# microsoft/StemGNN

Hardware: AMD Instinct MI355X
Metric: forecast-steps/sec (train) (higher is better)
Workload: dtype f32

## Files before the change

### include/stemgnn_hip.h

```cpp
#ifndef STEMGNN_HIP_H
#define STEMGNN_HIP_H

#include <stddef.h>
#include <stdint.h>

#ifdef __cplusplus
extern "C" {
#endif

#define SG_EINVAL (-10001)

#define SG_BLOCK_NPARAMS 33

const char* stemgnn_version(void);
int stemgnn_num_cus(void);

size_t stemgnn_table_floats(int W, int multi);
size_t stemgnn_packed_floats(int W, int multi);
size_t stemgnn_saved_floats(int B, int N, int W, int multi);
size_t stemgnn_scratch_floats(int B, int N, int W, int multi);
size_t stemgnn_gradpart_floats(int W, int multi, int nsplit);
size_t stemgnn_attn_saved_floats(int B, int N);
size_t stemgnn_attn_scratch_floats(int B, int N, int nchunk);
size_t stemgnn_scratch_offset_dG(int B, int N, int W, int multi);
// ... 81 lines not shown
int stemgnn_gru_bwd_rank2_ok(int B, int Hd);
int stemgnn_gru_bwd_rank2(const float* dkey, const float* dquery, const float* wk, const float* wq, const float* x,
                          const float* w_hh, const float* h_ext, const float* reserve, int B, int S, int Hd, int W,
                          float* scratch, float* dw_ih, float* dw_hh, float* db_ih, float* db_hh, int* status, void* stream);
int stemgnn_gru_bwd_rank2_dq(const float* dkey, float* dquery, int nchunk, int flags, const float* wk, const float* wq, const float* x,
                             const float* w_hh, const float* h_ext, const float* reserve, int B, int S, int Hd, int W,
                             float* scratch, float* dw_ih, float* dw_hh, float* db_ih, float* db_hh, int* status, void* stream);
int stemgnn_gru_bwd_overlap_ok(int B, int S, int Hd, int W);
size_t stemgnn_gru_bwd_ctl_words(int S);
int stemgnn_gru_bwd_rank2_begin(const float* dkey, const float* dquery, const float* wk, const float* wq, const float* x,
                                const float* w_hh, const float* h_ext, const float* reserve, int B, int S, int Hd, int W,
                                float* scratch, float* dw_ih, float* dw_hh, float* db_ih, float* db_hh, int* status,
                                unsigned* ctl, void* stream);
int stemgnn_gru_bwd_rank2_finish(const float* dkey, const float* dquery, const float* wk, const float* wq, const float* x,
                                 const float* w_hh, const float* h_ext, const float* reserve, int B, int S, int Hd, int W,
                                 float* scratch, float* dw_ih, float* dw_hh, float* db_ih, float* db_hh, int* status,
                                 unsigned* ctl, void* side_stream, void* stream);
int stemgnn_gru_bwd_recur(const float* dh_all, const float* x, const float* w_hh, const float* h_ext, const float* reserve,
                          int B, int S, int Hd, int W, float* scratch, int* status, void* stream);
int stemgnn_gru_bwd_rank2_recur(const float* dkey, float* dquery, int nchunk, const float* wk, const float* wq, const float* x,
                                const float* w_hh, const float* h_ext, const float* reserve, int B, int S, int Hd, int W,
                                float* scratch, int* status, void* stream);
int stemgnn_gru_input_grad(const float* scratch, const float* w_ih, int B, int S, int Hd, int W, float* dx, void* stream);

int stemgnn_block_pack(const float* const* params_host, const float* tables, float* packed,
                       int W, int multi, void* stream);
int stemgnn_block_pack_panels(const float* const* params_host, const float* tables, float* packed, int W, int multi,
                              void* stream);
int stemgnn_glu_fused_repack(float* packed, int W, int multi, void* stream);
int stemgnn_block_unpack_grads(const float* gradpart, int nsplit, const float* tables,
                               float* const* grads_host, int W, int multi, int has_backcast, void* stream);

int stemgnn_gft_fwd(const float* mul_L, const float* X, long xs_b, long xs_n, long xs_t,
                    float* G, int B, int N, int W, void* stream);
int stemgnn_gft_bwd(const float* mul_L, const float* X, long xs_b, long xs_n, long xs_t,
                    const float* dG, float* dX, float* dmul_L, int accumulate,
                    int B, int N, int W, void* stream);
int stemgnn_gft_bwd_dt2(const float* X0, long xs0_b, long xs0_n, long xs0_t, const float* dG0, const float* X1, long xs1_b,
                        long xs1_n, long xs1_t, const float* dG1, float* dmul_L, int B, int N, int W, void* stream);

int stemgnn_spectral_glu_fwd(const float* packed, float* saved, int B, int N, int W, int multi, void* stream);
int stemgnn_spectral_glu_bwd(const float* packed, const float* saved, float* scratch, float* gradpart,
                             int nsplit, int parts, int B, int N, int W, int multi, void* stream);
size_t stemgnn_glu_split_floats(int W, int multi, int splits);
int stemgnn_glu_split_panels(const float* packed, float* split, int W, int multi, int splits, void* stream);
int stemgnn_spectral_glu_fwd_split(const float* packed, const float* split, float* saved, int B, int N, int W, int multi,
                                   int splits, void* stream);
size_t stemgnn_glu_warm_saved_floats(int W, int multi);
int stemgnn_spectral_glu_fwd_warm(const float* packed, const float* split, float* saved, int B, int N, int W, int multi,
                                  int splits, void* stream);
int stemgnn_spectral_glu_dgrad_split(const float* packed, const float* split, const float* saved, float* scratch,
                                     int B, int N, int W, int multi, int splits, void* stream);
int stemgnn_glu_fused_bf16_ok(int W, int multi, int splits);

int stemgnn_igft_heads_fwd(const float* const* params_host, const float* packed, float* saved,
                           const float* X, long xs_b, long xs_n, long xs_t,
                           float* forecast, int accumulate, float* backcast,
                           int B, int N, int W, int multi, void* stream);
int stemgnn_igft_heads_bwd(const float* const* params_host, const float* packed, const float* saved,
                           const float* X, long xs_b, long xs_n, long xs_t,
                           const float* dforecast, const float* dbackcast, const float* backcast,
                           float* scratch, float* gradpart, int nsplit, int parts,
                           int B, int N, int W, int multi, void* stream);

int stemgnn_shortcut_dx(const float* scratch, const float* bs_w, float* dX, int B, int N, int W, int multi, void* stream);

int stemgnn_block_wgrad(const float* const* params_host, const float* packed, const float* saved,
                        const float* X, long xs_b, long xs_n, long xs_t, const float* dforecast, int has_bc,
                        float* scratch, float* gradpart, int nsplit, int cu_percent,
                        int B, int N, int W, int multi, void* stream);
int stemgnn_block_wgrad_split(const float* const* params_host, const float* packed, const float* saved,
                              const float* X, long xs_b, long xs_n, long xs_t, const float* dforecast, int has_bc,
                              float* scratch, float* gradpart, int nsplit, int cu_percent, int B, int N, int W,
                              int multi, int splits, void* stream);

#define SG_PATH_GLU_FWD_FUSED   1
#define SG_PATH_GLU_DGRAD_FUSED 2
#define SG_PATH_HEADS_FWD_FUSED 4
#define SG_PATH_HEADS_BWD_FUSED 8
#define SG_PATH_HEADS_BWD_16W   16
#define SG_PATH_LONG_K          32
#define SG_PATH_WGRAD_FUSED     64
#define SG_PATH_GLU_WGRAD_FUSED 128
int stemgnn_block_paths(int B, int N, int W, int multi, int splits);

size_t stemgnn_infer_workspace_floats(int B, int N, int W, int multi);
size_t stemgnn_infer_workspace_split_floats(int B, int N, int W, int multi, int splits);
int stemgnn_gru_fwd_infer(const float* x, const float* w_ih, const float* w_hh, const float* b_ih, const float* b_hh,
                          int B, int S, int Hd, int W, float* scratch, float* h_ext, int* status, void* stream);
int stemgnn_spectral_glu_fwd_infer(const float* packed, float* ws, size_t ws_floats, int B, int N, int W, int multi,
                                   void* stream);
int stemgnn_spectral_glu_fwd_split_infer(const float* packed, const float* split, float* ws, size_t ws_floats, int B, int N,
                                         int W, int multi, int splits, void* stream);
int stemgnn_igft_heads_fwd_infer(const float* const* params_host, const float* packed, float* ws, size_t ws_floats,
                                 const float* X, long xs_b, long xs_n, long xs_t, float* forecast, int accumulate,
                                 float* backcast, int B, int N, int W, int multi, void* stream);

int stemgnn_fc_tail_supported(int W, int H);
size_t stemgnn_fc_tail_scratch_floats(int B, int N, int W, int H);
int stemgnn_fc_tail_fwd(const float* fsum, const float* w0, const float* b0, const float* w2, const float* b2,
                        int B, int N, int W, int H, float* forecast, void* stream);
int stemgnn_fc_tail_bwd(const float* dforecast, const float* fsum, const float* w0, const float* b0, const float* w2,
                        int B, int N, int W, int H, float* scratch, float* dfsum, float* dw0, float* db0,
                        float* dw2, float* db2, void* stream);
size_t stemgnn_fc_tail_train_scratch_floats(int B, int N, int W, int H);
int stemgnn_fc_tail_train(const float* fsum, const float* target, const float* w0, const float* b0, const float* w2,
                          const float* b2, int B, int N, int W, int H, float* scratch, float* forecast,
                          float* loss, double* loss_accum, float* dfsum, float* dw0, float* db0, float* dw2,
                          float* db2, void* stream);
int stemgnn_fc_tail_train_rows(const float* fsum, const float* target, const float* w0, const float* b0, const float* w2,
                               const float* b2, int B, int N, int W, int H, float* scratch, float* forecast, float* dfsum,
                               void* stream);
int stemgnn_fc_tail_train_finish(const float* scratch, int B, int N, int W, int H, float* loss, double* loss_accum,
                                 float* dw0, float* db0, float* dw2, float* db2, void* stream);
int stemgnn_fill_zero(void* ptr, size_t bytes, void* stream);
int stemgnn_rmsprop_step(float* params, float* grads, float* square_avg, size_t n, const float* lr_dev,
                         float alpha, float eps, int zero_grad, float grad_scale, void* stream);

int stemgnn_adam_step(float* params, float* grads, float* exp_avg, float* exp_avg_sq, size_t n, const float* lr_dev,
                      float* step_dev, float beta1, float beta2, float eps, int zero_grad, float grad_scale,
                      void* stream);

int stemgnn_normalize_series(const double* raw, const double* sub, const double* div, int clip01, float* out,
                             long T, int N, void* stream);
int stemgnn_window_gather(const float* series, const long long* hi, float* x, float* y, int B, int W, int H, int N,
                          long T, int* status, void* stream);
int stemgnn_window_gather_queue(const float* series, const long long* order, long long* queue, float* x, float* y, int B,
                                int W, int H, int N, long T, int* status, void* stream);
size_t stemgnn_mse_scratch_floats(void);
int stemgnn_mse_fwd(const float* forecast, const float* target, size_t n, float* scratch, float* loss,
                    double* loss_accum, void* stream);
int stemgnn_mse_bwd(const float* forecast, const float* target, size_t n, const float* grad_loss, float* dforecast,
                    void* stream);
int stemgnn_roll_window(const float* inputs, const float* forecast, float* inputs_next, float* forecast_steps,
                        int B, int W, int L, int N, int step, int horizon, void* stream);
int stemgnn_forecast_store(const float* forecast, const float* target, const long long* pos, float* out_forecast,
                           float* out_target, int B, int H, int N, long capacity, void* stream);
size_t stemgnn_eval_scratch_doubles(long count, int H, int N);
size_t stemgnn_eval_out_doubles(int H, int N);
int stemgnn_eval_metrics(const float* target, const float* forecast, const double* mul, const double* add,
                         long count, int H, int N, double* scratch, double* out, void* stream);

#ifdef __cplusplus
}
#endif
#endif
```

### stemgnn_amd/_lib.py

```python
import ctypes
import os
from ctypes import POINTER, c_char_p, c_float, c_int, c_long, c_size_t, c_void_p

_HERE = os.path.dirname(os.path.abspath(__file__))
LIB_PATH = os.environ.get("STEMGNN_HIP_LIB", os.path.join(_HERE, "libstemgnn_hip.so"))
SG_BLOCK_NPARAMS = 33
SG_EINVAL = -10001
SG_PATH = {"glu_fwd_fused": 1, "glu_dgrad_fused": 2, "heads_fwd_fused": 4, "heads_bwd_fused": 8, "heads_bwd_16w": 16,
           "long_k": 32, "wgrad_fused": 64, "glu_wgrad_fused": 128}
SG_GRU_PATH_WORDS = 16
SG_GRU_WORD = {"fwd_family": 0, "fwd_P": 1, "fwd_K": 2, "gi_stream": 3, "bwd_family": 4, "bwd_P": 5, "bwd_KU": 6,
               "bwd_slices": 7, "ih_folded": 8, "hh_form": 9, "ih_slabs": 10, "rank2_ok": 11, "wide_passes": 12,
               "wide_MT": 13, "wide_GWf": 14, "wide_GWb": 15}
SG_GRU_FAM = {"stream": 0, "cluster1": 1, "cluster2": 2, "cluster4": 3, "wide": 4}
SG_GRU_HH = {"slabs": 0, "tiles": 1, "flat": 2}


def gru_paths(B, S, Hd, W, cus=0):
    out = (c_int * SG_GRU_PATH_WORDS)()
    check(load().stemgnn_gru_paths(B, S, Hd, W, cus, out), "stemgnn_gru_paths")
    return {k: int(out[i]) for k, i in SG_GRU_WORD.items()}


_P = c_void_p
_PP = POINTER(c_void_p)

SIGNATURES = {
    "stemgnn_version": (c_char_p, []),
    "stemgnn_num_cus": (c_int, []),
    "stemgnn_table_floats": (c_size_t, [c_int, c_int]),
    "stemgnn_packed_floats": (c_size_t, [c_int, c_int]),
    "stemgnn_saved_floats": (c_size_t, [c_int, c_int, c_int, c_int]),
    "stemgnn_scratch_floats": (c_size_t, [c_int, c_int, c_int, c_int]),
    "stemgnn_scratch_offset_dG": (c_size_t, [c_int, c_int, c_int, c_int]),
    "stemgnn_gradpart_floats": (c_size_t, [c_int, c_int, c_int]),
    "stemgnn_attn_saved_floats": (c_size_t, [c_int, c_int]),
    "stemgnn_attn_scratch_floats": (c_size_t, [c_int, c_int, c_int]),
    "stemgnn_make_tables_host": (c_int, [c_int, c_int, _P]),
    "stemgnn_attn_laplacian_fwd": (c_int, [_P, _P, _P, c_float, c_float, c_int, _P, c_int, c_int, _P, _P, _P, c_int, _P]),
    "stemgnn_attn_laplacian_bwd": (c_int, [_P, _P, _P, _P, c_float, c_float, c_int, _P, c_int, c_int, _P, _P, c_int,
                                           _P, _P, _P, c_int, _P]),
    "stemgnn_attn_laplacian_bwd_ext": (c_int, [_P, _P, _P, _P, _P, c_float, c_float, c_int, _P, c_int, c_int, _P, _P, c_int,
                                               _P, _P, _P, c_int, _P]),
    "stemgnn_dropout_mask": (c_int, [c_float, _P, c_int, c_int, _P, _P]),
    "stemgnn_dropout_seed_next": (c_int, [_P, _P, _P]),
    "stemgnn_cheb_fwd": (c_int, [_P, c_int, _P]),
    "stemgnn_cheb_bwd": (c_int, [_P, _P, _P, _P, c_int, _P]),
    "stemgnn_eigh_scratch_floats": (c_size_t, [c_int]),
    "stemgnn_eigh_fwd": (c_int, [_P, _P, _P, _P, c_int, c_int, _P]),
    "stemgnn_eigh_batched": (c_int, [_P, _P, _P, _P, c_int, c_int, _P]),
    "stemgnn_eigh_status": (c_int, []),
    "stemgnn_eigh_cluster_fixes": (c_int, []),
    "stemgnn_split_planes_floats": (c_size_t, [c_int, c_int, c_int]),
    "stemgnn_split_weights_bf16": (c_int, [_P, c_int, c_int, c_int, _P, _P]),
    "stemgnn_glu_gemm_bf16": (c_int, [_P, _P, _P, c_int, c_int, c_int, c_int, _P]),
    "stemgnn_glu_gemm_f32": (c_int, [_P, _P, _P, c_int, c_int, c_int, _P]),
    "stemgnn_sgemm_f32": (c_int, [_P, c_int, c_int, _P, c_int, c_int, _P, c_int, c_int, c_int, c_int, c_int, _P]),
    "stemgnn_glu_combine_fwd": (c_int, [_P, _P, _P, _P, _P, _P, _P, c_int, c_int, _P]),
    "stemgnn_glu_combine_bwd": (c_int, [_P, _P, _P, _P, _P, c_int, c_int, _P]),
    "stemgnn_colsum": (c_int, [_P, c_int, c_int, _P, _P]),
    "stemgnn_glu_fused_repack": (c_int, [_P, c_int, c_int, _P]),
    "stemgnn_shortcut_dx": (c_int, [_P, _P, _P, c_int, c_int, c_int, c_int, _P]),
    "stemgnn_gru_reserve_floats": (c_size_t, [c_int, c_int, c_int]),
    "stemgnn_gru_fwd_scratch_floats": (c_size_t, [c_int, c_int, c_int]),
    "stemgnn_gru_bwd_scratch_floats": (c_size_t, [c_int, c_int, c_int, c_int]),
    "stemgnn_gru_bwd_cus": (c_int, [c_int, c_int]),
    "stemgnn_gru_paths": (c_int, [c_int, c_int, c_int, c_int, c_int, POINTER(c_int)]),
    "stemgnn_gru_fwd": (c_int, [_P, _P, _P, _P, _P, c_int, c_int, c_int, c_int, _P, _P, _P, _P, _P]),
    "stemgnn_gru_bwd": (c_int, [_P, _P, _P, _P, _P, c_int, c_int, c_int, c_int, _P, _P, _P, _P, _P, _P, _P]),
    "stemgnn_gru_bwd_rank2_ok": (c_int, [c_int, c_int]),
    "stemgnn_gru_bwd_rank2": (c_int, [_P, _P, _P, _P, _P, _P, _P, _P, c_int, c_int, c_int, c_int, _P, _P, _P, _P, _P, _P, _P]),
    "stemgnn_gru_bwd_rank2_dq": (c_int, [_P, _P, c_int, c_int, _P, _P, _P, _P, _P, _P, c_int, c_int, c_int, c_int, _P, _P, _P, _P, _P, _P, _P]),
    "stemgnn_gru_bwd_overlap_ok": (c_int, [c_int, c_int, c_int, c_int]),
    "stemgnn_gru_bwd_ctl_words": (c_size_t, [c_int]),
    "stemgnn_gru_bwd_rank2_begin": (c_int, [_P, _P, _P, _P, _P, _P, _P, _P, c_int, c_int, c_int, c_int, _P, _P, _P, _P, _P, _P, _P, _P]),
    "stemgnn_gru_bwd_rank2_finish": (c_int, [_P, _P, _P, _P, _P, _P, _P, _P, c_int, c_int, c_int, c_int, _P, _P, _P, _P, _P, _P, _P, _P, _P]),
    "stemgnn_gru_bwd_recur": (c_int, [_P, _P, _P, _P, _P, c_int, c_int, c_int, c_int, _P, _P, _P]),
    "stemgnn_gru_bwd_rank2_recur": (c_int, [_P, _P, c_int, _P, _P, _P, _P, _P, _P, c_int, c_int, c_int, c_int, _P, _P, _P]),
    "stemgnn_gru_input_grad": (c_int, [_P, _P, c_int, c_int, c_int, c_int, _P, _P]),
    "stemgnn_keyquery_wgrad": (c_int, [_P, _P, _P, _P, c_int, c_int, _P]),
    "stemgnn_attn_dquery_reduce": (c_int, [_P, c_int, c_int, c_int, _P, _P]),
    "stemgnn_keyquery_wgrad2": (c_int, [_P, _P, _P, _P, _P, c_int, c_int, _P]),
    "stemgnn_fc_tail_supported": (c_int, [c_int, c_int]),
    "stemgnn_fc_tail_scratch_floats": (c_size_t, [c_int, c_int, c_int, c_int]),
    "stemgnn_fc_tail_fwd": (c_int, [_P, _P, _P, _P, _P, c_int, c_int, c_int, c_int, _P, _P]),
    "stemgnn_fc_tail_bwd": (c_int, [_P, _P, _P, _P, _P, c_int, c_int, c_int, c_int, _P, _P, _P, _P, _P, _P, _P]),
    "stemgnn_fill_zero": (c_int, [_P, c_size_t, _P]),
    "stemgnn_rmsprop_step": (c_int, [_P, _P, _P, c_size_t, _P, c_float, c_float, c_int, c_float, _P]),
    "stemgnn_adam_step": (c_int, [_P, _P, _P, _P, c_size_t, _P, _P, c_float, c_float, c_float, c_int, c_float, _P]),
    "stemgnn_normalize_series": (c_int, [_P, _P, _P, c_int, _P, c_long, c_int, _P]),
    "stemgnn_window_gather": (c_int, [_P, _P, _P, _P, c_int, c_int, c_int, c_int, c_long, _P, _P]),
    "stemgnn_window_gather_queue": (c_int, [_P, _P, _P, _P, _P, c_int, c_int, c_int, c_int, c_long, _P, _P]),
    "stemgnn_mse_scratch_floats": (c_size_t, []),
    "stemgnn_mse_fwd": (c_int, [_P, _P, c_size_t, _P, _P, _P, _P]),
    "stemgnn_mse_bwd": (c_int, [_P, _P, c_size_t, _P, _P, _P]),
    "stemgnn_roll_window": (c_int, [_P, _P, _P, _P, c_int, c_int, c_int, c_int, c_int, c_int, _P]),
    "stemgnn_forecast_store": (c_int, [_P, _P, _P, _P, _P, c_int, c_int, c_int, c_long, _P]),
    "stemgnn_eval_scratch_doubles": (c_size_t, [c_long, c_int, c_int]),
    "stemgnn_eval_out_doubles": (c_size_t, [c_int, c_int]),
    "stemgnn_eval_metrics": (c_int, [_P, _P, _P, _P, c_long, c_int, c_int, _P, _P, _P]),
    "stemgnn_block_pack": (c_int, [_PP, _P, _P, c_int, c_int, _P]),
    "stemgnn_block_pack_panels": (c_int, [_PP, _P, _P, c_int, c_int, _P]),
    "stemgnn_block_unpack_grads": (c_int, [_P, c_int, _P, _PP, c_int, c_int, c_int, _P]),
    "stemgnn_gft_fwd": (c_int, [_P, _P, c_long, c_long, c_long, _P, c_int, c_int, c_int, _P]),
    "stemgnn_gft_bwd": (c_int, [_P, _P, c_long, c_long, c_long, _P, _P, _P, c_int, c_int, c_int, c_int, _P]),
    "stemgnn_gft_bwd_dt2": (c_int, [_P, c_long, c_long, c_long, _P, _P, c_long, c_long, c_long, _P, _P, c_int, c_int, c_int, _P]),
    "stemgnn_spectral_glu_fwd": (c_int, [_P, _P, c_int, c_int, c_int, c_int, _P]),
    "stemgnn_spectral_glu_bwd": (c_int, [_P, _P, _P, _P, c_int, c_int, c_int, c_int, c_int, c_int, _P]),
    "stemgnn_glu_split_floats": (c_size_t, [c_int, c_int, c_int]),
    "stemgnn_glu_split_panels": (c_int, [_P, _P, c_int, c_int, c_int, _P]),
    "stemgnn_glu_fused_bf16_ok": (c_int, [c_int, c_int, c_int]),
    "stemgnn_block_paths": (c_int, [c_int, c_int, c_int, c_int, c_int]),
    "stemgnn_spectral_glu_fwd_split": (c_int, [_P, _P, _P, c_int, c_int, c_int, c_int, c_int, _P]),
    "stemgnn_glu_warm_saved_floats": (c_size_t, [c_int, c_int]),
    "stemgnn_spectral_glu_fwd_warm": (c_int, [_P, _P, _P, c_int, c_int, c_int, c_int, c_int, _P]),
    "stemgnn_spectral_glu_dgrad_split": (c_int, [_P, _P, _P, _P, c_int, c_int, c_int, c_int, c_int, _P]),
    "stemgnn_igft_heads_fwd": (c_int, [_PP, _P, _P, _P, c_long, c_long, c_long, _P, c_int, _P,
                                       c_int, c_int, c_int, c_int, _P]),
    "stemgnn_igft_heads_bwd": (c_int, [_PP, _P, _P, _P, c_long, c_long, c_long, _P, _P, _P, _P, _P, c_int, c_int,
                                       c_int, c_int, c_int, c_int, _P]),
    "stemgnn_fc_tail_train_scratch_floats": (c_size_t, [c_int, c_int, c_int, c_int]),
    "stemgnn_fc_tail_train": (c_int, [_P, _P, _P, _P, _P, _P, c_int, c_int, c_int, c_int, _P, _P, _P, _P, _P, _P, _P, _P,
                                      _P, _P]),
    "stemgnn_fc_tail_train_rows": (c_int, [_P, _P, _P, _P, _P, _P, c_int, c_int, c_int, c_int, _P, _P, _P, _P]),
    "stemgnn_fc_tail_train_finish": (c_int, [_P, c_int, c_int, c_int, c_int, _P, _P, _P, _P, _P, _P, _P]),
    "stemgnn_infer_workspace_floats": (c_size_t, [c_int, c_int, c_int, c_int]),
    "stemgnn_infer_workspace_split_floats": (c_size_t, [c_int, c_int, c_int, c_int, c_int]),
    "stemgnn_gru_fwd_infer": (c_int, [_P, _P, _P, _P, _P, c_int, c_int, c_int, c_int, _P, _P, _P, _P]),
    "stemgnn_spectral_glu_fwd_infer": (c_int, [_P, _P, c_size_t, c_int, c_int, c_int, c_int, _P]),
    "stemgnn_spectral_glu_fwd_split_infer": (c_int, [_P, _P, _P, c_size_t, c_int, c_int, c_int, c_int, c_int, _P]),
    "stemgnn_igft_heads_fwd_infer": (c_int, [_PP, _P, _P, c_size_t, _P, c_long, c_long, c_long, _P, c_int, _P,
                                             c_int, c_int, c_int, c_int, _P]),
    "stemgnn_block_wgrad": (c_int, [_PP, _P, _P, _P, c_long, c_long, c_long, _P, c_int, _P, _P, c_int, c_int,
                                    c_int, c_int, c_int, c_int, _P]),
    "stemgnn_block_wgrad_split": (c_int, [_PP, _P, _P, _P, c_long, c_long, c_long, _P, c_int, _P, _P, c_int, c_int,
                                          c_int, c_int, c_int, c_int, c_int, _P]),
}

_lib = None


class StemGNNHipError(RuntimeError):
    pass


def load():
    global _lib
    if _lib is not None:
        return _lib
    if not os.path.isfile(LIB_PATH):
        raise StemGNNHipError(
            f"{LIB_PATH} not found -- build it with `python __graft_entry__.py` (hipcc --offload-arch=gfx950); "
            "stemgnn_amd has no CPU / eager fallback.")
    lib = ctypes.CDLL(LIB_PATH)
    for name, (res, args) in SIGNATURES.items():
        fn = getattr(lib, name)
        fn.restype = res
        fn.argtypes = args
    _lib = lib
    return lib


def check(rc, what):
    if rc != 0:
        if rc == SG_EINVAL:
            raise StemGNNHipError(f"{what}: invalid argument (SG_EINVAL)")
        raise StemGNNHipError(f"{what}: HIP error {-rc}")


def ptr_array(tensors):
    arr = (c_void_p * SG_BLOCK_NPARAMS)()
    for i, t in enumerate(tensors):
        arr[i] = None if t is None else t.data_ptr()
    return arr
```

### stemgnn_amd/base_model.py

```python
import itertools
import os

import torch
import torch.nn as nn

from . import _lib, ops
from .ops import FcTail, FcTailMse, GruFront, SpectralHotPath, StockBlockFn

_instance_counter = itertools.count()
_BLOCK_FIELDS = ("forecast", "forecast_result", "backcast", "backcast_short_cut")
_FC_TAIL_MAX_W, _FC_TAIL_MAX_H = 64, 32


class GLU(nn.Module):

    def __init__(self, input_channel, output_channel):
        super().__init__()
        self.linear_left = nn.Linear(input_channel, output_channel)
        self.linear_right = nn.Linear(input_channel, output_channel)

    def forward(self, x):
        if not x.is_cuda:
            raise _lib.StemGNNHipError(f"input is on {x.device}: stemgnn_amd.GLU runs only on a HIP device (no CPU fallback)")
        lead = x.shape[:-1]
# ... 34 lines not shown
            raise _lib.StemGNNHipError(
                f"input is on {x.device}: stemgnn_amd.StockBlockLayer runs only on a HIP device (no CPU fallback)")
        B, _, N, W = x.shape
        forecast, backcast = StockBlockFn.apply(x.reshape(B, N, W), mul_L, self.multi, self.stack_cnt == 0,
                                                *self.hip_params())
        return forecast, (backcast.unsqueeze(1) if backcast is not None else None)


class Model(nn.Module):
    def __init__(self, units, stack_cnt, time_step, multi_layer, horizon=1, dropout_rate=0.5, leaky_rate=0.2,
                 device='cpu'):
        super().__init__()
        self.unit, self.stack_cnt, self.alpha = units, stack_cnt, leaky_rate
        self.time_step, self.horizon, self.multi_layer = time_step, horizon, multi_layer
        if time_step > _FC_TAIL_MAX_W or horizon > _FC_TAIL_MAX_H:
            raise _lib.StemGNNHipError(
                f"Model(time_step={time_step}, horizon={horizon}): the fc tail kernels (csrc/tail.hip) cover time_step <= "
                f"{_FC_TAIL_MAX_W} and horizon <= {_FC_TAIL_MAX_H}; stemgnn_amd has no torch fallback for larger ones")
        self.dropout_rate = float(dropout_rate)
        self.weight_key = nn.Parameter(torch.zeros(units, 1))
        nn.init.xavier_uniform_(self.weight_key.data, gain=1.414)
        self.weight_query = nn.Parameter(torch.zeros(units, 1))
        nn.init.xavier_uniform_(self.weight_query.data, gain=1.414)
        self.GRU = nn.GRU(time_step, units)
        self.stock_block = nn.ModuleList(
            StockBlockLayer(time_step, units, multi_layer, stack_cnt=i) for i in range(stack_cnt))
        self.fc = nn.Sequential(nn.Linear(time_step, time_step), nn.LeakyReLU(), nn.Linear(time_step, horizon))
        self._seed = None
        self._instance = next(_instance_counter)
        self.hot_state = ops.HotPathState()
        self.to(device)

    def _next_seed(self, device):
        if self._seed is None or self._seed.device != device:
            rank = 0
            if torch.distributed.is_available() and torch.distributed.is_initialized():
                rank = torch.distributed.get_rank()
            key = (torch.cuda.default_generators[device.index if device.index is not None
                                                 else torch.cuda.current_device()].initial_seed()
                   + 0x9E3779B97F4A7C15 * (self._instance + 1) + 0xD1B54A32D192ED03 * rank) % (1 << 62)
            self._seed = torch.tensor([key, 0], dtype=torch.int64, device=device)
        used = torch.empty_like(self._seed)
        _lib.check(_lib.load().stemgnn_dropout_seed_next(self._seed.data_ptr(), used.data_ptr(),
                                                         torch.cuda.current_stream(device).cuda_stream), "dropout_seed_next")
        return used

    def set_dropout_seed(self, seed, offset=0, device=None):
        device = device or self.weight_key.device
        self._seed = torch.tensor([int(seed), int(offset)], dtype=torch.int64, device=device)

    def __getstate__(self):
        state = self.__dict__.copy()
        state["_seed"] = None
        state["hot_state"] = None
        return state

    def __setstate__(self, state):
        self.__dict__.update(state)
        self._instance = next(_instance_counter)
        self.hot_state = ops.HotPathState()

    def train(self, mode=True):
        out = super().train(mode)
        dev = self.weight_key.device if hasattr(self, "weight_key") else None
        if dev is not None and dev.type == "cuda" and ops.gru_status_exists(dev) \
                and not torch.cuda.is_current_stream_capturing():
            ops.check_gru_status(dev)
            if os.environ.get("STEMGNN_SPECTRAL", "cheb") == "eig":
                ops.check_eigh_status(dev)
        return out

    def prefetch_side(self, device=None, batch=None):
        hs = self.hot_state
        if not hs.overlap or hs.prepacked is not None:
            return
        device = device or self.weight_key.device
        blocks = (self.stock_block[0].hip_params(), self.stock_block[1].hip_params())
        ops.prepack_blocks(hs, blocks, self.time_step, self.multi_layer, device,
                           batch_shape=None if batch is None else (int(batch), self.unit))
        if self.training and self.dropout_rate > 0.0:
            with torch.cuda.stream(ops._side_stream(device)):
                hs.preseed = self._next_seed(device)

    def hot_path(self, x):
        if not x.is_cuda:
            raise _lib.StemGNNHipError(
                f"input is on {x.device}: stemgnn_amd.Model runs only on a HIP device (no CPU fallback)")
        if self.stack_cnt > 2:
            raise AttributeError("'NoneType' object has no attribute 'unsqueeze'")
        if self.stack_cnt < 2:
            raise IndexError("list index out of range")
        x = x.contiguous()
        blocks = (self.stock_block[0].hip_params(), self.stock_block[1].hip_params())
        use_drop = self.training and self.dropout_rate > 0.0
        hs = self.hot_state
        if hs.overlap and hs.prepacked is None:
            self.prefetch_side(x.device, batch=x.shape[0])
        seed, hs.preseed = hs.preseed, None
        if seed is not None and not torch.cuda.is_current_stream_capturing():
            seed.record_stream(torch.cuda.current_stream())
        if os.environ.get("STEMGNN_GRU", "hip") == "miopen":
            h, _ = self.GRU(x.permute(2, 0, 1).contiguous())
        else:
            g = self.GRU
            h = GruFront.apply(x, g.weight_ih_l0, g.weight_hh_l0, g.bias_ih_l0, g.bias_hh_l0, hs)
            hs.gru_front_live = True
        if use_drop and seed is None:
            seed = self._next_seed(x.device)
        params = blocks[0] + blocks[1]
        return SpectralHotPath.apply(h, x, self.weight_key, self.weight_query, self.multi_layer, self.alpha,
                                     self.dropout_rate, self.training, seed, hs, *params)

    def loss(self, x, target, loss_out=None, accum=None, unit_grad=False, return_attention=False):
        self._require_fc_tail()
        fsum, attention, _ = self.hot_path(x)
        loss = FcTailMse.apply(fsum, target, self.fc[0].weight, self.fc[0].bias, self.fc[2].weight, self.fc[2].bias,
                               self.hot_state, loss_out, accum, bool(unit_grad) and torch.is_grad_enabled())
        return (loss, attention) if return_attention else loss

    def _require_fc_tail(self):
        if not _lib.load().stemgnn_fc_tail_supported(self.time_step, self.horizon):
            raise _lib.StemGNNHipError(f"fc tail: time_step={self.time_step}, horizon={self.horizon} outside the HIP kernels' "
                                       "range (time_step <= 64, horizon <= 32); stemgnn_amd has no torch fallback")

    def predict(self, x):
        self._require_fc_tail()
        if not x.is_cuda:
            raise _lib.StemGNNHipError(
                f"input is on {x.device}: stemgnn_amd.Model runs only on a HIP device (no CPU fallback)")
        if self.stack_cnt > 2:
            raise AttributeError("'NoneType' object has no attribute 'unsqueeze'")
        if self.stack_cnt < 2:
            raise IndexError("list index out of range")
        g = self.GRU
        blocks = self.stock_block[0].hip_params() + self.stock_block[1].hip_params()
        with torch.no_grad():
            return ops.forecast_forward(x, (g.weight_ih_l0, g.weight_hh_l0, g.bias_ih_l0, g.bias_hh_l0), self.weight_key,
                                        self.weight_query, self.multi_layer, self.alpha, self.dropout_rate, blocks,
                                        (self.fc[0].weight, self.fc[0].bias, self.fc[2].weight, self.fc[2].bias))

    def forward(self, x):
        self._require_fc_tail()
        fsum, attention, _ = self.hot_path(x)
        return FcTail.apply(fsum, self.fc[0].weight, self.fc[0].bias, self.fc[2].weight, self.fc[2].bias,
                            self.hot_state), attention
```

### stemgnn_amd/csrc/block.hip

```cpp
#include <hip/hip_runtime.h>

#include "../../include/stemgnn_hip.h"
#include "devattr.h"
#include "gemm2.h"
#include "gemm2s.h"
#include "gemm_core.h"
#include "gemm_phased.h"
#include "layout.h"
#include "reduce.h"
#include "wgrad.h"
#include "heads.h"
#include "glu_fused.h"
#include "glu_fused_bf16.h"

#define SG_TRY(e)                                \
  do {                                           \
    hipError_t _e = (e);                         \
    if (_e != hipSuccess) return -(int)_e;       \
  } while (0)

__device__ __forceinline__ float sg_sigmoid(float v) { return __frcp_rn(1.f + __expf(-v)); }

struct SgDiv {
  unsigned d, magic;
  __device__ __forceinline__ int div(int x) const { return d == 1u ? x : (int)__umulhi((unsigned)x, magic); }
  __device__ __forceinline__ void divmod(int x, int& q, int& r) const { q = div(x); r = x - q * (int)d; }
};
static inline SgDiv sg_div(int d) {
  SgDiv v;
  v.d = (unsigned)d;
  v.magic = d > 1 ? (unsigned)((1ull << 32) / (unsigned)d + 1ull) : 0u;
  return v;
}
static inline bool sg_div_ok(long xmax, int d) { return d >= 1 && xmax >= 0 && (unsigned long long)xmax * (unsigned)d < (1ull << 32); }

struct XView {
  const float* p;
  long sb, sn, st;
  int N;
  __device__ __forceinline__ float at(int b, int n, int t) const { return p[b * sb + n * sn + t * st]; }
  __device__ __forceinline__ float row(int m, int t) const {
    const int b = m / N;
    return at(b, m - b * N, t);
  }
};

struct GftFwdOp {
  const float* T;
  XView X;
  float* G;
  int B, N, W;
  SgDiv dN, dW;
  __device__ bool setup(int, int& M, int& Nn, int& K0, int& K1) const {
    M = 3 * N; Nn = B * W; K0 = 0; K1 = N;
    return true;
  }
  __device__ float a(int, int i, int k) const { return T[(size_t)i * N + k]; }
  __device__ float b(int, int k, int j) const {
    int bb, t;
    dW.divmod(j, bb, t);
    return X.at(bb, k, t);
  }
  __device__ void epi(int, int i, int j, float v) const {
    int kq, n, bb, t;
    dN.divmod(i, kq, n);
    dW.divmod(j, bb, t);
    G[((size_t)bb * N + n) * (3 * W) + kq * W + t] = v;
  }
};

struct GftBwdDxOp {
  const float* T;
  const float* dG;
  float* dX;
  int B, N, W;
  size_t slab;
  SgDiv dN, dW;
  __device__ bool setup(int, int& M, int& Nn, int& K0, int& K1) const {
    M = N; Nn = B * W; K0 = 0; K1 = 3 * N;
    return true;
  }
  __device__ float a(int, int i, int k) const { return T[(size_t)k * N + i]; }
  __device__ float b(int, int k, int j) const {
    int kq, n, bb, t;
    dN.divmod(k, kq, n);
    dW.divmod(j, bb, t);
    const size_t o = ((size_t)bb * N + n) * (3 * W) + kq * W + t;
    return dG[o] + dG[o + slab];
  }
  __device__ void epi(int, int i, int j, float v) const {
    int bb, t;
    dW.divmod(j, bb, t);
    dX[((size_t)bb * N + i) * W + t] = v;
  }
// ... 943 lines not shown
      a.out0[r] = saved + S.out[r][0]; a.gate0[r] = saved + S.gate[r][0];
      a.dact1[r] = scratch + C.dact[r][1]; a.dact0[r] = scratch + C.dact[r][0];
      a.dG[r] = scratch + C.dG + (size_t)r * d.M * d.KG;
      a.nstA[r] = gdg.nstA[r]; a.ns[r] = gdg.ns[r];
    }
    const dim3 grid(8 * ((a.nrb + 3) / 4));
    const size_t lds = mt == 3 ? gdg.lds_bytes3 : gdg.lds_bytes;
    static SgDynLds guard[4];
#define GD_LAUNCH(MT_, NT_, GI)                                                                            \
    do {                                                                                                  \
      SG_TRY(sg_ensure_dyn_lds((const void*)sg_glu_fused_dgrad_kernel<MT_, NT_>, lds, guard[GI]));         \
      hipLaunchKernelGGL((sg_glu_fused_dgrad_kernel<MT_, NT_>), grid, dim3(256), lds, st, a);              \
    } while (0)
    if (mt == 3) { if (gdg.nt == 2) GD_LAUNCH(3, 2, 3); else GD_LAUNCH(3, 1, 2); }
    else { if (gdg.nt == 2) GD_LAUNCH(2, 2, 1); else GD_LAUNCH(2, 1, 0); }
#undef GD_LAUNCH
    SG_TRY(hipGetLastError());
  }
  for (int l = 2; l >= 0; --l) {
    const int slot = l;
    if ((parts & 2) && !fused) {
      G2Args g;
      GluWgradEpi e;
      for (int r = 0; r < 2; ++r) {
        g.A[r] = scratch + C.dact[r][slot];
        g.lda[r] = sg_glu_np(d, l, r);
        g.B[r] = l == 0 ? saved + S.G : saved + S.out[r][l - 1];
        g.ldb[r] = l == 0 ? d.KG : d.CP;
        g.M[r] = sg_glu_np(d, l, r); g.N[r] = sg_glu_kin(d, l) + 1; g.K[r] = d.M;
        e.part[r] = gradpart + Gl.w[r][l];
      }
      g.nsplit = nsplit; g.chunk = chunk; g.b_ones_col = sg_glu_kin(d, l);
      SG_TRY((g2_launch<GluWgradEpi, false, false>(g, e, 2, st)));
    }
    if (!(parts & 1)) continue;
    if (fused_dgrad) continue;
    if (l > 0) {
      G2Args g;
      GluDpreEpi e;
      for (int r = 0; r < 2; ++r) {
        g.A[r] = scratch + C.dact[r][slot];
        g.lda[r] = sg_glu_np(d, l, r);
        g.B[r] = packed + P.w[r][l];
        g.ldb[r] = sg_glu_np(d, l, r);
        g.M[r] = d.M; g.N[r] = d.CP; g.K[r] = sg_glu_np(d, l, r);
        e.out[r] = saved + S.out[r][l - 1];
        e.gate[r] = saved + S.gate[r][l - 1];
        e.dpre[r] = scratch + C.dact[r][l - 1];
      }
      e.cp = d.CP;
      g.nsplit = 1; g.chunk = (2 * d.CP + 15) & ~15; g.b_ones_col = -1;
      if (2 * d.CP > SG_LONG_K) SG_TRY((g2_launch<GluDpreEpi, true, true, 64, true>(g, e, 2, st)));
      else SG_TRY((g2_launch<GluDpreEpi, true, true, 64>(g, e, 2, st)));
    } else {
      GluDgrad0Op op;
      for (int r = 0; r < 2; ++r) { op.dpre[r] = scratch + C.dact[r][slot]; op.wp[r] = packed + P.w[r][0]; }
      op.dG = scratch + C.dG; op.np0 = sg_glu_np(d, 0, 0); op.KG = d.KG; op.M = d.M;
      if (op.np0 > SG_LONG_K) SG_TRY((sg_launch_gemm<GluDgrad0Op, 32, 64, true, true, false, 64, true>(op, d.M, d.KG, 2, st)));
      else SG_TRY((sg_launch_gemm<GluDgrad0Op, 32, 64, true, true, false, 64>(op, d.M, d.KG, 2, st)));
    }
  }
  if (parts & 2) {
    if (fused) {
      SG_TRY(wg_launch(wq, 6, d.M, gradpart + Gl.wg_ws, reinterpret_cast<unsigned*>(gradpart + Gl.wg_cnt), Gl.wg_smax, st, true, 100,
                       false, nullptr, nullptr, (parts & 4) != 0));
    } else if (nsplit > 1) {
      SgSlabRegions R;
      R.n = 0;
      for (int r = 0; r < 2; ++r)
        for (int l = 0; l < 3; ++l) {
          R.off[R.n] = Gl.w[r][l];
          R.slab[R.n] = (size_t)sg_glu_np(d, l, r) * (sg_glu_kin(d, l) + 1);
          ++R.n;
        }
      SG_TRY(sg_reduce_slabs(gradpart, R, nsplit, st));
    }
  }
  return 0;
}

static bool heads_fused_ok(const SgDims& d) {
  return hd_fwd_lds_floats(d.KF, d.WmP, d.W) * sizeof(float) <= (size_t)150 * 1024 && d.KF <= SG_LONG_K;
}
template <bool SAVE = true>
static int heads_fwd_impl(const float* const* params_host, const float* packed, const float* const (&a3)[2], float* ig, float* fs,
                          const float* X, long xs_b, long xs_n, long xs_t, float* forecast, int accumulate, float* backcast,
                          int B, int N, int W, int multi, void* stream) {
  const SgDims d = sg_dims(B, N, W, multi);
  const SgPackedLayout P = sg_packed_layout(d);
  hipStream_t st = (hipStream_t)stream;
  const int has_bc = backcast != nullptr;
  if (has_bc && (!params_host[5] || !params_host[6])) return SG_EINVAL;
  const size_t hd_bytes = hd_fwd_lds_floats(d.KF, d.WmP, W) * sizeof(float);
  if (heads_fused_ok(d)) {
    HeadsFwdArgs a;
    for (int r = 0; r < 2; ++r) { a.a3[r] = a3[r]; a.cp2[r] = d.CP2[r]; }
    a.wfold = packed + P.wfold;
    a.Fw = params_host[1]; a.Fb = params_host[2]; a.FRw = params_host[3]; a.FRb = params_host[4];
    a.BCw = params_host[5]; a.BCb = params_host[6]; a.BSw = params_host[7]; a.BSb = params_host[8];
    a.X = HdXView{X, xs_b, xs_n, xs_t, N};
    a.ig = ig; a.fs = fs; a.forecast = forecast; a.backcast = backcast;
    a.M = d.M; a.W = W; a.Wm = d.Wm; a.WmP = d.WmP; a.KF = d.KF; a.accumulate = accumulate; a.has_bc = has_bc;
    a.lda = hd_lda(d.KF); a.ldi = d.WmP + 1;
    static const int waves_env = getenv("STEMGNN_HEADS_FWD_WAVES") ? atoi(getenv("STEMGNN_HEADS_FWD_WAVES")) : 8;
    if (waves_env == 8) {
      static SgDynLds lds_guard8;
      SG_TRY(sg_ensure_dyn_lds((const void*)sg_heads_fwd_kernel<8, SAVE>, hd_bytes, lds_guard8));
      hipLaunchKernelGGL((sg_heads_fwd_kernel<8, SAVE>), dim3((d.M + HD_RB - 1) / HD_RB), dim3(512), hd_bytes, st, a);
    } else {
      static SgDynLds lds_guard;
      SG_TRY(sg_ensure_dyn_lds((const void*)sg_heads_fwd_kernel<4, SAVE>, hd_bytes, lds_guard));
      hipLaunchKernelGGL((sg_heads_fwd_kernel<4, SAVE>), dim3((d.M + HD_RB - 1) / HD_RB), dim3(256), hd_bytes, st, a);
    }
    SG_TRY(hipGetLastError());
    return 0;
  }
  {
    IgftOp op;
    if (!ig || !fs) return SG_EINVAL;
    for (int r = 0; r < 2; ++r) { op.a3[r] = a3[r]; op.cp2[r] = d.CP2[r]; }
    op.wfold = packed + P.wfold; op.ig = ig; op.M = d.M; op.Wm = d.Wm; op.WmP = d.WmP;
    if (d.KF > SG_LONG_K) SG_TRY((sg_launch_gemm<IgftOp, 32, 64, true, false, false, 64, true>(op, d.M, d.Wm, 1, st)));
    else SG_TRY((sg_launch_gemm<IgftOp, 32, 64, true, false, false, 64>(op, d.M, d.Wm, 1, st)));
  }
  {
    Head1Op op{ig, XView{X, xs_b, xs_n, xs_t, N},
               params_host[1], params_host[2], params_host[5], params_host[6], params_host[7], params_host[8],
               fs, backcast, d.M, W, d.Wm, has_bc};
    SG_TRY((sg_launch_gemm<Head1Op, 32, 64, true, true, false, 64>(op, d.M, d.Wm + (has_bc ? W : 0), 1, st)));
  }
  {
    Head2Op op{fs, params_host[3], params_host[4], forecast, d.M, W, d.Wm, accumulate};
    SG_TRY((sg_launch_gemm<Head2Op, 64, 32, true, true, false>(op, d.M, W, 1, st)));
  }
  return 0;
}

extern "C" int stemgnn_igft_heads_fwd(const float* const* params_host, const float* packed, float* saved,
                                      const float* X, long xs_b, long xs_n, long xs_t,
                                      float* forecast, int accumulate, float* backcast,
                                      int B, int N, int W, int multi, void* stream) {
  if (!params_host || !packed || !saved || !X || !forecast || B <= 0 || N <= 0 || W <= 0 || multi <= 0)
    return SG_EINVAL;
  const SgSavedLayout S = sg_saved_layout(sg_dims(B, N, W, multi));
  const float* const a3[2] = {saved + S.out[0][2], saved + S.out[1][2]};
  return heads_fwd_impl<true>(params_host, packed, a3, saved + S.ig, saved + S.fs, X, xs_b, xs_n, xs_t, forecast, accumulate,
                              backcast, B, N, W, multi, stream);
}

static bool infer_needs_pp(const SgDims& d, int splits) {
  const char* ef = getenv("STEMGNN_GLU_FUSED");
  const bool fused_on = !(ef && atoi(ef) == 0);
  const bool glu_fused = fused_on && gf_geom(d).ok && gb_geom(d).ok && splits != 3;
  return !glu_fused || !heads_fused_ok(d);
}
static size_t infer_ws_floats(int B, int N, int W, int multi, int splits) {
  if (B <= 0 || N <= 0 || W <= 0 || multi <= 0) return 0;
  const SgDims d = sg_dims(B, N, W, multi);
  return sg_infer_layout(d, infer_needs_pp(d, splits)).total;
}
extern "C" size_t stemgnn_infer_workspace_floats(int B, int N, int W, int multi) { return infer_ws_floats(B, N, W, multi, 0); }
extern "C" size_t stemgnn_infer_workspace_split_floats(int B, int N, int W, int multi, int splits) {
  if (splits != 0 && splits != 2 && splits != 3) return 0;
  return infer_ws_floats(B, N, W, multi, splits);
}
static bool infer_ws_ok(const SgDims& d, size_t ws_floats, bool* pp) {
  *pp = ws_floats >= sg_infer_layout(d, true).total;
  return ws_floats >= sg_infer_layout(d, false).total;
}
extern "C" int stemgnn_spectral_glu_fwd_infer(const float* packed, float* ws, size_t ws_floats, int B, int N, int W, int multi,
                                              void* stream) {
  if (!packed || !ws || B <= 0 || N <= 0 || W <= 0 || multi <= 0) return SG_EINVAL;
  const SgDims d = sg_dims(B, N, W, multi);
  bool pp = false;
  if (!infer_ws_ok(d, ws_floats, &pp)) return SG_EINVAL;
  return glu_fwd_impl<true>(packed, glu_bufs_infer(d, ws, pp), B, N, W, multi, stream, 0, false);
}
extern "C" int stemgnn_spectral_glu_fwd_split_infer(const float* packed, const float* split, float* ws, size_t ws_floats, int B,
                                                    int N, int W, int multi, int splits, void* stream) {
  if (!packed || !split || !ws || B <= 0 || N <= 0 || W <= 0 || multi <= 0 || splits < 2 || splits > 3) return SG_EINVAL;
  const SgDims d = sg_dims(B, N, W, multi);
  bool pp = false;
  if (!infer_ws_ok(d, ws_floats, &pp)) return SG_EINVAL;
  return glu_fwd_split_impl<true>(packed, split, glu_bufs_infer(d, ws, pp), B, N, W, multi, splits, stream);
}
extern "C" int stemgnn_igft_heads_fwd_infer(const float* const* params_host, const float* packed, float* ws, size_t ws_floats,
                                            const float* X, long xs_b, long xs_n, long xs_t, float* forecast, int accumulate,
                                            float* backcast, int B, int N, int W, int multi, void* stream) {
// ... 53 lines not shown
    const size_t hb = hd_bwd_lds_floats(d.WmP, W) * sizeof(float);
    if ((parts & 1) && heads_bwd_fused_ok(d)) {
      HeadsBwdArgs a;
      a.dfo = dforecast; a.dbc = dbackcast; a.bc = backcast; a.fs = saved + S.fs; a.wfold = packed + P.wfold;
      a.Fw = params_host[1]; a.FRw = params_host[3]; a.BCw = params_host[5];
      for (int r = 0; r < 2; ++r) {
        a.out2[r] = saved + S.out[r][2]; a.gate2[r] = saved + S.gate[r][2]; a.dpre2[r] = scratch + C.dact[r][2];
        a.cp2[r] = d.CP2[r];
      }
      a.dpF = dpF; a.dpB = dpB; a.dig = dig;
      a.M = d.M; a.W = W; a.Wm = d.Wm; a.WmP = d.WmP; a.KF = d.KF; a.has_bc = has_bc;
      a.ldi = d.WmP + 1; a.ldw = ((W + 3) & ~3) + 1;
      const int waves = heads_bwd_waves(d);
      if (waves == 16) {
        static SgDynLds lds_guard16;
        SG_TRY(sg_ensure_dyn_lds((const void*)sg_heads_bwd_kernel<16>, hb, lds_guard16));
        hipLaunchKernelGGL(sg_heads_bwd_kernel<16>, dim3((d.M + HD_RB - 1) / HD_RB), dim3(1024), hb, st, a);
      } else if (waves == 8) {
        static SgDynLds lds_guard8;
        SG_TRY(sg_ensure_dyn_lds((const void*)sg_heads_bwd_kernel<8>, hb, lds_guard8));
        hipLaunchKernelGGL(sg_heads_bwd_kernel<8>, dim3((d.M + HD_RB - 1) / HD_RB), dim3(512), hb, st, a);
      } else {
        static SgDynLds lds_guard;
        SG_TRY(sg_ensure_dyn_lds((const void*)sg_heads_bwd_kernel<4>, hb, lds_guard));
        hipLaunchKernelGGL(sg_heads_bwd_kernel<4>, dim3((d.M + HD_RB - 1) / HD_RB), dim3(256), hb, st, a);
      }
      SG_TRY(hipGetLastError());
      fused_data = true;
    }
  }
  if (fused_data) parts &= ~1;
  if ((parts & 1) && has_bc) {
    const size_t n = (size_t)d.M * W;
    const int blocks = (int)((n + 255) / 256 < 2048 ? (n + 255) / 256 : 2048);
    hipLaunchKernelGGL(sg_dsigmoid_kernel, dim3(blocks), dim3(256), 0, st, dbackcast, backcast, dpB, n);
    SG_TRY(hipGetLastError());
  }
  if (parts & 1) {
    Head2BwdOp op{dforecast, params_host[3], saved + S.fs, dpF, d.M, W, d.Wm};
    SG_TRY((sg_launch_gemm<Head2BwdOp, 32, 64, true, false, false>(op, d.M, d.Wm, 1, st)));
  }
  if (parts & 1) {
    DigOp op{dpF, dpB, params_host[1], params_host[5], dig, d.M, W, d.Wm, has_bc};
    SG_TRY((sg_launch_gemm<DigOp, 32, 64, true, false, false, 64>(op, d.M, d.Wm, 1, st)));
  }
  if (parts & 1) {
    Da3Op op;
    op.dig = dig; op.wfold = packed + P.wfold;
    for (int r = 0; r < 2; ++r) {
      op.dpre[r] = scratch + C.dact[r][2];
      op.out[r] = saved + S.out[r][2];
      op.gate[r] = saved + S.gate[r][2];
      op.cp2[r] = d.CP2[r];
    }
    op.M = d.M; op.Wm = d.Wm; op.WmP = d.WmP;
    const int maxN = d.CP2[0] > d.CP2[1] ? d.CP2[0] : d.CP2[1];
    SG_TRY((sg_launch_gemm<Da3Op, 32, 64, true, true, false, 64>(op, d.M, maxN, 2, st)));
  }
  if (parts & 2) {
    HeadsWgradOp op;
    const float* a3[2] = {saved + S.out[0][2], saved + S.out[1][2]};
    const int huge = 1 << 30;
    auto set = [&](int w, const float* A0, int lda, int rows, float sg, const float* Bp, int ldb, int ncolB, float* part,
                   int ldp, int enabled) {
      op.pa0[w] = A0; op.pa1[w] = A0; op.lda0[w] = lda; op.lda1[w] = lda; op.split[w] = huge; op.Mw[w] = rows;
      op.Nw[w] = ldp; op.nb[w] = ncolB; op.rdiv[w] = huge; op.ldp[w] = ldp; op.on[w] = enabled; op.sign[w] = sg;
      op.pb[w] = Bp; op.sb[w] = 0; op.sn[w] = ldb; op.st[w] = 1; op.part[w] = part;
    };
    set(0, dforecast, W, W, 1.f, saved + S.fs, d.Wm, d.Wm, gradpart + Gl.fr, d.Wm + 1, 1);
    set(1, dpF, d.Wm, d.Wm, 1.f, saved + S.ig, d.Wm, d.Wm, gradpart + Gl.fc, d.Wm + 1, 1);
    set(2, dpB, W, W, 1.f, saved + S.ig, d.Wm, d.Wm, gradpart + Gl.bc, d.Wm + 1, has_bc);
    set(3, dpB, W, W, -1.f, X, 0, W, gradpart + Gl.bs, W + 1, has_bc);
    op.rdiv[3] = N; op.sb[3] = xs_b; op.sn[3] = xs_n; op.st[3] = xs_t;
    set(4, a3[0], d.CP2[0], d.KF, 1.f, dig, d.Wm, d.Wm, gradpart + Gl.wfold, d.WmP, 1);
    op.pa1[4] = a3[1]; op.lda1[4] = d.CP2[1]; op.split[4] = d.CP2[0]; op.Nw[4] = d.Wm;
    op.M = d.M; op.S = nsplit; op.chunk = split_chunk(d.M, nsplit);
    const int maxM = d.KF > d.Wm ? d.KF : d.Wm;
    SG_TRY((sg_launch_gemm<HeadsWgradOp, 64, 64, false, false, false, 64>(op, maxM, d.Wm + 1, 5 * nsplit, st)));
    SG_TRY(heads_reduce(d, Gl, gradpart, nsplit, has_bc, 31, st));
  }
  return 0;
}

__global__ void sg_shortcut_dx_kernel(const float* __restrict__ dpB, const float* __restrict__ bs_w, float* __restrict__ dX,
                                      size_t M, int W) {
  const size_t idx = (size_t)blockIdx.x * blockDim.x + threadIdx.x;
  if (idx >= M * W) return;
  const size_t m = idx / W;
  const int t = (int)(idx - m * W);
  float acc = 0.f;
  for (int o = 0; o < W; ++o) acc = fmaf(dpB[m * W + o], bs_w[(size_t)o * W + t], acc);
  dX[idx] -= acc;
}
extern "C" int stemgnn_shortcut_dx(const float* scratch, const float* bs_w, float* dX, int B, int N, int W, int multi,
                                   void* stream) {
  if (!scratch || !bs_w || !dX || B <= 0 || N <= 0 || W <= 0 || multi <= 0) return SG_EINVAL;
  const SgDims d = sg_dims(B, N, W, multi);
  const SgScratchLayout C = sg_scratch_layout(d);
  const size_t n = (size_t)d.M * W;
  hipLaunchKernelGGL(sg_shortcut_dx_kernel, dim3((unsigned)((n + 255) / 256)), dim3(256), 0, (hipStream_t)stream,
                     scratch + C.dpB, bs_w, dX, (size_t)d.M, W);
  SG_TRY(hipGetLastError());
  return 0;
}

static bool block_wgrad_list(const SgDims& d, const float* saved, const float* scratch, const float* dforecast, float* gradpart,
                             const SgGradLayout& Gl, int has_bc, WgGemm* q, int* n_out) {
  const SgSavedLayout S = sg_saved_layout(d);
  const SgScratchLayout C = sg_scratch_layout(d);
  const int W = d.W;
  int n = 0;
  bool ok = true;
  auto add = [&](const float* A, int lda, int Mi, const float* Bp, int ldb, int ncolB, bool ones, float* out, int ldo) {
    WgGemm& g = q[n++];
    g.A = A; g.lda = lda; g.Mi = Mi; g.B = Bp; g.ldb = ldb; g.Nj = ncolB + (ones ? 1 : 0); g.ones_col = ones ? ncolB : -1;
    g.out = out; g.ldo = ldo; g.out_bias = nullptr;
    ok = ok && wg_gemm_ok(g);
  };
  for (int l = 0; l < 3; ++l)
    for (int r = 0; r < 2; ++r)
      add(scratch + C.dact[r][l], sg_glu_np(d, l, r), sg_glu_np(d, l, r), l == 0 ? saved + S.G : saved + S.out[r][l - 1],
          l == 0 ? d.KG : d.CP, sg_glu_kin(d, l), true, gradpart + Gl.w[r][l], sg_glu_kin(d, l) + 1);
  add(dforecast, W, W, saved + S.fs, d.Wm, d.Wm, true, gradpart + Gl.fr, d.Wm + 1);
  add(scratch + C.dpF, d.Wm, d.Wm, saved + S.ig, d.Wm, d.Wm, true, gradpart + Gl.fc, d.Wm + 1);
  if (has_bc) add(scratch + C.dpB, W, W, saved + S.ig, d.Wm, d.Wm, true, gradpart + Gl.bc, d.Wm + 1);
  for (int r = 0; r < 2; ++r)
    add(saved + S.out[r][2], d.CP2[r], d.CP2[r], scratch + C.dig, d.Wm, d.Wm, false,
        gradpart + Gl.wfold + (r ? (size_t)d.CP2[0] * d.WmP : 0), d.WmP);
  *n_out = n;
  return ok && wg_tiles_fit(q, n);
}

static int block_wgrad_impl(const float* const* params_host, const float* packed, const float* saved,
                            const float* X, long xs_b, long xs_n, long xs_t, const float* dforecast, int has_bc,
                            float* scratch, float* gradpart, int nsplit, int cu_percent, int B, int N, int W,
                            int multi, void* stream, int splits) {
  if (!params_host || !packed || !saved || !X || !dforecast || !scratch || !gradpart || nsplit <= 0 || B <= 0 || N <= 0 ||
      W <= 0 || multi <= 0)
    return SG_EINVAL;
  const SgDims d = sg_dims(B, N, W, multi);
  const SgScratchLayout C = sg_scratch_layout(d);
  const SgGradLayout Gl = sg_grad_layout(d, nsplit);
  hipStream_t st = (hipStream_t)stream;
  has_bc = has_bc ? 1 : 0;
  if (has_bc && !params_host[5]) return SG_EINVAL;
  WgGemm q[WG_MAXG];
  int n = 0;
  const bool ok = block_wgrad_list(d, saved, scratch, dforecast, gradpart, Gl, has_bc, q, &n);
  if (!ok) {
    const int rc = stemgnn_igft_heads_bwd(params_host, packed, saved, X, xs_b, xs_n, xs_t, dforecast,
                                          has_bc ? dforecast : nullptr, has_bc ? dforecast : nullptr, scratch, gradpart,
                                          nsplit, 2, B, N, W, multi, stream);
    if (rc) return rc;
    return stemgnn_spectral_glu_bwd(packed, saved, scratch, gradpart, nsplit, 2, B, N, W, multi, stream);
  }
  SG_TRY(wg_launch(q, n, d.M, gradpart + Gl.wg_ws, reinterpret_cast<unsigned*>(gradpart + Gl.wg_cnt), Gl.wg_smax, st, true,
                   cu_percent, false, nullptr, nullptr, splits == 2));
  if (has_bc) {
    HeadsWgradOp op;
    const int huge = 1 << 30;
    for (int w = 0; w < 5; ++w) {
      op.pa0[w] = op.pa1[w] = scratch + C.dpB; op.lda0[w] = op.lda1[w] = W; op.split[w] = huge; op.Mw[w] = W; op.Nw[w] = W + 1;
      op.nb[w] = W; op.rdiv[w] = huge; op.ldp[w] = W + 1; op.on[w] = 0; op.sign[w] = 1.f; op.pb[w] = X; op.sb[w] = 0;
      op.sn[w] = 0; op.st[w] = 1; op.part[w] = gradpart + Gl.bs;
    }
    op.on[3] = 1; op.sign[3] = -1.f; op.rdiv[3] = N; op.sb[3] = xs_b; op.sn[3] = xs_n; op.st[3] = xs_t;
    op.M = d.M; op.S = nsplit; op.chunk = split_chunk(d.M, nsplit);
    SG_TRY((sg_launch_gemm<HeadsWgradOp, 64, 64, false, false, false, 64>(op, W, W + 1, 5 * nsplit, st)));
    SG_TRY(heads_reduce(d, Gl, gradpart, nsplit, 1, 16, st));
  }
  return 0;
}

extern "C" int stemgnn_block_wgrad(const float* const* params_host, const float* packed, const float* saved,
                                   const float* X, long xs_b, long xs_n, long xs_t, const float* dforecast, int has_bc,
                                   float* scratch, float* gradpart, int nsplit, int cu_percent, int B, int N, int W,
                                   int multi, void* stream) {
  return block_wgrad_impl(params_host, packed, saved, X, xs_b, xs_n, xs_t, dforecast, has_bc, scratch, gradpart, nsplit,
                          cu_percent, B, N, W, multi, stream, 0);
}
extern "C" int stemgnn_block_wgrad_split(const float* const* params_host, const float* packed, const float* saved,
                                         const float* X, long xs_b, long xs_n, long xs_t, const float* dforecast, int has_bc,
                                         float* scratch, float* gradpart, int nsplit, int cu_percent, int B, int N, int W,
                                         int multi, int splits, void* stream) {
  if (splits != 0 && splits != 2) return SG_EINVAL;
  return block_wgrad_impl(params_host, packed, saved, X, xs_b, xs_n, xs_t, dforecast, has_bc, scratch, gradpart, nsplit,
                          cu_percent, B, N, W, multi, stream, splits);
}

extern "C" int stemgnn_block_paths(int B, int N, int W, int multi, int splits) {
  if (B <= 0 || N <= 0 || W <= 0 || multi <= 0 || (splits != 0 && splits != 2 && splits != 3)) return SG_EINVAL;
  const SgDims d = sg_dims(B, N, W, multi);
  float* const base = reinterpret_cast<float*>((uintptr_t)256);
  const int nsplit = 32;
  const SgGradLayout Gl = sg_grad_layout(d, nsplit);
  const int mode = glu_fused_mode();
  int bits = 0;
  if (splits == 0 ? glu_fwd_fused_ok(d, mode, base) : glu_fwd_fused_bf16_ok(d, splits)) bits |= SG_PATH_GLU_FWD_FUSED;
  if (splits == 0 ? glu_dgrad_fused_ok(d, mode, base, base) : glu_dgrad_fused_bf16_ok(d, splits, base))
    bits |= SG_PATH_GLU_DGRAD_FUSED;
  if (heads_fused_ok(d)) bits |= SG_PATH_HEADS_FWD_FUSED;
  if (heads_bwd_fused_ok(d)) {
    bits |= SG_PATH_HEADS_BWD_FUSED;
    if (heads_bwd_waves(d) == 16) bits |= SG_PATH_HEADS_BWD_16W;
  }
  if (d.KF > SG_LONG_K) bits |= SG_PATH_LONG_K;
  WgGemm q[WG_MAXG];
  int n = 0;
  if (block_wgrad_list(d, base, base, base, base, Gl, 1, q, &n)) bits |= SG_PATH_WGRAD_FUSED;
  WgGemm wq[6];
  if (glu_wgrad_list(d, base, base, base, Gl, wq)) bits |= SG_PATH_GLU_WGRAD_FUSED;
  return bits;
}
```

### stemgnn_amd/csrc/heads.h

```cpp
#pragma once
#include <hip/hip_runtime.h>

constexpr int HD_RB = 32;
typedef float hd_f4 __attribute__((ext_vector_type(4)));

struct HdXView {
  const float* p;
  long sb, sn, st;
  int N;
};

struct HeadsFwdArgs {
  const float* a3[2];
  int cp2[2];
  const float* wfold;
  const float *Fw, *Fb, *FRw, *FRb, *BCw, *BCb, *BSw, *BSb;
  HdXView X;
  float *ig, *fs, *forecast, *backcast;
  int M, W, Wm, WmP, KF, accumulate, has_bc;
  int lda, ldi;
};

static inline int hd_lda(int KF) { return ((KF + 31) & ~31) + 2; }
static inline size_t hd_fwd_lds_floats(int KF, int WmP, int W) {
  return (size_t)HD_RB * hd_lda(KF) + 2 * (size_t)HD_RB * (WmP + 1) + (size_t)HD_RB * (((W + 3) & ~3) + 1);
}

template <class BF>
__device__ __forceinline__ void hd_gemm_tile(const float* __restrict__ Al, int lda, int K, BF Bf, int j, int kq, int i,
                                             hd_f4& c0, hd_f4& c1) {
  const float* a0p = Al + i * lda + kq;
  const float* a1p = a0p + 16 * lda;
  float b[8], nb[8];
  const int nfull = K >> 5;
  if (nfull > 0) {
#pragma unroll
    for (int u = 0; u < 8; ++u) b[u] = Bf(4 * u + kq, j);
  }
  for (int t = 0; t < nfull; ++t) {
    const int k0 = t << 5;
    if (t + 1 < nfull) {
#pragma unroll
      for (int u = 0; u < 8; ++u) nb[u] = Bf(k0 + 32 + 4 * u + kq, j);
    }
#pragma unroll
    for (int u = 0; u < 8; ++u) {
      c0 = __builtin_amdgcn_mfma_f32_16x16x4f32(a0p[k0 + 4 * u], b[u], c0, 0, 0, 0);
      c1 = __builtin_amdgcn_mfma_f32_16x16x4f32(a1p[k0 + 4 * u], b[u], c1, 0, 0, 0);
    }
#pragma unroll
    for (int u = 0; u < 8; ++u) b[u] = nb[u];
  }
  const int ktail = nfull << 5, nrem = (K - ktail) >> 2;
#pragma unroll
  for (int u = 0; u < 8; ++u) b[u] = u < nrem ? Bf(ktail + 4 * u + kq, j) : 0.f;
#pragma unroll
  for (int u = 0; u < 8; ++u)
    if (u < nrem) {
      c0 = __builtin_amdgcn_mfma_f32_16x16x4f32(a0p[ktail + 4 * u], b[u], c0, 0, 0, 0);
      c1 = __builtin_amdgcn_mfma_f32_16x16x4f32(a1p[ktail + 4 * u], b[u], c1, 0, 0, 0);
    }
}

template <class BF>
__device__ __forceinline__ void hd_gemm_tile1(const float* __restrict__ Al, int lda, int K, BF Bf, int j, int kq, int i,
                                              hd_f4& c0) {
  const float* a0p = Al + i * lda + kq;
  float b[8], nb[8];
  const int nfull = K >> 5;
  if (nfull > 0) {
#pragma unroll
    for (int u = 0; u < 8; ++u) b[u] = Bf(4 * u + kq, j);
  }
  for (int t = 0; t < nfull; ++t) {
    const int k0 = t << 5;
    if (t + 1 < nfull) {
#pragma unroll
      for (int u = 0; u < 8; ++u) nb[u] = Bf(k0 + 32 + 4 * u + kq, j);
    }
#pragma unroll
    for (int u = 0; u < 8; ++u) c0 = __builtin_amdgcn_mfma_f32_16x16x4f32(a0p[k0 + 4 * u], b[u], c0, 0, 0, 0);
#pragma unroll
    for (int u = 0; u < 8; ++u) b[u] = nb[u];
  }
  const int ktail = nfull << 5, nrem = (K - ktail) >> 2;
#pragma unroll
  for (int u = 0; u < 8; ++u) b[u] = u < nrem ? Bf(ktail + 4 * u + kq, j) : 0.f;
#pragma unroll
  for (int u = 0; u < 8; ++u)
    if (u < nrem) c0 = __builtin_amdgcn_mfma_f32_16x16x4f32(a0p[ktail + 4 * u], b[u], c0, 0, 0, 0);
}

__device__ __forceinline__ float hd_sigmoid(float v) { return __frcp_rn(1.f + __expf(-v)); }

template <int NW, bool SAVE = true>
__global__ __launch_bounds__(NW * 64) void sg_heads_fwd_kernel(const HeadsFwdArgs g) {
  constexpr int NT = NW * 64;
  constexpr bool SPLIT = NW == 8;
  extern __shared__ __attribute__((aligned(16))) float hd_lds[];
  float* As = hd_lds;
  float* igs = As + HD_RB * g.lda;
  float* fss = igs + HD_RB * g.ldi;
  float* Xs = fss + HD_RB * g.ldi;
  const int tid = threadIdx.x, lane = tid & 63, wave = tid >> 6;
  const int m0 = blockIdx.x * HD_RB;
  const int M = g.M, W = g.W, Wm = g.Wm, KF = g.KF, lda = g.lda, ldi = g.ldi;
  const int KFp = (KF + 3) & ~3, Wmp4 = (Wm + 3) & ~3, W4 = (W + 3) & ~3;

  {
    const int cpr = KFp >> 2;
    const int nch = HD_RB * cpr;
    const int c0n = g.cp2[0] >> 2;
    for (int base = 0; base < nch; base += NT * 8) {
      float4 v[8];
#pragma unroll
      for (int u = 0; u < 8; ++u) {
        const int e = base + u * NT + tid;
        const int ee = e < nch ? e : nch - 1;
        const int row = ee / cpr, c = ee - row * cpr;
        const int m = m0 + row < M ? m0 + row : M - 1;
        const bool lo = c < c0n;
        const float* src = lo ? g.a3[0] + (size_t)m * g.cp2[0] + 4 * c
                              : g.a3[1] + (size_t)m * g.cp2[1] + 4 * (c - c0n < (g.cp2[1] >> 2) ? c - c0n : 0);
        v[u] = *reinterpret_cast<const float4*>(src);
      }
#pragma unroll
      for (int u = 0; u < 8; ++u) {
        const int e = base + u * NT + tid;
        if (e < nch) {
          const int row = e / cpr, c = e - row * cpr;
          float* d = As + row * lda + 4 * c;
          const bool live = 4 * c < KF;
          *reinterpret_cast<float2*>(d) = live ? make_float2(v[u].x, v[u].y) : make_float2(0.f, 0.f);
          *reinterpret_cast<float2*>(d + 2) = live ? make_float2(v[u].z, v[u].w) : make_float2(0.f, 0.f);
        }
      }
    }
  }
  const int xs = W4 + 1;
  for (int e = tid; e < HD_RB * W4; e += NT) {
    const int row = e / W4, t = e - row * W4;
    const int m = m0 + row < M ? m0 + row : M - 1;
    const int b = m / g.X.N;
    Xs[row * xs + t] = (t < W && g.has_bc) ? g.X.p[b * g.X.sb + (m - b * g.X.N) * g.X.sn + (t < W ? t : 0) * g.X.st] : 0.f;
  }
  for (int e = tid; e < HD_RB * 4; e += NT) {
    const int row = e >> 2, k = Wm + (e & 3);
    if (k < ldi) { igs[row * ldi + k] = 0.f; fss[row * ldi + k] = 0.f; }
  }
  __syncthreads();

  const int j = lane & 15, kq = lane >> 4;
  const int nct = (Wm + 15) >> 4;
  const int cw = SPLIT ? (wave & 3) : wave;
  const int rh = SPLIT ? (wave >> 2) : 0;
  for (int ct = cw; ct < nct; ct += 4) {
    hd_f4 c0 = {0.f, 0.f, 0.f, 0.f}, c1 = c0;
    const float* wf = g.wfold + ct * 16;
    const int WmP = g.WmP;
    auto Bf = [&](int k, int jj) { return wf[(size_t)(k < KF ? k : KF - 1) * WmP + jj]; };
    if constexpr (SPLIT) hd_gemm_tile1(As + rh * 16 * lda, lda, KFp, Bf, j, kq, j, c0);
    else hd_gemm_tile(As, lda, KFp, Bf, j, kq, j, c0, c1);
    const int col = ct * 16 + j;
#pragma unroll
    for (int reg = 0; reg < 4; ++reg) {
      const int r0 = rh * 16 + kq * 4 + reg, r1 = 16 + r0;
      if (col < Wm) {
        igs[r0 * ldi + col] = c0[reg];
        if (SAVE && m0 + r0 < M) g.ig[(size_t)(m0 + r0) * Wm + col] = c0[reg];
        if constexpr (!SPLIT) {
          igs[r1 * ldi + col] = c1[reg];
          if (SAVE && m0 + r1 < M) g.ig[(size_t)(m0 + r1) * Wm + col] = c1[reg];
        }
      }
    }
  }
  __syncthreads();
  for (int ct = cw; ct < nct; ct += 4) {
    hd_f4 c0 = {0.f, 0.f, 0.f, 0.f}, c1 = c0;
    const int col = ct * 16 + j;
    const float* fr = g.Fw + (size_t)(col < Wm ? col : Wm - 1) * Wm;
    auto Bf = [&](int k, int) { return fr[k < Wm ? k : Wm - 1]; };
    if constexpr (SPLIT) hd_gemm_tile1(igs + rh * 16 * ldi, ldi, Wmp4, Bf, j, kq, j, c0);
    else hd_gemm_tile(igs, ldi, Wmp4, Bf, j, kq, j, c0, c1);
    const float bias = g.Fb[col < Wm ? col : Wm - 1];
#pragma unroll
    for (int reg = 0; reg < 4; ++reg) {
      const int r0 = rh * 16 + kq * 4 + reg, r1 = 16 + r0;
      if (col < Wm) {
        const float s0 = hd_sigmoid(c0[reg] + bias);
        fss[r0 * ldi + col] = s0;
        if (SAVE && m0 + r0 < M) g.fs[(size_t)(m0 + r0) * Wm + col] = s0;
        if constexpr (!SPLIT) {
          const float s1 = hd_sigmoid(c1[reg] + bias);
          fss[r1 * ldi + col] = s1;
          if (SAVE && m0 + r1 < M) g.fs[(size_t)(m0 + r1) * Wm + col] = s1;
        }
      }
    }
  }
  __syncthreads();
  const int nwt = (W + 15) >> 4;
  const int rh3 = SPLIT ? ((wave >> 1) & 1) : 0;
  for (int ct = SPLIT ? (wave >> 2) : (wave >> 1); ct < nwt; ct += 2) {
    const int col = ct * 16 + j;
    const int cc = col < W ? col : W - 1;
    hd_f4 c0 = {0.f, 0.f, 0.f, 0.f}, c1 = c0;
    if ((wave & 1) == 0) {
      const float* fr = g.FRw + (size_t)cc * Wm;
      auto Bf = [&](int k, int) { return fr[k < Wm ? k : Wm - 1]; };
      if constexpr (SPLIT) hd_gemm_tile1(fss + rh3 * 16 * ldi, ldi, Wmp4, Bf, j, kq, j, c0);
      else hd_gemm_tile(fss, ldi, Wmp4, Bf, j, kq, j, c0, c1);
      const float bias = g.FRb[cc];
#pragma unroll
      for (int reg = 0; reg < 4; ++reg) {
        const int r0 = rh3 * 16 + kq * 4 + reg, r1 = 16 + r0;
        if (col < W) {
          if (m0 + r0 < M) { float* o = g.forecast + (size_t)(m0 + r0) * W + col; *o = (g.accumulate ? *o : 0.f) + c0[reg] + bias; }
          if constexpr (!SPLIT) {
            if (m0 + r1 < M) { float* o = g.forecast + (size_t)(m0 + r1) * W + col; *o = (g.accumulate ? *o : 0.f) + c1[reg] + bias; }
          }
        }
      }
    } else if (g.has_bc) {
      const float* bcr = g.BCw + (size_t)cc * Wm;
      auto Bc = [&](int k, int) { return bcr[k < Wm ? k : Wm - 1]; };
      hd_f4 d0 = {0.f, 0.f, 0.f, 0.f}, d1 = d0;
      const float* bsr = g.BSw + (size_t)cc * W;
      auto Bs = [&](int k, int) { return bsr[k < W ? k : W - 1]; };
      if constexpr (SPLIT) {
        hd_gemm_tile1(igs + rh3 * 16 * ldi, ldi, Wmp4, Bc, j, kq, j, c0);
        hd_gemm_tile1(Xs + rh3 * 16 * xs, xs, W4, Bs, j, kq, j, d0);
      } else {
        hd_gemm_tile(igs, ldi, Wmp4, Bc, j, kq, j, c0, c1);
        hd_gemm_tile(Xs, xs, W4, Bs, j, kq, j, d0, d1);
      }
      const float bias = g.BCb[cc] - g.BSb[cc];
#pragma unroll
      for (int reg = 0; reg < 4; ++reg) {
        const int r0 = rh3 * 16 + kq * 4 + reg, r1 = 16 + r0;
        if (col < W) {
          if (m0 + r0 < M) g.backcast[(size_t)(m0 + r0) * W + col] = hd_sigmoid(c0[reg] - d0[reg] + bias);
          if constexpr (!SPLIT) {
            if (m0 + r1 < M) g.backcast[(size_t)(m0 + r1) * W + col] = hd_sigmoid(c1[reg] - d1[reg] + bias);
          }
        }
      }
    }
  }
}

struct HeadsBwdArgs {
  const float *dfo, *dbc, *bc;
  const float* fs;
  const float* wfold;
  const float *Fw, *FRw, *BCw;
  const float* out2[2];
  const float* gate2[2];
  float* dpre2[2];
  int cp2[2];
  float *dpF, *dpB, *dig;
  int M, W, Wm, WmP, KF, has_bc;
  int ldi, ldw;
};
static inline size_t hd_bwd_lds_floats(int WmP, int W) {
  return 2 * (size_t)HD_RB * (WmP + 1) + 2 * (size_t)HD_RB * (((W + 3) & ~3) + 1);
}

template <int TJ, class BF>
__device__ __forceinline__ void hd_gemm_tiles(const float* __restrict__ Al, int lda, int K, BF Bf, int kq, int i,
                                              hd_f4 (&c)[TJ][2]) {
  const float* a0p = Al + i * lda + kq;
  const float* a1p = a0p + 16 * lda;
  const int nb8 = (K + 31) >> 5;
  float b[TJ][8], nb[TJ][8];
#pragma unroll
  for (int t = 0; t < TJ; ++t)
#pragma unroll
    for (int u = 0; u < 8; ++u) b[t][u] = Bf(4 * u + kq, t);
  for (int bt = 0; bt < nb8; ++bt) {
    const int k0 = bt << 5;
    if (bt + 1 < nb8) {
#pragma unroll
      for (int t = 0; t < TJ; ++t)
#pragma unroll
        for (int u = 0; u < 8; ++u) nb[t][u] = Bf(k0 + 32 + 4 * u + kq, t);
    }
#pragma unroll
    for (int u = 0; u < 8; ++u) {
      if (k0 + 4 * u < K) {
        const float a0 = a0p[k0 + 4 * u], a1 = a1p[k0 + 4 * u];
#pragma unroll
        for (int t = 0; t < TJ; ++t) {
          c[t][0] = __builtin_amdgcn_mfma_f32_16x16x4f32(a0, b[t][u], c[t][0], 0, 0, 0);
          c[t][1] = __builtin_amdgcn_mfma_f32_16x16x4f32(a1, b[t][u], c[t][1], 0, 0, 0);
        }
      }
    }
#pragma unroll
    for (int t = 0; t < TJ; ++t)
#pragma unroll
      for (int u = 0; u < 8; ++u) b[t][u] = nb[t][u];
  }
}

template <int NW>
__global__ __launch_bounds__(NW * 64) void sg_heads_bwd_kernel(const HeadsBwdArgs g) {
  constexpr int NT = NW * 64;
  extern __shared__ __attribute__((aligned(16))) float hd_lds[];
  float* dpFs = hd_lds;
  float* digs = dpFs + HD_RB * g.ldi;
  float* dfos = digs + HD_RB * g.ldi;
  float* dpBs = dfos + HD_RB * g.ldw;
  const int tid = threadIdx.x, lane = tid & 63, wave = tid >> 6;
  const int m0 = blockIdx.x * HD_RB;
  const int M = g.M, W = g.W, Wm = g.Wm, KF = g.KF, ldi = g.ldi, ldw = g.ldw, WmP = g.WmP;
  const int Wmp4 = (Wm + 3) & ~3, W4 = (W + 3) & ~3;

  const int j = lane & 15, kq = lane >> 4;
  const int nkt = (KF + 15) >> 4;
  constexpr int TJ = 16 / NW;
  const bool hoist = nkt <= 16;
  float gt[TJ][2][4], yv[TJ][2][4];
  auto load_saved = [&](int ct0) {
#pragma unroll
    for (int t = 0; t < TJ; ++t) {
      const int kk = (ct0 + t) * 16 + j;
      const int kc = kk < KF ? kk : KF - 1;
      const int r = kc >= g.cp2[0];
      const int cch = kc - (r ? g.cp2[0] : 0), cp = g.cp2[r];
      const float* pg = g.gate2[r] + cch;
      const float* py = g.out2[r] + cch;
#pragma unroll
      for (int reg = 0; reg < 4; ++reg)
#pragma unroll
        for (int h = 0; h < 2; ++h) {
          const int mm = m0 + h * 16 + kq * 4 + reg;
          const size_t o = (size_t)(mm < M ? mm : M - 1) * cp;
          gt[t][h][reg] = pg[o];
          yv[t][h][reg] = py[o];
        }
    }
  };
  if (hoist) load_saved(wave * TJ);
  const int nct = (Wm + 15) >> 4;
  const bool hoist_fs = nct <= NW;
  float sv[2][4];
  auto load_fs = [&](int ct) {
    const int col = ct * 16 + j, cc = col < Wm ? col : Wm - 1;
#pragma unroll
    for (int reg = 0; reg < 4; ++reg)
#pragma unroll
      for (int h = 0; h < 2; ++h) {
        const int r = h * 16 + kq * 4 + reg;
        const int m = m0 + r < M ? m0 + r : M - 1;
        sv[h][reg] = g.fs[(size_t)m * Wm + cc];
      }
  };
  if (hoist_fs) load_fs(wave < nct ? wave : nct - 1);

  for (int e = tid; e < HD_RB * W4; e += NT) {
    const int row = e / W4, t = e - row * W4;
    const int m = m0 + row < M ? m0 + row : M - 1;
    const size_t o = (size_t)m * W + (t < W ? t : 0);
    const float df = g.dfo[o];
    float pb = 0.f;
    if (g.has_bc) {
      const float s = g.bc[o];
      pb = g.dbc[o] * s * (1.f - s);
      if (t < W && m0 + row < M) g.dpB[o] = pb;
    }
    dfos[row * ldw + t] = t < W ? df : 0.f;
    dpBs[row * ldw + t] = t < W ? pb : 0.f;
  }
  for (int e = tid; e < HD_RB * 4; e += NT) {
    const int row = e >> 2, k = Wm + (e & 3);
    if (k < ldi) { dpFs[row * ldi + k] = 0.f; digs[row * ldi + k] = 0.f; }
  }
  __syncthreads();

  for (int ct = wave; ct < nct; ct += NW) {
    hd_f4 c[1][2] = {{{0.f, 0.f, 0.f, 0.f}, {0.f, 0.f, 0.f, 0.f}}};
    const int col = ct * 16 + j, cc = col < Wm ? col : Wm - 1;
    const float* fr = g.FRw + cc;
    hd_gemm_tiles<1>(dfos, ldw, W4, [&](int k, int) { return fr[(size_t)(k < W ? k : W - 1) * Wm]; }, kq, j, c);
    if (!hoist_fs) load_fs(ct);
#pragma unroll
    for (int reg = 0; reg < 4; ++reg)
#pragma unroll
      for (int h = 0; h < 2; ++h) {
        const int r = h * 16 + kq * 4 + reg;
        const float s = sv[h][reg];
        const float v = c[0][h][reg] * s * (1.f - s);
        if (col < Wm) {
          dpFs[r * ldi + col] = v;
          if (m0 + r < M) g.dpF[(size_t)(m0 + r) * Wm + col] = v;
        }
      }
  }
  __syncthreads();
  for (int ct = wave; ct < nct; ct += NW) {
    hd_f4 c[1][2] = {{{0.f, 0.f, 0.f, 0.f}, {0.f, 0.f, 0.f, 0.f}}};
    const int col = ct * 16 + j, cc = col < Wm ? col : Wm - 1;
    const float* fw = g.Fw + cc;
    hd_gemm_tiles<1>(dpFs, ldi, Wmp4, [&](int k, int) { return fw[(size_t)(k < Wm ? k : Wm - 1) * Wm]; }, kq, j, c);
    if (g.has_bc) {
      const float* bw = g.BCw + cc;
      hd_gemm_tiles<1>(dpBs, ldw, W4, [&](int k, int) { return bw[(size_t)(k < W ? k : W - 1) * Wm]; }, kq, j, c);
    }
#pragma unroll
    for (int reg = 0; reg < 4; ++reg)
#pragma unroll
      for (int h = 0; h < 2; ++h) {
        const int r = h * 16 + kq * 4 + reg;
        if (col < Wm) {
          digs[r * ldi + col] = c[0][h][reg];
          if (m0 + r < M) g.dig[(size_t)(m0 + r) * Wm + col] = c[0][h][reg];
        }
      }
  }
  __syncthreads();
  for (int ct0 = wave * TJ; ct0 < nkt; ct0 += TJ * NW) {
    hd_f4 c[TJ][2];
#pragma unroll
    for (int t = 0; t < TJ; ++t) { c[t][0] = (hd_f4){0.f, 0.f, 0.f, 0.f}; c[t][1] = c[t][0]; }
    const float* wr[TJ];
#pragma unroll
    for (int t = 0; t < TJ; ++t) {
      const int kk = (ct0 + t) * 16 + j;
      wr[t] = g.wfold + (size_t)(kk < KF ? kk : KF - 1) * WmP;
    }
    hd_gemm_tiles<TJ>(digs, ldi, Wmp4, [&](int k, int t) { return wr[t][k < Wm ? k : Wm - 1]; }, kq, j, c);
    if (!hoist) load_saved(ct0);
#pragma unroll
    for (int t = 0; t < TJ; ++t) {
      const int kk = (ct0 + t) * 16 + j;
      const int kc = kk < KF ? kk : KF - 1;
      const int r = kc >= g.cp2[0];
      const int cch = kc - (r ? g.cp2[0] : 0), cp = g.cp2[r];
      const int q = ((cch >> 4) << 5) + (cch & 15);
#pragma unroll
      for (int reg = 0; reg < 4; ++reg)
#pragma unroll
        for (int h = 0; h < 2; ++h) {
          const int m = m0 + h * 16 + kq * 4 + reg;
          const float v = c[t][h][reg];
          if (m < M && kk < KF) {
            float* dp = g.dpre2[r] + (size_t)m * 2 * cp + q;
            dp[0] = v * gt[t][h][reg];
            dp[16] = v * yv[t][h][reg] * (1.f - gt[t][h][reg]);
          }
        }
    }
  }
}
```

### stemgnn_amd/csrc/tail.hip

```cpp
#include <hip/hip_runtime.h>
#include <stdint.h>

#include "../../include/stemgnn_hip.h"
#include "devattr.h"

#define SG_TRY(e)                                \
  do {                                           \
    hipError_t _e = (e);                         \
    if (_e != hipSuccess) return -(int)_e;       \
  } while (0)

constexpr int TAIL_MAXW = 64;
constexpr int TAIL_MAXH = 32;
constexpr int TAIL_RB = 64;


__global__ __launch_bounds__(256) void sg_fc_tail_fwd_kernel(const float* __restrict__ fsum, const float* __restrict__ w0,
                                                             const float* __restrict__ b0, const float* __restrict__ w2,
                                                             const float* __restrict__ b2, int B, int N, int W, int H,
                                                             float* __restrict__ forecast) {
  extern __shared__ __attribute__((aligned(16))) float sm[];
  float* sw0 = sm;
  float* sb0 = sw0 + W * W;
  float* sw2 = sb0 + W;
  float* sb2 = sw2 + H * W;
  float* sx = sb2 + H;
  float* sa = sx + TAIL_RB * (W + 1);
  const int tid = threadIdx.x, r = tid & 63, q = tid >> 6;
  const int M = B * N, m0 = blockIdx.x * TAIL_RB, m = m0 + r;
  for (int i = tid; i < W * W; i += 256) sw0[i] = w0[i];
  for (int i = tid; i < W; i += 256) sb0[i] = b0[i];
  for (int i = tid; i < H * W; i += 256) sw2[i] = w2[i];
  for (int i = tid; i < H; i += 256) sb2[i] = b2[i];
  for (int i = tid; i < TAIL_RB * W; i += 256) {
    const int rr = i / W, t = i - rr * W;
    sx[rr * (W + 1) + t] = m0 + rr < M ? fsum[(size_t)m0 * W + i] : 0.f;
  }
  __syncthreads();
  for (int t = q; t < W; t += 4) {
    float z = sb0[t];
    for (int u = 0; u < W; ++u) z = fmaf(sx[r * (W + 1) + u], sw0[t * W + u], z);
    sa[r * (W + 1) + t] = z > 0.f ? z : 0.01f * z;
  }
  __syncthreads();
  if (m < M) {
    const int b = m / N, n = m - b * N;
    for (int h = q; h < H; h += 4) {
      float y = sb2[h];
      for (int t = 0; t < W; ++t) y = fmaf(sa[r * (W + 1) + t], sw2[h * W + t], y);
      forecast[((size_t)b * H + h) * N + n] = y;
    }
  }
}

__global__ __launch_bounds__(256) void sg_fc_tail_bwd_kernel(const float* __restrict__ dforecast, const float* __restrict__ fsum,
                                                             const float* __restrict__ w0, const float* __restrict__ b0,
                                                             const float* __restrict__ w2, int B, int N, int W, int H,
                                                             float* __restrict__ dfsum, float* __restrict__ partial) {
  extern __shared__ __attribute__((aligned(16))) float sm[];
  const int nacc = W * W + W + H * W + H;
  float* sw0 = sm;
  float* sb0 = sw0 + W * W;
  float* sw2 = sb0 + W;
  float* sx = sw2 + H * W;
  float* sdz = sx + TAIL_RB * (W + 1);
  float* sa = sdz + TAIL_RB * (W + 1);
  float* sdy = sa + TAIL_RB * (W + 1);
  const int tid = threadIdx.x, r = tid & 63, q = tid >> 6;
  const int M = B * N, m0 = blockIdx.x * TAIL_RB, m = m0 + r;
  for (int i = tid; i < W * W; i += 256) sw0[i] = w0[i];
  for (int i = tid; i < W; i += 256) sb0[i] = b0[i];
  for (int i = tid; i < H * W; i += 256) sw2[i] = w2[i];
  for (int i = tid; i < TAIL_RB * W; i += 256) {
    const int rr = i / W, t = i - rr * W;
    sx[rr * (W + 1) + t] = m0 + rr < M ? fsum[(size_t)m0 * W + i] : 0.f;
  }
  {
    const int mc = m < M ? m : 0, b = mc / N, n = mc - b * N;
    for (int h = q; h < H; h += 4) sdy[r * (H + 1) + h] = m < M ? dforecast[((size_t)b * H + h) * N + n] : 0.f;
  }
  __syncthreads();
  for (int t = q; t < W; t += 4) {
    float z = sb0[t];
    for (int u = 0; u < W; ++u) z = fmaf(sx[r * (W + 1) + u], sw0[t * W + u], z);
    float da = 0.f;
    for (int h = 0; h < H; ++h) da = fmaf(sdy[r * (H + 1) + h], sw2[h * W + t], da);
    sa[r * (W + 1) + t] = m < M ? (z > 0.f ? z : 0.01f * z) : 0.f;
    sdz[r * (W + 1) + t] = m < M ? (z > 0.f ? da : 0.01f * da) : 0.f;
  }
  __syncthreads();
  if (m < M)
    for (int u = q; u < W; u += 4) {
      float d = 0.f;
      for (int t = 0; t < W; ++t) d = fmaf(sdz[r * (W + 1) + t], sw0[t * W + u], d);
      dfsum[(size_t)m * W + u] = d;
    }
// ... 1 lines not shown
    float sum = 0.f;
    if (e < W * W) {
      const int t = e / W, u = e - t * W;
      for (int rr = 0; rr < TAIL_RB; ++rr) sum = fmaf(sdz[rr * (W + 1) + t], sx[rr * (W + 1) + u], sum);
    } else if (e < W * W + W) {
      const int t = e - W * W;
      for (int rr = 0; rr < TAIL_RB; ++rr) sum += sdz[rr * (W + 1) + t];
    } else if (e < W * W + W + H * W) {
      const int qq = e - W * W - W, h = qq / W, t = qq - h * W;
      for (int rr = 0; rr < TAIL_RB; ++rr) sum = fmaf(sdy[rr * (H + 1) + h], sa[rr * (W + 1) + t], sum);
    } else {
      const int h = e - W * W - W - H * W;
      for (int rr = 0; rr < TAIL_RB; ++rr) sum += sdy[rr * (H + 1) + h];
    }
    partial[(size_t)blockIdx.x * nacc + e] = sum;
  }
}

__global__ __launch_bounds__(256) void sg_fc_tail_reduce_kernel(const float* __restrict__ partial, int nblocks, int W, int H,
                                                                float* __restrict__ dw0, float* __restrict__ db0,
                                                                float* __restrict__ dw2, float* __restrict__ db2) {
  __shared__ float red[4][64];
  const int nacc = W * W + W + H * W + H;
  const int i = blockIdx.x * 64 + (threadIdx.x & 63), q = threadIdx.x >> 6;
  float s = 0.f;
  if (i < nacc)
    for (int b = q; b < nblocks; b += 4) s += partial[(size_t)b * nacc + i];
  red[q][threadIdx.x & 63] = s;
  __syncthreads();
  if (q != 0 || i >= nacc) return;
  s = (red[0][threadIdx.x] + red[1][threadIdx.x]) + (red[2][threadIdx.x] + red[3][threadIdx.x]);
  if (i < W * W) dw0[i] = s;
  else if (i < W * W + W) db0[i - W * W] = s;
  else if (i < W * W + W + H * W) dw2[i - W * W - W] = s;
  else db2[i - W * W - W - H * W] = s;
}

static size_t fc_tail_fwd_lds(int W, int H) { return (size_t)(W * W + W + H * W + H + 2 * TAIL_RB * (W + 1)) * sizeof(float); }
static size_t fc_tail_bwd_lds(int W, int H) {
  return (size_t)(W * W + W + H * W + TAIL_RB * (3 * (W + 1) + H + 1)) * sizeof(float);
}
extern "C" int stemgnn_fc_tail_supported(int W, int H) {
  return W > 0 && H > 0 && W <= TAIL_MAXW && H <= TAIL_MAXH && fc_tail_bwd_lds(W, H) <= 150 * 1024;
}
extern "C" size_t stemgnn_fc_tail_scratch_floats(int B, int N, int W, int H) {
  return (size_t)((B * N + TAIL_RB - 1) / TAIL_RB) * (W * W + W + H * W + H);
}

extern "C" int stemgnn_fc_tail_fwd(const float* fsum, const float* w0, const float* b0, const float* w2, const float* b2,
                                   int B, int N, int W, int H, float* forecast, void* stream) {
  if (!fsum || !w0 || !b0 || !w2 || !b2 || !forecast || B <= 0 || N <= 0 || !stemgnn_fc_tail_supported(W, H))
    return SG_EINVAL;
  const size_t lds = fc_tail_fwd_lds(W, H);
  static SgDynLds lds_guard;
  SG_TRY(sg_ensure_dyn_lds((const void*)sg_fc_tail_fwd_kernel, lds, lds_guard));
  hipLaunchKernelGGL(sg_fc_tail_fwd_kernel, dim3((B * N + TAIL_RB - 1) / TAIL_RB), dim3(256), lds, (hipStream_t)stream, fsum,
                     w0, b0, w2, b2, B, N, W, H, forecast);
  SG_TRY(hipGetLastError());
  return 0;
}

extern "C" int stemgnn_fc_tail_bwd(const float* dforecast, const float* fsum, const float* w0, const float* b0,
                                   const float* w2, int B, int N, int W, int H, float* scratch, float* dfsum, float* dw0,
                                   float* db0, float* dw2, float* db2, void* stream) {
  if (!dforecast || !fsum || !w0 || !b0 || !w2 || !scratch || !dfsum || !dw0 || !db0 || !dw2 || !db2 || B <= 0 ||
      N <= 0 || W <= 0 || H <= 0 || W > TAIL_MAXW || H > TAIL_MAXH)
    return SG_EINVAL;
  hipStream_t st = (hipStream_t)stream;
  const int nacc = W * W + W + H * W + H;
  const int nblocks = (B * N + TAIL_RB - 1) / TAIL_RB;
  const size_t lds = fc_tail_bwd_lds(W, H);
  if (!stemgnn_fc_tail_supported(W, H)) return SG_EINVAL;
  static SgDynLds lds_guard;
  SG_TRY(sg_ensure_dyn_lds((const void*)sg_fc_tail_bwd_kernel, lds, lds_guard));
  hipLaunchKernelGGL(sg_fc_tail_bwd_kernel, dim3(nblocks), dim3(256), lds, st, dforecast, fsum, w0, b0, w2, B, N, W, H, dfsum,
                     scratch);
  SG_TRY(hipGetLastError());
  hipLaunchKernelGGL(sg_fc_tail_reduce_kernel, dim3((nacc + 63) / 64), dim3(256), 0, st, scratch, nblocks, W, H, dw0,
                     db0, dw2, db2);
  SG_TRY(hipGetLastError());
  return 0;
}

constexpr int TRAIN_RB = 32;
constexpr int TRAIN_RQ = 256 / TRAIN_RB;
__global__ __launch_bounds__(256) void sg_fc_tail_train_kernel(const float* __restrict__ fsum, const float* __restrict__ target,
                                                               const float* __restrict__ w0, const float* __restrict__ b0,
                                                               const float* __restrict__ w2, const float* __restrict__ b2,
                                                               int B, int N, int W, int H, float* __restrict__ forecast,
                                                               float* __restrict__ dfsum, float* __restrict__ partial) {
  extern __shared__ __attribute__((aligned(16))) float sm[];
  const int nacc = W * W + W + H * W + H;
  float* sw0 = sm;
  float* sb0 = sw0 + W * W;
  float* sw2 = sb0 + W;
  float* sb2 = sw2 + H * W;
  float* sx = sb2 + H;
  float* sdz = sx + TRAIN_RB * (W + 1);
  float* sa = sdz + TRAIN_RB * (W + 1);
  float* sdy = sa + TRAIN_RB * (W + 1);
  float* sred = sdy + TRAIN_RB * (H + 1);
  const int tid = threadIdx.x, r = tid % TRAIN_RB, q = tid / TRAIN_RB;
  const int M = B * N, m0 = blockIdx.x * TRAIN_RB, m = m0 + r;
  for (int i = tid; i < W * W; i += 256) sw0[i] = w0[i];
  for (int i = tid; i < W; i += 256) sb0[i] = b0[i];
  for (int i = tid; i < H * W; i += 256) sw2[i] = w2[i];
  for (int i = tid; i < H; i += 256) sb2[i] = b2[i];
  for (int i = tid; i < TRAIN_RB * W; i += 256) {
    const int rr = i / W, t = i - rr * W;
    sx[rr * (W + 1) + t] = m0 + rr < M ? fsum[(size_t)m0 * W + i] : 0.f;
  }
  __syncthreads();
  for (int t = q; t < W; t += TRAIN_RQ) {
    float z = sb0[t];
    for (int u = 0; u < W; ++u) z = fmaf(sx[r * (W + 1) + u], sw0[t * W + u], z);
    sdz[r * (W + 1) + t] = z;
    sa[r * (W + 1) + t] = m < M ? (z > 0.f ? z : 0.01f * z) : 0.f;
  }
  __syncthreads();
  float sq = 0.f;
  {
    const int mc = m < M ? m : 0, b = mc / N, n = mc - b * N;
    const float scale = 2.f / ((float)B * (float)H * (float)N);
    for (int h = q; h < H; h += TRAIN_RQ) {
      float y = sb2[h];
      for (int t = 0; t < W; ++t) y = fmaf(sa[r * (W + 1) + t], sw2[h * W + t], y);
      const size_t o = ((size_t)b * H + h) * N + n;
      const float d = m < M ? y - target[o] : 0.f;
      if (m < M && forecast) forecast[o] = y;
      sq = fmaf(d, d, sq);
      sdy[r * (H + 1) + h] = d * scale;
    }
  }
  sred[tid] = sq;
  __syncthreads();
  for (int t = q; t < W; t += TRAIN_RQ) {
    const float z = sdz[r * (W + 1) + t];
    float da = 0.f;
    for (int h = 0; h < H; ++h) da = fmaf(sdy[r * (H + 1) + h], sw2[h * W + t], da);
    sdz[r * (W + 1) + t] = m < M ? (z > 0.f ? da : 0.01f * da) : 0.f;
  }
  __syncthreads();
  if (m < M)
    for (int u = q; u < W; u += TRAIN_RQ) {
      float d = 0.f;
      for (int t = 0; t < W; ++t) d = fmaf(sdz[r * (W + 1) + t], sw0[t * W + u], d);
      dfsum[(size_t)m * W + u] = d;
    }
  for (int e = tid; e < nacc + 1; e += 256) {
    float sum = 0.f;
    if (e < W * W) {
      const int t = e / W, u = e - t * W;
      for (int rr = 0; rr < TRAIN_RB; ++rr) sum = fmaf(sdz[rr * (W + 1) + t], sx[rr * (W + 1) + u], sum);
    } else if (e < W * W + W) {
      const int t = e - W * W;
      for (int rr = 0; rr < TRAIN_RB; ++rr) sum += sdz[rr * (W + 1) + t];
    } else if (e < W * W + W + H * W) {
      const int qq = e - W * W - W, h = qq / W, t = qq - h * W;
      for (int rr = 0; rr < TRAIN_RB; ++rr) sum = fmaf(sdy[rr * (H + 1) + h], sa[rr * (W + 1) + t], sum);
    } else if (e < nacc) {
      const int h = e - W * W - W - H * W;
      for (int rr = 0; rr < TRAIN_RB; ++rr) sum += sdy[rr * (H + 1) + h];
    } else {
      for (int i = 0; i < 256; ++i) sum += sred[i];
    }
    partial[(size_t)blockIdx.x * (nacc + 1) + e] = sum;
  }
}

__global__ __launch_bounds__(256) void sg_fc_tail_train_reduce_kernel(const float* __restrict__ partial, int nblocks, int W,
                                                                      int H, float inv_n, float* __restrict__ dw0,
                                                                      float* __restrict__ db0, float* __restrict__ dw2,
                                                                      float* __restrict__ db2, float* __restrict__ loss,
                                                                      double* __restrict__ accum) {
  __shared__ float red[4][64];
  const int nacc = W * W + W + H * W + H;
  const int i = blockIdx.x * 64 + (threadIdx.x & 63), q = threadIdx.x >> 6;
  float s = 0.f;
  if (i <= nacc)
    for (int b = q; b < nblocks; b += 32) {
      float v[8];
#pragma unroll
      for (int u = 0; u < 8; ++u) {
        const int bb = b + 4 * u;
        const float x = partial[(size_t)(bb < nblocks ? bb : nblocks - 1) * (nacc + 1) + i];
        v[u] = bb < nblocks ? x : 0.f;
      }
#pragma unroll
      for (int u = 0; u < 8; ++u) s += v[u];
    }
  red[q][threadIdx.x & 63] = s;
  __syncthreads();
  if (q != 0 || i > nacc) return;
  s = (red[0][threadIdx.x] + red[1][threadIdx.x]) + (red[2][threadIdx.x] + red[3][threadIdx.x]);
  if (i < W * W) dw0[i] = s;
  else if (i < W * W + W) db0[i - W * W] = s;
  else if (i < W * W + W + H * W) dw2[i - W * W - W] = s;
  else if (i < nacc) db2[i - W * W - W - H * W] = s;
  else {
    const float l = s * inv_n;
    loss[0] = l;
    if (accum) accum[0] += (double)l;
  }
}

static size_t fc_tail_train_lds(int W, int H) {
  return (size_t)(W * W + W + H * W + H + TRAIN_RB * (3 * (W + 1) + H + 1) + 256) * sizeof(float);
}
extern "C" size_t stemgnn_fc_tail_train_scratch_floats(int B, int N, int W, int H) {
  return (size_t)((B * N + TRAIN_RB - 1) / TRAIN_RB) * (W * W + W + H * W + H + 1);
}
static int fc_tail_train_impl(const float* fsum, const float* target, const float* w0, const float* b0, const float* w2,
                              const float* b2, int B, int N, int W, int H, float* scratch, float* forecast, float* loss,
                              double* loss_accum, float* dfsum, float* dw0, float* db0, float* dw2, float* db2, void* stream,
                              int parts) {
  if (!scratch || B <= 0 || N <= 0 || !stemgnn_fc_tail_supported(W, H) || fc_tail_train_lds(W, H) > 150 * 1024) return SG_EINVAL;
  if ((parts & 1) && (!fsum || !target || !w0 || !b0 || !w2 || !b2 || !dfsum)) return SG_EINVAL;
  if ((parts & 2) && (!loss || !dw0 || !db0 || !dw2 || !db2)) return SG_EINVAL;
  hipStream_t st = (hipStream_t)stream;
  const int nacc = W * W + W + H * W + H;
  const int nblocks = (B * N + TRAIN_RB - 1) / TRAIN_RB;
  if (parts & 1) {
    const size_t lds = fc_tail_train_lds(W, H);
    static SgDynLds lds_guard;
    SG_TRY(sg_ensure_dyn_lds((const void*)sg_fc_tail_train_kernel, lds, lds_guard));
    hipLaunchKernelGGL(sg_fc_tail_train_kernel, dim3(nblocks), dim3(256), lds, st, fsum, target, w0, b0, w2, b2, B, N, W, H,
                       forecast, dfsum, scratch);
    SG_TRY(hipGetLastError());
  }
  if (parts & 2) {
    hipLaunchKernelGGL(sg_fc_tail_train_reduce_kernel, dim3((nacc + 1 + 63) / 64), dim3(256), 0, st, scratch, nblocks, W, H,
                       1.f / ((float)B * (float)H * (float)N), dw0, db0, dw2, db2, loss, loss_accum);
    SG_TRY(hipGetLastError());
  }
  return 0;
}
extern "C" int stemgnn_fc_tail_train(const float* fsum, const float* target, const float* w0, const float* b0, const float* w2,
                                     const float* b2, int B, int N, int W, int H, float* scratch, float* forecast,
                                     float* loss, double* loss_accum, float* dfsum, float* dw0, float* db0, float* dw2,
                                     float* db2, void* stream) {
  return fc_tail_train_impl(fsum, target, w0, b0, w2, b2, B, N, W, H, scratch, forecast, loss, loss_accum, dfsum, dw0, db0, dw2,
                            db2, stream, 3);
}
extern "C" int stemgnn_fc_tail_train_rows(const float* fsum, const float* target, const float* w0, const float* b0,
                                          const float* w2, const float* b2, int B, int N, int W, int H, float* scratch,
                                          float* forecast, float* dfsum, void* stream) {
  return fc_tail_train_impl(fsum, target, w0, b0, w2, b2, B, N, W, H, scratch, forecast, nullptr, nullptr, dfsum, nullptr,
                            nullptr, nullptr, nullptr, stream, 1);
}
extern "C" int stemgnn_fc_tail_train_finish(const float* scratch, int B, int N, int W, int H, float* loss, double* loss_accum,
                                            float* dw0, float* db0, float* dw2, float* db2, void* stream) {
  return fc_tail_train_impl(nullptr, nullptr, nullptr, nullptr, nullptr, nullptr, B, N, W, H, const_cast<float*>(scratch),
                            nullptr, loss, loss_accum, nullptr, dw0, db0, dw2, db2, stream, 2);
}

__global__ void sg_rmsprop_kernel(float* __restrict__ p, float* __restrict__ g, float* __restrict__ sq, size_t n,
                                  const float* __restrict__ lr_dev, float alpha, float eps, int zero_grad,
                                  float gscale) {
  const float lr = lr_dev[0];
  size_t i = ((size_t)blockIdx.x * blockDim.x + threadIdx.x) * 4;
  const size_t stride = (size_t)gridDim.x * blockDim.x * 4;
  for (; i + 3 < n; i += stride) {
    float4 pv = *reinterpret_cast<float4*>(p + i), gv = *reinterpret_cast<float4*>(g + i),
           sv = *reinterpret_cast<float4*>(sq + i);
    gv.x *= gscale; gv.y *= gscale; gv.z *= gscale; gv.w *= gscale;
    sv.x = alpha * sv.x + (1.f - alpha) * gv.x * gv.x; pv.x -= lr * gv.x / (sqrtf(sv.x) + eps);
    sv.y = alpha * sv.y + (1.f - alpha) * gv.y * gv.y; pv.y -= lr * gv.y / (sqrtf(sv.y) + eps);
    sv.z = alpha * sv.z + (1.f - alpha) * gv.z * gv.z; pv.z -= lr * gv.z / (sqrtf(sv.z) + eps);
    sv.w = alpha * sv.w + (1.f - alpha) * gv.w * gv.w; pv.w -= lr * gv.w / (sqrtf(sv.w) + eps);
    *reinterpret_cast<float4*>(p + i) = pv;
    *reinterpret_cast<float4*>(sq + i) = sv;
    if (zero_grad) *reinterpret_cast<float4*>(g + i) = make_float4(0.f, 0.f, 0.f, 0.f);
  }
  if (i < n && i + 3 >= n) {
    for (size_t j = i; j < n; ++j) {
      const float gv = g[j] * gscale;
      const float sv = alpha * sq[j] + (1.f - alpha) * gv * gv;
      sq[j] = sv;
      p[j] -= lr * gv / (sqrtf(sv) + eps);
      if (zero_grad) g[j] = 0.f;
    }
  }
}

extern "C" int stemgnn_fill_zero(void* ptr, size_t bytes, void* stream) {
  if (!ptr && bytes) return SG_EINVAL;
  SG_TRY(sg_zero_async(ptr, bytes, (hipStream_t)stream));
  return 0;
}

// ... 49 lines not shown
```

### stemgnn_amd/ops.py

```python
import os
import weakref

import torch

from . import _lib

_NSPLIT = 32
_side_streams = {}


def _side_stream(device, index=0):
    key = (str(device), index)
    st = _side_streams.get(key)
    if st is None:
        st = torch.cuda.Stream(device=device)
        _side_streams[key] = st
    return st


def fresh_side_stream(device, index=0):
    _side_streams.pop((str(device), index), None)
    return _side_stream(device, index)


class HotPathState:

    def __init__(self):
        self.direct = False
        self.overlap = False
        self.prepacked = None
        self.preseed = None
        self.fork_event = None
        self.pending = None
        self.exact_group = None
        self.gru_front_live = False
        self.dh_factors = None
        self.block_grads_hook = None
        self.gru_ctl = None
        self.gru_ctl_zeroed = False
        self.warm_saved = None
        self.tail_finish = None
        self.side_probe = None
        _states.add(self)

    def set(self, direct=True, overlap=False):
        self.direct = bool(direct)
        self.overlap = bool(direct) and bool(overlap)
        return self

    def join(self):
        item, self.pending = self.pending, None
        if item is not None:
            side, keep = item
            torch.cuda.current_stream().wait_stream(side)
            del keep

    def reset(self):
        for item in (self.prepacked, self.pending):
            if item is not None:
                try:
                    (item[1] if item is self.prepacked else item[0]).synchronize()
                except RuntimeError:
                    pass
        self.prepacked = None
        self.preseed = None
        self.fork_event = None
        self.pending = None
        self.dh_factors = None
        self.gru_ctl_zeroed = False
        self.tail_finish = None


_states = weakref.WeakSet()
_NO_STATE = None


def _state(state):
    global _NO_STATE
    if state is not None:
        return state
    if _NO_STATE is None:
        _NO_STATE = HotPathState()
# ... 195 lines not shown
                                                     gru_status(dev).data_ptr(), _stream()), "gru_bwd_recur")
        elif factors is not None:
            attn_scratch, fb, fn, wk, wq, after, dq_chunks = factors
            base = attn_scratch.data_ptr() + 4 * fn * fn
            tail = (x.data_ptr(), w_hh.data_ptr(), h_ext.data_ptr(), reserve.data_ptr(), B, S, Hd, W, scratch.data_ptr(),
                    dw_ih.data_ptr(), dw_hh.data_ptr(), db_ih.data_ptr(), db_hh.data_ptr(), gru_status(dev).data_ptr())
            args = (base, base + 4 * fb * fn, wk.data_ptr(), wq.data_ptr()) + tail
            beside = (ctx.state.overlap and ctx.state.pending is not None and ctx.state.gru_ctl_zeroed
                      and bool(lib.stemgnn_gru_bwd_overlap_ok(B, S, Hd, W))
                      and ctx.state.gru_ctl.numel() == lib.stemgnn_gru_bwd_ctl_words(S))
            ctx.state.gru_ctl_zeroed = False
            ctl = ctx.state.gru_ctl.data_ptr() if beside else None
            if beside:
                _lib.check(lib.stemgnn_gru_bwd_rank2_begin(*args, ctl, _stream()), "gru_bwd_rank2_begin")
            elif dq_chunks:
                wg_split = 1 if glu_splits() == 2 and os.environ.get("STEMGNN_WGRAD_BF16", "1") != "0" else 0
                _lib.check(lib.stemgnn_gru_bwd_rank2_dq(base, base + 4 * fb * fn, dq_chunks, wg_split, wk.data_ptr(), wq.data_ptr(),
                                                        *tail, _stream()), "gru_bwd_rank2_dq")
            else:
                _lib.check(lib.stemgnn_gru_bwd_rank2(*args, _stream()), "gru_bwd_rank2")
            if after is not None:
                after()
            if beside:
                side = ctx.state.pending[0]
                _lib.check(lib.stemgnn_gru_bwd_rank2_finish(*args, ctl, side.cuda_stream, _stream()), "gru_bwd_rank2_finish")
        else:
            _lib.check(lib.stemgnn_gru_bwd(dh_all.data_ptr(), x.data_ptr(), w_hh.data_ptr(), h_ext.data_ptr(),
                                           reserve.data_ptr(), B, S, Hd, W, scratch.data_ptr(), dw_ih.data_ptr(),
                                           dw_hh.data_ptr(), db_ih.data_ptr(), db_hh.data_ptr(),
                                           gru_status(dev).data_ptr(), _stream()), "gru_bwd")
        dx = None
        if ctx.needs_input_grad[0]:
            dx = torch.empty(B, W, S, device=dev, dtype=f32)
            _lib.check(lib.stemgnn_gru_input_grad(scratch.data_ptr(), w_ih.data_ptr(), B, S, Hd, W, dx.data_ptr(), _stream()),
                       "gru_input_grad")
        ctx.state.join()
        if direct or frozen:
            return dx, None, None, None, None, None
        return dx, dw_ih, dw_hh, db_ih, db_hh, None


class FcTail(torch.autograd.Function):

    @staticmethod
    def forward(ctx, fsum, w0, b0, w2, b2, state=None):
        lib = _lib.load()
        ctx.state = _state(state)
        fsum = fsum.contiguous()
        B, N, W = fsum.shape
        H = w2.shape[0]
        forecast = torch.empty(B, H, N, device=fsum.device, dtype=torch.float32)
        w0, b0, w2, b2 = (t.contiguous() for t in (w0, b0, w2, b2))
        _lib.check(lib.stemgnn_fc_tail_fwd(fsum.data_ptr(), w0.data_ptr(), b0.data_ptr(), w2.data_ptr(), b2.data_ptr(),
                                           B, N, W, H, forecast.data_ptr(), _stream()), "fc_tail_fwd")
        ctx.save_for_backward(fsum, w0, b0, w2)
        ctx.fc_params = (w0, b0, w2, b2)
        return forecast

    @staticmethod
    def backward(ctx, dforecast):
        lib = _lib.load()
        fsum, w0, b0, w2 = ctx.saved_tensors
        B, N, W = fsum.shape
        H = w2.shape[0]
        dev, f32 = fsum.device, torch.float32
        dforecast = dforecast.contiguous()
        prm = ctx.fc_params
        direct = ctx.state.direct and all(p.grad is not None and p.grad.is_contiguous() for p in prm)
        if direct:
            dw0, db0, dw2, db2 = (p.grad for p in prm)
        else:
            dw0, db0, dw2, db2 = (torch.empty_like(p) for p in prm)
        dfsum = torch.empty_like(fsum)
        scratch = torch.empty(lib.stemgnn_fc_tail_scratch_floats(B, N, W, H), device=dev, dtype=f32)
        _lib.check(lib.stemgnn_fc_tail_bwd(dforecast.data_ptr(), fsum.data_ptr(), w0.data_ptr(), b0.data_ptr(),
                                           w2.data_ptr(), B, N, W, H, scratch.data_ptr(), dfsum.data_ptr(),
                                           dw0.data_ptr(), db0.data_ptr(), dw2.data_ptr(), db2.data_ptr(), _stream()),
                   "fc_tail_bwd")
        if direct:
            return dfsum, None, None, None, None, None
        return dfsum, dw0, db0, dw2, db2, None


class FcTailMse(torch.autograd.Function):

    @staticmethod
    def forward(ctx, fsum, target, w0, b0, w2, b2, state=None, loss_out=None, accum=None, unit_grad=False):
        lib = _lib.load()
        ctx.state = _state(state)
        _require_gpu(fsum, "fsum")
        _require_gpu(target, "target")
        fsum, target = fsum.contiguous(), target.contiguous()
        B, N, W = fsum.shape
        H = w2.shape[0]
        if tuple(target.shape) != (B, H, N):
            raise _lib.StemGNNHipError(f"target must be [B,H,N]=({B},{H},{N}), got {tuple(target.shape)}")
        dev, f32 = fsum.device, torch.float32
        prm = (w0, b0, w2, b2)
        w0c, b0c, w2c, b2c = (t.contiguous() for t in prm)
        wanted = any(ctx.needs_input_grad[i] for i in (0, 2, 3, 4, 5))
        direct = ctx.state.direct and bool(unit_grad) and wanted and \
            all(p.grad is not None and p.grad.is_contiguous() for p in prm)
        grads = [p.grad for p in prm] if direct else [torch.empty_like(p) for p in prm]
        dfsum = torch.empty_like(fsum)
        loss = loss_out if loss_out is not None else torch.empty((), device=dev, dtype=f32)
        if accum is not None and (accum.dtype != torch.float64 or accum.device != dev):
            raise _lib.StemGNNHipError("accum must be a float64 scalar on the forecast's device")
        scratch = torch.empty(lib.stemgnn_fc_tail_train_scratch_floats(B, N, W, H), device=dev, dtype=f32)

        acc_ptr = accum.data_ptr() if accum is not None else None
        defer = direct and ctx.state.overlap and ctx.state.tail_finish is None
        if defer:
            _lib.check(lib.stemgnn_fc_tail_train_rows(
                fsum.data_ptr(), target.data_ptr(), w0c.data_ptr(), b0c.data_ptr(), w2c.data_ptr(), b2c.data_ptr(), B, N, W, H,
                scratch.data_ptr(), None, dfsum.data_ptr(), _stream()), "fc_tail_train_rows")
            g0, g1, g2, g3 = grads

            def finish(stream, scratch=scratch, loss=loss, g0=g0, g1=g1, g2=g2, g3=g3):
                _lib.check(lib.stemgnn_fc_tail_train_finish(scratch.data_ptr(), B, N, W, H, loss.data_ptr(), acc_ptr, g0.data_ptr(),
                                                            g1.data_ptr(), g2.data_ptr(), g3.data_ptr(), stream),
                           "fc_tail_train_finish")
            ctx.state.tail_finish = finish
        else:
            _lib.check(lib.stemgnn_fc_tail_train(
                fsum.data_ptr(), target.data_ptr(), w0c.data_ptr(), b0c.data_ptr(), w2c.data_ptr(), b2c.data_ptr(), B, N, W, H,
                scratch.data_ptr(), None, loss.data_ptr(), acc_ptr, dfsum.data_ptr(),
                grads[0].data_ptr(), grads[1].data_ptr(), grads[2].data_ptr(), grads[3].data_ptr(), _stream()), "fc_tail_train")
        ctx.direct, ctx.unit_grad = direct, bool(unit_grad)
        ctx.held = (dfsum, None if direct else grads)
        ctx.set_materialize_grads(False)
        if loss_out is not None:
            ctx.mark_dirty(loss_out)
        return loss

    @staticmethod
    def backward(ctx, grad_loss):
        dfsum, grads = ctx.held
        ctx.held = None
        if ctx.state.tail_finish is not None and not ctx.state.overlap:
            fin, ctx.state.tail_finish = ctx.state.tail_finish, None
            fin(_stream())
        if not ctx.unit_grad:
            dfsum = dfsum * grad_loss
            if grads is not None:
                grads = [g * grad_loss for g in grads]
        if grads is None:
            return dfsum, None, None, None, None, None, None, None, None, None
        return dfsum, None, grads[0], grads[1], grads[2], grads[3], None, None, None, None


class GluFn(torch.autograd.Function):

    @staticmethod
    def forward(ctx, x, wl, bl, wr, br):
        lib = _lib.load()
        for name, t in (("x", x), ("linear_left.weight", wl), ("linear_right.weight", wr)):
            _require_gpu(t, name)
        x, wl, bl, wr, br = (t.contiguous() for t in (x, wl, bl, wr, br))
        M, K = x.shape
        C = wl.shape[0]
        dev, st = x.device, _stream()
        U = torch.empty(M, C, device=dev)
        V = torch.empty(M, C, device=dev)
        for w, o in ((wl, U), (wr, V)):
            _lib.check(lib.stemgnn_sgemm_f32(x.data_ptr(), K, 1, w.data_ptr(), K, 1, o.data_ptr(), C, M, C, K, 0, st), "sgemm")
        out, gate, lin = (torch.empty(M, C, device=dev) for _ in range(3))
        _lib.check(lib.stemgnn_glu_combine_fwd(U.data_ptr(), V.data_ptr(), bl.data_ptr(), br.data_ptr(), out.data_ptr(),
                                               gate.data_ptr(), lin.data_ptr(), M, C, st), "glu_combine_fwd")
        ctx.save_for_backward(x, wl, wr, lin, gate)
        return out

    @staticmethod
    def backward(ctx, dout):
        lib = _lib.load()
        x, wl, wr, lin, gate = ctx.saved_tensors
        M, K = x.shape
        C = wl.shape[0]
        dev, st = x.device, _stream()
        dout = dout.contiguous()
        dU, dV = torch.empty(M, C, device=dev), torch.empty(M, C, device=dev)
        _lib.check(lib.stemgnn_glu_combine_bwd(dout.data_ptr(), lin.data_ptr(), gate.data_ptr(), dU.data_ptr(),
                                               dV.data_ptr(), M, C, st), "glu_combine_bwd")
        dx = torch.empty(M, K, device=dev)
        dwl, dwr = torch.empty_like(wl), torch.empty_like(wr)
        dbl, dbr = torch.empty(C, device=dev), torch.empty(C, device=dev)
        for i, (d, w, dw, db) in enumerate(((dU, wl, dwl, dbl), (dV, wr, dwr, dbr))):
            _lib.check(lib.stemgnn_sgemm_f32(d.data_ptr(), C, 1, w.data_ptr(), K, 0, dx.data_ptr(), K, M, K, C, int(i > 0), st), "sgemm")
            _lib.check(lib.stemgnn_sgemm_f32(d.data_ptr(), C, 0, x.data_ptr(), K, 0, dw.data_ptr(), K, C, K, M, 0, st), "sgemm")
            _lib.check(lib.stemgnn_colsum(d.data_ptr(), M, C, db.data_ptr(), st), "colsum")
        return dx, dwl, dbl, dwr, dbr


class StockBlockFn(torch.autograd.Function):

    @staticmethod
    def forward(ctx, X, mul_L, multi, has_bc, *params):
        lib = _lib.load()
        _require_gpu(X, "x")
        _require_gpu(mul_L, "mul_L")
        X = X.contiguous()
        mul_L = mul_L.contiguous()
        B, N, W = X.shape
        dev, f32 = X.device, torch.float32
        st = _stream()
        params = [None if p is None else p.contiguous() for p in params]
        tables = dft_tables(W, multi, dev)
        pk = torch.empty(lib.stemgnn_packed_floats(W, multi), device=dev, dtype=f32)
        sv = torch.empty(lib.stemgnn_saved_floats(B, N, W, multi), device=dev, dtype=f32)
        forecast = torch.empty(B, N, W, device=dev, dtype=f32)
        backcast = torch.empty(B, N, W, device=dev, dtype=f32) if has_bc else None
        parr = _lib.ptr_array(params)
        sb, sn, stt = N * W, W, 1
        _lib.check(lib.stemgnn_block_pack(parr, tables.data_ptr(), pk.data_ptr(), W, multi, st), "block_pack")
        _lib.check(lib.stemgnn_gft_fwd(mul_L.data_ptr(), X.data_ptr(), sb, sn, stt, sv.data_ptr(), B, N, W, st), "gft_fwd")
        _lib.check(lib.stemgnn_spectral_glu_fwd(pk.data_ptr(), sv.data_ptr(), B, N, W, multi, st), "spectral_glu_fwd")
        _lib.check(lib.stemgnn_igft_heads_fwd(parr, pk.data_ptr(), sv.data_ptr(), X.data_ptr(), sb, sn, stt,
                                              forecast.data_ptr(), 0, backcast.data_ptr() if has_bc else None,
                                              B, N, W, multi, st), "igft_heads_fwd")
        ctx.dims = (B, N, W, multi, bool(has_bc))
        ctx.params = params
        ctx.aux = (X, mul_L, tables, pk, sv, backcast.detach() if has_bc else None)
        if has_bc:
            return forecast, backcast
        return forecast, None

    @staticmethod
    def backward(ctx, dforecast, dbackcast):
        lib = _lib.load()
        B, N, W, multi, has_bc = ctx.dims
        X, mul_L, tables, pk, sv, backcast = ctx.aux
        params = ctx.params
# ... 16 lines not shown
        sb, sn, stt = N * W, W, 1
        _lib.check(lib.stemgnn_igft_heads_bwd(
            parr, pk.data_ptr(), sv.data_ptr(), X.data_ptr(), sb, sn, stt, dforecast.data_ptr(),
            dbackcast.contiguous().data_ptr() if use_bc else None, backcast.data_ptr() if use_bc else None,
            scratch.data_ptr(), gradpart.data_ptr(), nsplit, 1, B, N, W, multi, st), "igft_heads_bwd")
        _lib.check(lib.stemgnn_spectral_glu_bwd(pk.data_ptr(), sv.data_ptr(), scratch.data_ptr(), gradpart.data_ptr(),
                                                nsplit, 1, B, N, W, multi, st), "spectral_glu_bwd")
        _lib.check(lib.stemgnn_block_wgrad(parr, pk.data_ptr(), sv.data_ptr(), X.data_ptr(), sb, sn, stt,
                                           dforecast.data_ptr(), int(use_bc), scratch.data_ptr(), gradpart.data_ptr(),
                                           nsplit, 100, B, N, W, multi, st), "block_wgrad")
        _lib.check(lib.stemgnn_gft_bwd(mul_L.data_ptr(), X.data_ptr(), sb, sn, stt, dG.data_ptr(), dX.data_ptr(),
                                       dmul_L.data_ptr(), 0, B, N, W, st), "gft_bwd")
        grads = [None] * 33
        for i, p in enumerate(params):
            if p is None or (not has_bc and i in (7, 8)):
                continue
            grads[i] = torch.empty_like(p)
        _lib.check(lib.stemgnn_block_unpack_grads(gradpart.data_ptr(), nsplit, tables.data_ptr(), _lib.ptr_array(grads),
                                                  W, multi, int(has_bc), st), "block_unpack_grads")
        if use_bc and ctx.needs_input_grad[0]:
            _lib.check(lib.stemgnn_shortcut_dx(scratch.data_ptr(), params[7].data_ptr(), dX.data_ptr(), B, N, W, multi, st),
                       "shortcut_dx")
        return (dX, dmul_L, None, None, *grads)


_keep_attention_state = False
_last_attention_state = {}


def capture_attention_state(flag=True):
    global _keep_attention_state
    _keep_attention_state = bool(flag)
    if not flag:
        _last_attention_state.clear()


def last_attention_state(device):
    return _last_attention_state.get(str(torch.device(device)))


def prepack_blocks(state, block_params, W, multi, device, batch_shape=None):
    lib = _lib.load()
    side, main = _side_stream(device), torch.cuda.current_stream()
    tables = dft_tables(W, multi, device)
    n_packed = lib.stemgnn_packed_floats(W, multi)
    blocks = [[None if p is None else p.contiguous() for p in blk] for blk in block_params]
    packed = [torch.empty(n_packed, device=device, dtype=torch.float32) for _ in blocks]
    ev, state.fork_event = state.fork_event, None
    if ev is not None:
        side.wait_event(ev)
    else:
        side.wait_stream(main)
    splits = glu_splits()
    split = []
    for blk, pk in zip(blocks, packed):
        parr = _lib.ptr_array(blk)

        def pack(stream, parr=parr, pk=pk, blk=blk):
            _pack_block(lib, parr, tables, pk, W, multi, splits, stream)
        pack(side.cuda_stream)
        if state.side_probe is not None:
            state.side_probe.append(pack)
        if splits:
            split.append(_split_panels(lib, pk, W, multi, splits, device, side.cuda_stream))
    if batch_shape is not None and bool(lib.stemgnn_gru_bwd_overlap_ok(batch_shape[0], batch_shape[1], batch_shape[1], W)):
        nctl = lib.stemgnn_gru_bwd_ctl_words(batch_shape[1])
        if state.gru_ctl is None or state.gru_ctl.numel() != nctl or state.gru_ctl.device != torch.device(device):
            state.gru_ctl = torch.zeros(nctl, device=device, dtype=torch.int32)
        _lib.check(lib.stemgnn_fill_zero(state.gru_ctl.data_ptr(), 4 * nctl, side.cuda_stream), "fill_zero")
        state.gru_ctl_zeroed = True
    if batch_shape is not None and splits == 0 and os.environ.get("STEMGNN_GLU_WARM", "1") != "0":
        nwarm = lib.stemgnn_glu_warm_saved_floats(W, multi)
        if state.warm_saved is None or state.warm_saved.numel() != nwarm or state.warm_saved.device != torch.device(device):
            state.warm_saved = torch.zeros(nwarm, device=device, dtype=torch.float32)
        _lib.check(lib.stemgnn_spectral_glu_fwd_warm(packed[0].data_ptr(), split[0].data_ptr() if splits else None,
                                                     state.warm_saved.data_ptr(), batch_shape[0], batch_shape[1], W, multi,
                                                     splits, side.cuda_stream), "spectral_glu_fwd_warm")
    state.prepacked = (packed, side, blocks, (splits, split))


class SpectralHotPath(torch.autograd.Function):

    @staticmethod
    def forward(ctx, h, x, wk, wq, multi, alpha, drop_p, training, seed, state, *block_params):
        lib = _lib.load()
        state = ctx.state = _state(state)
        ctx.factored, state.gru_front_live = bool(getattr(state, "gru_front_live", False)), False
        for name, t in (("gru output", h), ("x", x), ("weight_key", wk), ("weight_query", wq)):
            _require_gpu(t, name)
        assert len(block_params) == 2 * _lib.SG_BLOCK_NPARAMS
        h = h.contiguous()
        x = x.contiguous()
        B, W, N = x.shape
        if h.shape != (N, B, N):
            raise _lib.StemGNNHipError(f"gru output must be [N,B,N]=({N},{B},{N}), got {tuple(h.shape)}")
        dev, f32 = x.device, torch.float32
        st = _stream()
        M = B * N
        blocks = [list(block_params[:33]), list(block_params[33:])]
        blocks = [[None if p is None else p.contiguous() for p in blk] for blk in blocks]
        tables = dft_tables(W, multi, dev)

        mul_L = torch.empty(4, N, N, device=dev, dtype=f32)
        attention = torch.empty(N, N, device=dev, dtype=f32)
        attn_saved = torch.empty(lib.stemgnn_attn_saved_floats(B, N), device=dev, dtype=f32)
        use_drop = bool(training) and drop_p > 0.0
        pre, state.prepacked = state.prepacked, None
        if pre is not None:
            torch.cuda.current_stream().wait_stream(pre[1])
        exact = state.exact_group
        for part in ((3,) if exact is None else (1, 2)):
            _lib.check(lib.stemgnn_attn_laplacian_fwd(
                h.data_ptr(), wk.data_ptr(), wq.data_ptr(), float(alpha), float(drop_p), int(bool(training)),
                seed.data_ptr() if use_drop else None, B, N, attn_saved.data_ptr(), attention.data_ptr(),
                mul_L.data_ptr(), part, st), "attn_laplacian_fwd")
            if exact is not None and part == 1:
                _all_reduce_mean(attn_saved[3 * B * N:3 * B * N + N * N + N], exact)
        if _keep_attention_state:
            _last_attention_state[str(dev)] = (attn_saved[:B * N].view(B, N).clone(),
                                               attn_saved[B * N:2 * B * N].view(B, N).clone())
        if os.environ.get("STEMGNN_SPECTRAL", "cheb") == "eig":
            lam = torch.empty(N, device=dev, dtype=f32)
            U = torch.empty(N, N, device=dev, dtype=f32)
            escr = torch.empty(lib.stemgnn_eigh_scratch_floats(N), device=dev, dtype=f32)
            _lib.check(lib.stemgnn_eigh_fwd(mul_L.data_ptr(), lam.data_ptr(), U.data_ptr(), escr.data_ptr(), N,
                                            0, st), "eigh_fwd")
        else:
            _lib.check(lib.stemgnn_cheb_fwd(mul_L.data_ptr(), N, st), "cheb_fwd")

        fsum = torch.empty(B, N, W, device=dev, dtype=f32)
        backcast = torch.empty(B, N, W, device=dev, dtype=f32)
        packed, saved, split = [], [], []
        splits = pre[3][0] if pre is not None else glu_splits()
        n_packed = lib.stemgnn_packed_floats(W, multi)
        n_saved = lib.stemgnn_saved_floats(B, N, W, multi)
        xviews = [(x, W * N, 1, N), (backcast, N * W, W, 1)]
        for s in range(2):
            sv = torch.empty(n_saved, device=dev, dtype=f32)
            parr = _lib.ptr_array(blocks[s])
            X, sb, sn, stt = xviews[s]
            sp = None
            if pre is not None:
                pk = pre[0][s]
                sp = pre[3][1][s] if splits else None
            else:
                pk = torch.empty(n_packed, device=dev, dtype=f32)
                _pack_block(lib, parr, tables, pk, W, multi, splits, st)
                if splits:
                    sp = _split_panels(lib, pk, W, multi, splits, dev, st)
            _lib.check(lib.stemgnn_gft_fwd(mul_L.data_ptr(), X.data_ptr(), sb, sn, stt, sv.data_ptr(), B, N, W, st),
                       "gft_fwd")
            if splits:
                _lib.check(lib.stemgnn_spectral_glu_fwd_split(pk.data_ptr(), sp.data_ptr(), sv.data_ptr(), B, N, W, multi,
                                                              splits, st), "spectral_glu_fwd_split")
            else:
                _lib.check(lib.stemgnn_spectral_glu_fwd(pk.data_ptr(), sv.data_ptr(), B, N, W, multi, st),
                           "spectral_glu_fwd")
            split.append(sp)
            _lib.check(lib.stemgnn_igft_heads_fwd(
                parr, pk.data_ptr(), sv.data_ptr(), X.data_ptr(), sb, sn, stt, fsum.data_ptr(), int(s == 1),
                backcast.data_ptr() if s == 0 else None, B, N, W, multi, st), "igft_heads_fwd")
            packed.append(pk)
            saved.append(sv)

        ctx.dims = (B, N, W, multi, float(alpha), float(drop_p), bool(training))
        ctx.blocks = blocks
        ctx.aux = (h, x, wk, wq, seed, tables, mul_L, attn_saved, backcast, packed, saved)
        ctx.split = (splits, split)
        ctx.mark_non_differentiable(mul_L)
        ctx.set_materialize_grads(False)
        return fsum, attention, mul_L

    @staticmethod
    def backward(ctx, dfsum, datt, _dmulL):
        if dfsum is None and datt is None:
            return (None,) * (10 + 2 * _lib.SG_BLOCK_NPARAMS)
        lib = _lib.load()
        B, N, W, multi, alpha, drop_p, training = ctx.dims
        h, x, wk, wq, seed, tables, mul_L, attn_saved, backcast, packed, saved = ctx.aux
        blocks = ctx.blocks
        state = ctx.state
        splits, split = ctx.split
        dev, f32 = x.device, torch.float32
        st = _stream()
        tail_finish, state.tail_finish = state.tail_finish, None
        if dfsum is None and tail_finish is not None:
            dfsum = torch.zeros(B, N, W, device=dev, dtype=f32)
        attn_only = dfsum is None
        if not attn_only:
            dfsum = dfsum.contiguous()
        if datt is not None:
            datt = datt.contiguous()
        nsplit = _NSPLIT
        n_scratch = lib.stemgnn_scratch_floats(B, N, W, multi)
        off_dG = lib.stemgnn_scratch_offset_dG(B, N, W, multi)
        n_gradpart = lib.stemgnn_gradpart_floats(W, multi, nsplit)
        dmul_L = None if attn_only else torch.empty(4, N, N, device=dev, dtype=f32)
        dbackcast = None if attn_only else torch.empty(B, N, W, device=dev, dtype=f32)
        xviews = [(x, W * N, 1, N), (backcast, N * W, W, 1)]
        grads = [[None] * 33, [None] * 33]
        direct_idx = set()
        nig = ctx.needs_input_grad
        live = [not attn_only and any(nig[10 + 33 * s + i] for i, p in enumerate(blocks[s]) if p is not None) for s in (0, 1)]
        kq_live = nig[2] or nig[3]
        for s in (1, 0):
            for i, p in enumerate(blocks[s]):
                if p is None or (s == 1 and i in (7, 8)) or not live[s]:
                    continue
                if state.direct and p.grad is not None and p.grad.is_contiguous():
                    grads[s][i] = p.grad
                    direct_idx.add((s, i))
                else:
                    grads[s][i] = torch.empty_like(p)
        n_block_grads = sum(g is not None for blk in grads for g in blk)
        overlap = state.overlap and n_block_grads > 0 and len(direct_idx) == n_block_grads
        side = _side_stream(dev) if overlap else None
        main = torch.cuda.current_stream()
        keep = []
        if tail_finish is not None and not overlap:
            tail_finish(st)
            tail_finish = None
        defer_b1 = overlap
        scratch0 = None if attn_only else torch.empty(n_scratch, device=dev, dtype=f32)
        gradpart0 = None if attn_only else torch.empty(n_gradpart, device=dev, dtype=f32)
        bufs = {0: (scratch0, gradpart0), 1: (scratch0, gradpart0)}
        if defer_b1:
            bufs[1] = (torch.empty(n_scratch, device=dev, dtype=f32), torch.empty(n_gradpart, device=dev, dtype=f32))

        def stage_fns(s):
            scratch, gradpart = bufs[s]
            parr = _lib.ptr_array(blocks[s])
            X, sb, sn, stt = xviews[s]
            has_bc = s == 0
            garr = _lib.ptr_array(grads[s])
            keep.append((parr, garr))

            def heads(stream):
                _lib.check(lib.stemgnn_igft_heads_bwd(
                    parr, packed[s].data_ptr(), saved[s].data_ptr(), X.data_ptr(), sb, sn, stt, dfsum.data_ptr(),
                    dbackcast.data_ptr() if has_bc else None, backcast.data_ptr() if has_bc else None,
                    scratch.data_ptr(), gradpart.data_ptr(), nsplit, 1, B, N, W, multi, stream), "igft_heads_bwd")

            def glu(stream):
                if splits:
                    _lib.check(lib.stemgnn_spectral_glu_dgrad_split(
                        packed[s].data_ptr(), split[s].data_ptr(), saved[s].data_ptr(), scratch.data_ptr(),
                        B, N, W, multi, splits, stream), "spectral_glu_dgrad_split")
                    return
                _lib.check(lib.stemgnn_spectral_glu_bwd(
                    packed[s].data_ptr(), saved[s].data_ptr(), scratch.data_ptr(), gradpart.data_ptr(), nsplit, 1,
                    B, N, W, multi, stream), "spectral_glu_bwd")

            def wgrad(stream, cu_percent):
                _lib.check(lib.stemgnn_block_wgrad_split(
                    parr, packed[s].data_ptr(), saved[s].data_ptr(), X.data_ptr(), sb, sn, stt, dfsum.data_ptr(),
                    int(has_bc), scratch.data_ptr(), gradpart.data_ptr(), nsplit, cu_percent, B, N, W, multi,
                    2 if splits == 2 and os.environ.get("STEMGNN_WGRAD_BF16", "1") != "0" else 0, stream), "block_wgrad")

            def unpack(stream):
                _lib.check(lib.stemgnn_block_unpack_grads(
                    gradpart.data_ptr(), nsplit, tables.data_ptr(), garr, W, multi, int(has_bc), stream),
                    "block_unpack_grads")

            return heads, glu, wgrad, unpack

        dt1 = None
        for s in (() if attn_only else (1, 0)):
            scratch = bufs[s][0]
            dG = scratch[off_dG:]
            X, sb, sn, stt = xviews[s]
            heads, glu, wgrad, unpack = stage_fns(s)
            heads(st)
            glu(st)
            if not overlap:
                if live[s]:
                    wgrad(st, 100)
                    unpack(st)
                _lib.check(lib.stemgnn_gft_bwd(
                    mul_L.data_ptr(), X.data_ptr(), sb, sn, stt, dG.data_ptr(),
                    dbackcast.data_ptr() if s == 1 else None, dmul_L.data_ptr(), int(s == 0), B, N, W, st), "gft_bwd")
            elif s == 1:
                _lib.check(lib.stemgnn_gft_bwd(mul_L.data_ptr(), X.data_ptr(), sb, sn, stt, dG.data_ptr(),
                                               dbackcast.data_ptr(), None, 0, B, N, W, st), "gft_bwd dX")
                dt1 = (X, sb, sn, stt, dG)
            else:
                fork = torch.cuda.Event()
                fork.record(main)
                X1, sb1, sn1, stt1, dG1 = dt1
                _lib.check(lib.stemgnn_gft_bwd_dt2(X.data_ptr(), sb, sn, stt, dG.data_ptr(), X1.data_ptr(), sb1, sn1, stt1,
                                                   dG1.data_ptr(), dmul_L.data_ptr(), B, N, W, st), "gft_bwd_dt2")
                side.wait_event(fork)
                with torch.cuda.stream(side):
                    sst = side.cuda_stream
                    for ss in (0, 1):
                        if not live[ss]:
                            continue
                        _h, _g, w2, u2 = (heads, glu, wgrad, unpack) if ss == 0 else stage_fns(1)
                        w2(sst, _wg_cu(ss, B, N))
                        u2(sst)
                        if state.side_probe is not None:
                            state.side_probe.append(lambda stream, w2=w2, pc=_wg_cu(ss, B, N): w2(stream, pc))
                            state.side_probe.append(u2)
                    if tail_finish is not None:
                        tail_finish(sst)
                        keep.append(tail_finish)
                        if state.side_probe is not None:
                            state.side_probe.append(tail_finish)
                    if state.block_grads_hook is not None:
                        state.block_grads_hook()
                keep.append(bufs)
        dX0 = None
        if nig[1] and not attn_only:
            X, sb, sn, stt = xviews[0]
            dX0 = torch.empty(B, N, W, device=dev, dtype=f32)
            _lib.check(lib.stemgnn_gft_bwd(mul_L.data_ptr(), X.data_ptr(), sb, sn, stt, scratch0[off_dG:].data_ptr(),
                                           dX0.data_ptr(), None, 0, B, N, W, st), "gft_bwd dX")
            _lib.check(lib.stemgnn_shortcut_dx(scratch0.data_ptr(), blocks[0][7].data_ptr(), dX0.data_ptr(), B, N, W, multi, st),
                       "shortcut_dx")
        if overlap:
            state.pending = (side, (keep, packed, saved, split, backcast, dfsum, dbackcast))
        dL = None
        if not attn_only:
            dL = torch.empty(N, N, device=dev, dtype=f32)
            cheb_scratch = torch.empty(2 * N * N, device=dev, dtype=f32)
            _lib.check(lib.stemgnn_cheb_bwd(mul_L.data_ptr(), dmul_L.data_ptr(), dL.data_ptr(), cheb_scratch.data_ptr(),
                                            N, st), "cheb_bwd")
        factored = ctx.factored and ctx.needs_input_grad[0] and bool(lib.stemgnn_gru_bwd_rank2_ok(B, N))
        dh = torch.empty(1, device=dev, dtype=f32).expand(N, B, N) if factored else torch.empty_like(h)
        kq_direct = kq_live and state.direct and wk.grad is not None and wq.grad is not None
        if kq_live:
            dwk = wk.grad if kq_direct else torch.empty_like(wk)
            dwq = wq.grad if kq_direct else torch.empty_like(wq)
        elif factored:
            dwk = dwq = None
        else:
            dwk, dwq = torch.empty(2, N, device=dev, dtype=f32)
        _ptr = lambda t: None if t is None else t.data_ptr()
        attn_scratch = torch.empty(lib.stemgnn_attn_scratch_floats(B, N, _NCHUNK), device=dev, dtype=f32)
        use_drop = training and drop_p > 0.0
        exact = state.exact_group
        follower = bool(overlap and ctx.factored and state.gru_ctl_zeroed and lib.stemgnn_gru_bwd_overlap_ok(B, N, N, W))
        dq_parts = bool(factored and overlap and kq_direct and not follower)
        if not kq_live:
            dq_parts = bool(factored and not follower)
        if datt is None:
            bwd_entry, head = lib.stemgnn_attn_laplacian_bwd, (dL.data_ptr(),)
        else:
            bwd_entry, head = lib.stemgnn_attn_laplacian_bwd_ext, (_ptr(dL), datt.data_ptr())
        for part in ((3,) if exact is None else (1, 2)):
            _lib.check(bwd_entry(
                *head, h.data_ptr(), wk.data_ptr(), wq.data_ptr(), alpha, drop_p, int(training),
                seed.data_ptr() if use_drop else None, B, N, attn_saved.data_ptr(), attn_scratch.data_ptr(), _NCHUNK,
                None if factored else dh.data_ptr(), _ptr(dwk), _ptr(dwq),
                part | ((4 | (8 if dq_parts else 0)) if factored and part != 1 else 0), st), "attn_laplacian_bwd")
            if exact is not None and part == 1:
                _all_reduce_mean(attn_scratch[:N * N], exact)
        if factored:
            after = None
            if overlap and kq_direct:
                kq_ready = torch.cuda.Event()
                kq_ready.record(main)
                pend, hh, kdwk, kdwq = state.pending, h, dwk, dwq
                dq2 = torch.empty(B, N, device=dev, dtype=f32) if dq_parts else None

                def kq_wgrad(stream):
                    if dq2 is not None:
                        _lib.check(lib.stemgnn_attn_dquery_reduce(attn_scratch.data_ptr(), B, N, _NCHUNK, dq2.data_ptr(), stream),
                                   "attn_dquery_reduce")
                        _lib.check(lib.stemgnn_keyquery_wgrad2(hh.data_ptr(), attn_scratch.data_ptr() + 4 * N * N, dq2.data_ptr(),
                                                               kdwk.data_ptr(), kdwq.data_ptr(), B, N, stream), "keyquery_wgrad2")
                        return
                    _lib.check(lib.stemgnn_keyquery_wgrad(hh.data_ptr(), attn_scratch.data_ptr(), kdwk.data_ptr(),
                                                          kdwq.data_ptr(), B, N, stream), "keyquery_wgrad")

                def after():
                    side.wait_event(kq_ready)
                    with torch.cuda.stream(side):
                        kq_wgrad(side.cuda_stream)
                    pend[1][0].append((attn_scratch, hh, dq2))
                if state.side_probe is not None:
                    state.side_probe.append(kq_wgrad)
            state.dh_factors = (attn_scratch, B, N, wk, wq, after, _NCHUNK if dq_parts else 0)
            if after is None and kq_live:
                _lib.check(lib.stemgnn_keyquery_wgrad(h.data_ptr(), attn_scratch.data_ptr(), dwk.data_ptr(), dwq.data_ptr(),
                                                      B, N, st), "keyquery_wgrad")
        for s_, i_ in direct_idx:
            grads[s_][i_] = None
        if kq_direct or not kq_live:
            dwk = dwq = None
        dx = dX0.permute(0, 2, 1) if dX0 is not None else None
        return (dh, dx, dwk, dwq, None, None, None, None, None, None, *grads[0], *grads[1])



def forecast_forward(x, gru_params, wk, wq, multi, alpha, drop_p, block_params, fc_params):
    lib = _lib.load()
    w_ih, w_hh, b_ih, b_hh = (t.contiguous() for t in gru_params)
    for name, t in (("x", x), ("GRU.weight_ih_l0", w_ih), ("GRU.weight_hh_l0", w_hh), ("weight_key", wk),
                    ("weight_query", wq)):
        _require_gpu(t, name)
    assert len(block_params) == 2 * _lib.SG_BLOCK_NPARAMS
    x = x.contiguous()
    B, W, N = x.shape
    Hd = w_hh.shape[1]
    if Hd != N:
        raise _lib.StemGNNHipError(f"GRU hidden size {Hd} != units {N}")
    dev, f32 = x.device, torch.float32
    st = _stream()
    h_ext = torch.empty(N + 1, B, Hd, device=dev, dtype=f32)
    gscr = torch.empty(lib.stemgnn_gru_fwd_scratch_floats(B, N, Hd), device=dev, dtype=f32)
    _lib.check(lib.stemgnn_gru_fwd_infer(x.data_ptr(), w_ih.data_ptr(), w_hh.data_ptr(), b_ih.data_ptr(), b_hh.data_ptr(),
                                         B, N, Hd, W, gscr.data_ptr(), h_ext.data_ptr(), gru_status(dev).data_ptr(), st),
               "gru_fwd_infer")
    del gscr
    mul_L = torch.empty(4, N, N, device=dev, dtype=f32)
    attention = torch.empty(N, N, device=dev, dtype=f32)
    attn_saved = torch.empty(lib.stemgnn_attn_saved_floats(B, N), device=dev, dtype=f32)
    _lib.check(lib.stemgnn_attn_laplacian_fwd(h_ext[1:].data_ptr(), wk.data_ptr(), wq.data_ptr(), float(alpha), float(drop_p),
                                              0, None, B, N, attn_saved.data_ptr(), attention.data_ptr(), mul_L.data_ptr(), 3,
                                              st), "attn_laplacian_fwd")
    if os.environ.get("STEMGNN_SPECTRAL", "cheb") == "eig":
        lam = torch.empty(N, device=dev, dtype=f32)
        U = torch.empty(N, N, device=dev, dtype=f32)
        escr = torch.empty(lib.stemgnn_eigh_scratch_floats(N), device=dev, dtype=f32)
        _lib.check(lib.stemgnn_eigh_fwd(mul_L.data_ptr(), lam.data_ptr(), U.data_ptr(), escr.data_ptr(), N, 0, st), "eigh_fwd")
    else:
        _lib.check(lib.stemgnn_cheb_fwd(mul_L.data_ptr(), N, st), "cheb_fwd")
    del attn_saved
    splits = glu_splits()
    tables = dft_tables(W, multi, dev)
    n_ws = lib.stemgnn_infer_workspace_split_floats(B, N, W, multi, splits)
    ws = torch.empty(n_ws, device=dev, dtype=f32)
    fsum = torch.empty(B, N, W, device=dev, dtype=f32)
    backcast = torch.empty(B, N, W, device=dev, dtype=f32)
    n_packed = lib.stemgnn_packed_floats(W, multi)
    blocks = [list(block_params[:33]), list(block_params[33:])]
    xviews = [(x, W * N, 1, N), (backcast, N * W, W, 1)]
    for s in range(2):
        blk = [None if p is None else p.contiguous() for p in blocks[s]]
        parr = _lib.ptr_array(blk)
        X, sb, sn, stt = xviews[s]
        pk = torch.empty(n_packed, device=dev, dtype=f32)
        _pack_block(lib, parr, tables, pk, W, multi, splits, st)
        _lib.check(lib.stemgnn_gft_fwd(mul_L.data_ptr(), X.data_ptr(), sb, sn, stt, ws.data_ptr(), B, N, W, st), "gft_fwd")
        if splits:
            sp = _split_panels(lib, pk, W, multi, splits, dev, st)
            _lib.check(lib.stemgnn_spectral_glu_fwd_split_infer(pk.data_ptr(), sp.data_ptr(), ws.data_ptr(), n_ws, B, N, W,
                                                                multi, splits, st), "spectral_glu_fwd_split_infer")
        else:
            _lib.check(lib.stemgnn_spectral_glu_fwd_infer(pk.data_ptr(), ws.data_ptr(), n_ws, B, N, W, multi, st),
                       "spectral_glu_fwd_infer")
        _lib.check(lib.stemgnn_igft_heads_fwd_infer(parr, pk.data_ptr(), ws.data_ptr(), n_ws, X.data_ptr(), sb, sn, stt,
                                                    fsum.data_ptr(), int(s == 1), backcast.data_ptr() if s == 0 else None,
                                                    B, N, W, multi, st), "igft_heads_fwd_infer")
    w0, b0, w2, b2 = (t.contiguous() for t in fc_params)
    H = w2.shape[0]
    forecast = torch.empty(B, H, N, device=dev, dtype=f32)
    _lib.check(lib.stemgnn_fc_tail_fwd(fsum.data_ptr(), w0.data_ptr(), b0.data_ptr(), w2.data_ptr(), b2.data_ptr(),
                                       B, N, W, H, forecast.data_ptr(), st), "fc_tail_fwd")
    return forecast, attention


def forecast_store(forecast, target, pos, out_forecast, out_target):
    lib = _lib.load()
    B, H, N = forecast.shape
    if target.shape != forecast.shape or out_forecast.shape[1:] != (H, N) or out_target.shape != out_forecast.shape:
        raise _lib.StemGNNHipError("forecast_store: shape mismatch")
    if pos.dtype != torch.int64 or pos.device != forecast.device:
        raise _lib.StemGNNHipError("forecast_store: pos must be an int64 tensor on the forecast's device")
    _lib.check(lib.stemgnn_forecast_store(forecast.data_ptr(), target.data_ptr(), pos.data_ptr(), out_forecast.data_ptr(),
                                          out_target.data_ptr(), B, H, N, out_forecast.shape[0], _stream()), "forecast_store")


class MSELossFn(torch.autograd.Function):
# ... 145 lines not shown
```

Before: 85060.

## Fuse block-1 heads forward, FC tail loss rows and heads backward into one kernel

Adds a turnaround kernel that, for the second stock block in unit-grad training, runs the iGFT heads forward, the FC-tail MSE row computation and the heads backward inside a single launch. The forecast sum stays in LDS instead of going through global memory, and the separate heads-forward and heads-backward launches are skipped in the autograd path. The fc-tail finish now runs immediately in that case. This adds a large LDS-heavy kernel and ties forward and backward scheduling together through a token object, so the block-1 heads work can no longer overlap with other work.

Result: no change. 85300 (median of 6 runs) (+0.3%).

```diff
diff --git a/include/stemgnn_hip.h b/include/stemgnn_hip.h
--- a/include/stemgnn_hip.h
+++ b/include/stemgnn_hip.h
@@ -187,7 +187,15 @@
 #define SG_PATH_LONG_K          32
 #define SG_PATH_WGRAD_FUSED     64
 #define SG_PATH_GLU_WGRAD_FUSED 128
+#define SG_PATH_HEADS_TURNAROUND 256
 int stemgnn_block_paths(int B, int N, int W, int multi, int splits);
+
+int stemgnn_block_turnaround(const float* const* params_host, const float* packed, float* saved, const float* X, long xs_b,
+                             long xs_n, long xs_t, float* fsum, const float* target, const float* w0, const float* b0,
+                             const float* w2, const float* b2, float* tail_scratch, float* forecast, float* dfsum,
+                             float* scratch, float* gradpart, int nsplit, int B, int N, int W, int multi, int H, int* path,
+                             void* stream);
+int stemgnn_block_turnaround_ok(int B, int N, int W, int multi, int H);
 
 size_t stemgnn_infer_workspace_floats(int B, int N, int W, int multi);
 size_t stemgnn_infer_workspace_split_floats(int B, int N, int W, int multi, int splits);
diff --git a/stemgnn_amd/_lib.py b/stemgnn_amd/_lib.py
--- a/stemgnn_amd/_lib.py
+++ b/stemgnn_amd/_lib.py
@@ -7,7 +7,7 @@
 SG_BLOCK_NPARAMS = 33
 SG_EINVAL = -10001
 SG_PATH = {"glu_fwd_fused": 1, "glu_dgrad_fused": 2, "heads_fwd_fused": 4, "heads_bwd_fused": 8, "heads_bwd_16w": 16,
-           "long_k": 32, "wgrad_fused": 64, "glu_wgrad_fused": 128}
+           "long_k": 32, "wgrad_fused": 64, "glu_wgrad_fused": 128, "heads_turnaround": 256}
 SG_GRU_PATH_WORDS = 16
 SG_GRU_WORD = {"fwd_family": 0, "fwd_P": 1, "fwd_K": 2, "gi_stream": 3, "bwd_family": 4, "bwd_P": 5, "bwd_KU": 6,
                "bwd_slices": 7, "ih_folded": 8, "hh_form": 9, "ih_slabs": 10, "rank2_ok": 11, "wide_passes": 12,
@@ -122,6 +122,9 @@
     "stemgnn_fc_tail_train_scratch_floats": (c_size_t, [c_int, c_int, c_int, c_int]),
     "stemgnn_fc_tail_train": (c_int, [_P, _P, _P, _P, _P, _P, c_int, c_int, c_int, c_int, _P, _P, _P, _P, _P, _P, _P, _P,
                                       _P, _P]),
+    "stemgnn_block_turnaround": (c_int, [_PP, _P, _P, _P, c_long, c_long, c_long, _P, _P, _P, _P, _P, _P, _P, _P, _P, _P, _P,
+                                         c_int, c_int, c_int, c_int, c_int, c_int, POINTER(c_int), _P]),
+    "stemgnn_block_turnaround_ok": (c_int, [c_int, c_int, c_int, c_int, c_int]),
     "stemgnn_fc_tail_train_rows": (c_int, [_P, _P, _P, _P, _P, _P, c_int, c_int, c_int, c_int, _P, _P, _P, _P]),
     "stemgnn_fc_tail_train_finish": (c_int, [_P, c_int, c_int, c_int, c_int, _P, _P, _P, _P, _P, _P, _P]),
     "stemgnn_infer_workspace_floats": (c_size_t, [c_int, c_int, c_int, c_int]),
diff --git a/stemgnn_amd/base_model.py b/stemgnn_amd/base_model.py
--- a/stemgnn_amd/base_model.py
+++ b/stemgnn_amd/base_model.py
@@ -140,7 +140,7 @@
             with torch.cuda.stream(ops._side_stream(device)):
                 hs.preseed = self._next_seed(device)
 
-    def hot_path(self, x):
+    def hot_path(self, x, turn=None):
         if not x.is_cuda:
             raise _lib.StemGNNHipError(
                 f"input is on {x.device}: stemgnn_amd.Model runs only on a HIP device (no CPU fallback)")
@@ -167,14 +167,23 @@
             seed = self._next_seed(x.device)
         params = blocks[0] + blocks[1]
         return SpectralHotPath.apply(h, x, self.weight_key, self.weight_query, self.multi_layer, self.alpha,
-                                     self.dropout_rate, self.training, seed, hs, *params)
+                                     self.dropout_rate, self.training, seed, hs, turn, *params)
 
     def loss(self, x, target, loss_out=None, accum=None, unit_grad=False, return_attention=False):
         self._require_fc_tail()
-        fsum, attention, _ = self.hot_path(x)
+        unit_grad = bool(unit_grad) and torch.is_grad_enabled()
+        turn = ops.Turnaround() if unit_grad and self._turnaround_ok() else None
+        fsum, attention, _ = self.hot_path(x, turn)
         loss = FcTailMse.apply(fsum, target, self.fc[0].weight, self.fc[0].bias, self.fc[2].weight, self.fc[2].bias,
-                               self.hot_state, loss_out, accum, bool(unit_grad) and torch.is_grad_enabled())
+                               self.hot_state, loss_out, accum, unit_grad, turn)
         return (loss, attention) if return_attention else loss
+
+    def _turnaround_ok(self):
+        if not (self.hot_state.direct and self.training and self.stack_cnt == 2 and ops.Turnaround.switch_on()):
+            return False
+        in_place = lambda p: p.requires_grad and p.grad is not None and p.grad.is_contiguous()
+        blk1 = [p for i, p in enumerate(self.stock_block[1].hip_params()) if p is not None and i not in (7, 8)]
+        return all(in_place(p) for p in blk1) and all(in_place(p) for p in self.fc.parameters())
 
     def _require_fc_tail(self):
         if not _lib.load().stemgnn_fc_tail_supported(self.time_step, self.horizon):
diff --git a/stemgnn_amd/csrc/block.hip b/stemgnn_amd/csrc/block.hip
--- a/stemgnn_amd/csrc/block.hip
+++ b/stemgnn_amd/csrc/block.hip
@@ -10,6 +10,7 @@
 #include "reduce.h"
 #include "wgrad.h"
 #include "heads.h"
+#include "heads_turnaround.h"
 #include "glu_fused.h"
 #include "glu_fused_bf16.h"
 
@@ -1119,6 +1120,10 @@
 static bool heads_fused_ok(const SgDims& d) {
   return hd_fwd_lds_floats(d.KF, d.WmP, d.W) * sizeof(float) <= (size_t)150 * 1024 && d.KF <= SG_LONG_K;
 }
+static int heads_fwd_waves() {
+  static const int waves_env = getenv("STEMGNN_HEADS_FWD_WAVES") ? atoi(getenv("STEMGNN_HEADS_FWD_WAVES")) : 8;
+  return waves_env == 8 ? 8 : 4;
+}
 template <bool SAVE = true>
 static int heads_fwd_impl(const float* const* params_host, const float* packed, const float* const (&a3)[2], float* ig, float* fs,
                           const float* X, long xs_b, long xs_n, long xs_t, float* forecast, int accumulate, float* backcast,
@@ -1139,8 +1144,7 @@
     a.ig = ig; a.fs = fs; a.forecast = forecast; a.backcast = backcast;
     a.M = d.M; a.W = W; a.Wm = d.Wm; a.WmP = d.WmP; a.KF = d.KF; a.accumulate = accumulate; a.has_bc = has_bc;
     a.lda = hd_lda(d.KF); a.ldi = d.WmP + 1;
-    static const int waves_env = getenv("STEMGNN_HEADS_FWD_WAVES") ? atoi(getenv("STEMGNN_HEADS_FWD_WAVES")) : 8;
-    if (waves_env == 8) {
+    if (heads_fwd_waves() == 8) {
       static SgDynLds lds_guard8;
       SG_TRY(sg_ensure_dyn_lds((const void*)sg_heads_fwd_kernel<8, SAVE>, hd_bytes, lds_guard8));
       hipLaunchKernelGGL((sg_heads_fwd_kernel<8, SAVE>), dim3((d.M + HD_RB - 1) / HD_RB), dim3(512), hd_bytes, st, a);
@@ -1360,6 +1364,72 @@
   return 0;
 }
 
+static bool heads_turn_ok(const SgDims& d, int H) {
+  return heads_fused_ok(d) && heads_bwd_fused_ok(d) && H > 0 && stemgnn_fc_tail_supported(d.W, H) &&
+         hd_turn_lds_floats(d.KF, d.WmP, d.W, H) * sizeof(float) <= (size_t)150 * 1024;
+}
+extern "C" int stemgnn_block_turnaround_ok(int B, int N, int W, int multi, int H) {
+  if (B <= 0 || N <= 0 || W <= 0 || multi <= 0 || H <= 0) return SG_EINVAL;
+  return heads_turn_ok(sg_dims(B, N, W, multi), H);
+}
+static bool heads_turn_default_waves() {
+  static const bool bwd_default = !getenv("STEMGNN_HEADS_BWD_WAVES") || atoi(getenv("STEMGNN_HEADS_BWD_WAVES")) == 16;
+  return heads_fwd_waves() == 8 && bwd_default;
+}
+extern "C" int stemgnn_block_turnaround(const float* const* params_host, const float* packed, float* saved, const float* X,
+                                        long xs_b, long xs_n, long xs_t, float* fsum, const float* target, const float* w0,
+                                        const float* b0, const float* w2, const float* b2, float* tail_scratch, float* forecast,
+                                        float* dfsum, float* scratch, float* gradpart, int nsplit, int B, int N, int W,
+                                        int multi, int H, int* path, void* stream) {
+  if (!params_host || !packed || !saved || !X || !fsum || !target || !w0 || !b0 || !w2 || !b2 || !tail_scratch || !dfsum ||
+      !scratch || !gradpart || nsplit <= 0 || B <= 0 || N <= 0 || W <= 0 || multi <= 0 || H <= 0 ||
+      !stemgnn_fc_tail_supported(W, H))
+    return SG_EINVAL;
+  const SgDims d = sg_dims(B, N, W, multi);
+  const char* sw = getenv("STEMGNN_HEADS_TURNAROUND");
+  const bool fused = !(sw && atoi(sw) == 0) && heads_turn_ok(d, H) && heads_turn_default_waves();
+  if (path) *path = fused;
+  if (!fused) {
+    int rc = stemgnn_igft_heads_fwd(params_host, packed, saved, X, xs_b, xs_n, xs_t, fsum, 1, nullptr, B, N, W, multi, stream);
+    if (rc) return rc;
+    rc = stemgnn_fc_tail_train_rows(fsum, target, w0, b0, w2, b2, B, N, W, H, tail_scratch, forecast, dfsum, stream);
+    if (rc) return rc;
+    return stemgnn_igft_heads_bwd(params_host, packed, saved, X, xs_b, xs_n, xs_t, dfsum, nullptr, nullptr, scratch, gradpart,
+                                  nsplit, 1, B, N, W, multi, stream);
+  }
+  const SgPackedLayout P = sg_packed_layout(d);
+  const SgSavedLayout S = sg_saved_layout(d);
+  const SgScratchLayout C = sg_scratch_layout(d);
+  HeadsTurnArgs a;
+  HeadsFwdArgs& f = a.f;
+  for (int r = 0; r < 2; ++r) { f.a3[r] = saved + S.out[r][2]; f.cp2[r] = d.CP2[r]; }
+  f.wfold = packed + P.wfold;
+  f.Fw = params_host[1]; f.Fb = params_host[2]; f.FRw = params_host[3]; f.FRb = params_host[4];
+  f.BCw = f.BCb = f.BSw = f.BSb = nullptr;
+  f.X = HdXView{X, xs_b, xs_n, xs_t, N};
+  f.ig = saved + S.ig; f.fs = saved + S.fs; f.forecast = fsum; f.backcast = nullptr;
+  f.M = d.M; f.W = W; f.Wm = d.Wm; f.WmP = d.WmP; f.KF = d.KF; f.accumulate = 1; f.has_bc = 0;
+  f.lda = hd_lda(d.KF); f.ldi = d.WmP + 1;
+  a.t = TailTrainArgs{nullptr, target, w0, b0, w2, b2, B, N, W, H, forecast, dfsum, tail_scratch};
+  HeadsBwdArgs& b = a.b;
+  b.dfo = nullptr; b.dbc = nullptr; b.bc = nullptr; b.fs = nullptr; b.wfold = f.wfold;
+  b.Fw = f.Fw; b.FRw = f.FRw; b.BCw = nullptr;
+  for (int r = 0; r < 2; ++r) {
+    b.out2[r] = nullptr; b.gate2[r] = saved + S.gate[r][2]; b.dpre2[r] = scratch + C.dact[r][2];
+    b.cp2[r] = d.CP2[r];
+  }
+  b.dpF = scratch + C.dpF; b.dpB = nullptr; b.dig = scratch + C.dig;
+  b.M = d.M; b.W = W; b.Wm = d.Wm; b.WmP = d.WmP; b.KF = d.KF; b.has_bc = 0;
+  b.ldi = d.WmP + 1; b.ldw = ((W + 3) & ~3) + 1;
+  const size_t lds = hd_turn_lds_floats(d.KF, d.WmP, W, H) * sizeof(float);
+  static SgDynLds lds_guard;
+  SG_TRY(sg_ensure_dyn_lds((const void*)sg_heads_turnaround_kernel<HD_TURN_WAVES>, lds, lds_guard));
+  hipLaunchKernelGGL(sg_heads_turnaround_kernel<HD_TURN_WAVES>, dim3((d.M + HD_RB - 1) / HD_RB), dim3(HD_TURN_WAVES * 64), lds,
+                     (hipStream_t)stream, a);
+  SG_TRY(hipGetLastError());
+  return 0;
+}
+
 __global__ void sg_shortcut_dx_kernel(const float* __restrict__ dpB, const float* __restrict__ bs_w, float* __restrict__ dX,
                                       size_t M, int W) {
   const size_t idx = (size_t)blockIdx.x * blockDim.x + threadIdx.x;
@@ -1483,6 +1553,7 @@
     if (heads_bwd_waves(d) == 16) bits |= SG_PATH_HEADS_BWD_16W;
   }
   if (d.KF > SG_LONG_K) bits |= SG_PATH_LONG_K;
+  if (heads_turn_ok(d, TAIL_MAXH)) bits |= SG_PATH_HEADS_TURNAROUND;
   WgGemm q[WG_MAXG];
   int n = 0;
   if (block_wgrad_list(d, base, base, base, base, Gl, 1, q, &n)) bits |= SG_PATH_WGRAD_FUSED;
diff --git a/stemgnn_amd/csrc/heads.h b/stemgnn_amd/csrc/heads.h
--- a/stemgnn_amd/csrc/heads.h
+++ b/stemgnn_amd/csrc/heads.h
@@ -93,21 +93,17 @@
 
 __device__ __forceinline__ float hd_sigmoid(float v) { return __frcp_rn(1.f + __expf(-v)); }
 
-template <int NW, bool SAVE = true>
-__global__ __launch_bounds__(NW * 64) void sg_heads_fwd_kernel(const HeadsFwdArgs g) {
+template <int NW, bool SAVE, bool KEEP>
+__device__ __forceinline__ void hd_fwd_body(const HeadsFwdArgs& g, float* As, float* igs, float* fss, float* Xs, float* fol,
+                                            int ldf, int tid, int m0, bool active) {
   constexpr int NT = NW * 64;
   constexpr bool SPLIT = NW == 8;
-  extern __shared__ __attribute__((aligned(16))) float hd_lds[];
-  float* As = hd_lds;
-  float* igs = As + HD_RB * g.lda;
-  float* fss = igs + HD_RB * g.ldi;
-  float* Xs = fss + HD_RB * g.ldi;
-  const int tid = threadIdx.x, lane = tid & 63, wave = tid >> 6;
-  const int m0 = blockIdx.x * HD_RB;
+  const int lane = tid & 63, wave = tid >> 6;
   const int M = g.M, W = g.W, Wm = g.Wm, KF = g.KF, lda = g.lda, ldi = g.ldi;
   const int KFp = (KF + 3) & ~3, Wmp4 = (Wm + 3) & ~3, W4 = (W + 3) & ~3;
 
-  {
+  const int xs = W4 + 1;
+  if (active) {
     const int cpr = KFp >> 2;
     const int nch = HD_RB * cpr;
     const int c0n = g.cp2[0] >> 2;
@@ -136,17 +132,16 @@
         }
       }
     }
-  }
-  const int xs = W4 + 1;
-  for (int e = tid; e < HD_RB * W4; e += NT) {
-    const int row = e / W4, t = e - row * W4;
-    const int m = m0 + row < M ? m0 + row : M - 1;
-    const int b = m / g.X.N;
-    Xs[row * xs + t] = (t < W && g.has_bc) ? g.X.p[b * g.X.sb + (m - b * g.X.N) * g.X.sn + (t < W ? t : 0) * g.X.st] : 0.f;
-  }
-  for (int e = tid; e < HD_RB * 4; e += NT) {
-    const int row = e >> 2, k = Wm + (e & 3);
-    if (k < ldi) { igs[row * ldi + k] = 0.f; fss[row * ldi + k] = 0.f; }
+    for (int e = tid; e < HD_RB * W4; e += NT) {
+      const int row = e / W4, t = e - row * W4;
+      const int m = m0 + row < M ? m0 + row : M - 1;
+      const int b = m / g.X.N;
+      Xs[row * xs + t] = (t < W && g.has_bc) ? g.X.p[b * g.X.sb + (m - b * g.X.N) * g.X.sn + (t < W ? t : 0) * g.X.st] : 0.f;
+    }
+    for (int e = tid; e < HD_RB * 4; e += NT) {
+      const int row = e >> 2, k = Wm + (e & 3);
+      if (k < ldi) { igs[row * ldi + k] = 0.f; fss[row * ldi + k] = 0.f; }
+    }
   }
   __syncthreads();
 
@@ -154,7 +149,7 @@
   const int nct = (Wm + 15) >> 4;
   const int cw = SPLIT ? (wave & 3) : wave;
   const int rh = SPLIT ? (wave >> 2) : 0;
-  for (int ct = cw; ct < nct; ct += 4) {
+  for (int ct = active ? cw : nct; ct < nct; ct += 4) {
     hd_f4 c0 = {0.f, 0.f, 0.f, 0.f}, c1 = c0;
     const float* wf = g.wfold + ct * 16;
     const int WmP = g.WmP;
@@ -176,7 +171,7 @@
     }
   }
   __syncthreads();
-  for (int ct = cw; ct < nct; ct += 4) {
+  for (int ct = active ? cw : nct; ct < nct; ct += 4) {
     hd_f4 c0 = {0.f, 0.f, 0.f, 0.f}, c1 = c0;
     const int col = ct * 16 + j;
     const float* fr = g.Fw + (size_t)(col < Wm ? col : Wm - 1) * Wm;
@@ -202,7 +197,7 @@
   __syncthreads();
   const int nwt = (W + 15) >> 4;
   const int rh3 = SPLIT ? ((wave >> 1) & 1) : 0;
-  for (int ct = SPLIT ? (wave >> 2) : (wave >> 1); ct < nwt; ct += 2) {
+  for (int ct = !active ? nwt : SPLIT ? (wave >> 2) : (wave >> 1); ct < nwt; ct += 2) {
     const int col = ct * 16 + j;
     const int cc = col < W ? col : W - 1;
     hd_f4 c0 = {0.f, 0.f, 0.f, 0.f}, c1 = c0;
@@ -216,9 +211,12 @@
       for (int reg = 0; reg < 4; ++reg) {
         const int r0 = rh3 * 16 + kq * 4 + reg, r1 = 16 + r0;
         if (col < W) {
-          if (m0 + r0 < M) { float* o = g.forecast + (size_t)(m0 + r0) * W + col; *o = (g.accumulate ? *o : 0.f) + c0[reg] + bias; }
+          float v0 = 0.f, v1 = 0.f;
+          if (m0 + r0 < M) { float* o = g.forecast + (size_t)(m0 + r0) * W + col; *o = v0 = (g.accumulate ? *o : 0.f) + c0[reg] + bias; }
+          if constexpr (KEEP) fol[r0 * ldf + col] = v0;
           if constexpr (!SPLIT) {
-            if (m0 + r1 < M) { float* o = g.forecast + (size_t)(m0 + r1) * W + col; *o = (g.accumulate ? *o : 0.f) + c1[reg] + bias; }
+            if (m0 + r1 < M) { float* o = g.forecast + (size_t)(m0 + r1) * W + col; *o = v1 = (g.accumulate ? *o : 0.f) + c1[reg] + bias; }
+            if constexpr (KEEP) fol[r1 * ldf + col] = v1;
           }
         }
       }
@@ -248,6 +246,16 @@
       }
     }
   }
+}
+
+template <int NW, bool SAVE = true>
+__global__ __launch_bounds__(NW * 64) void sg_heads_fwd_kernel(const HeadsFwdArgs g) {
+  extern __shared__ __attribute__((aligned(16))) float hd_lds[];
+  float* As = hd_lds;
+  float* igs = As + HD_RB * g.lda;
+  float* fss = igs + HD_RB * g.ldi;
+  float* Xs = fss + HD_RB * g.ldi;
+  hd_fwd_body<NW, SAVE, false>(g, As, igs, fss, Xs, nullptr, 0, threadIdx.x, blockIdx.x * HD_RB, true);
 }
 
 struct HeadsBwdArgs {
@@ -304,6 +312,150 @@
   }
 }
 
+template <int TJ>
+struct HdSaved {
+  float gt[TJ][2][4], yv[TJ][2][4];
+};
+template <int TJ, bool YV>
+__device__ __forceinline__ void hd_bwd_load_saved(const HeadsBwdArgs& g, int ct0, int m0, int j, int kq, HdSaved<TJ>& S) {
+  const int M = g.M, KF = g.KF;
+#pragma unroll
+  for (int t = 0; t < TJ; ++t) {
+    const int kk = (ct0 + t) * 16 + j;
+    const int kc = kk < KF ? kk : KF - 1;
+    const int r = kc >= g.cp2[0];
+    const int cch = kc - (r ? g.cp2[0] : 0), cp = g.cp2[r];
+    const float* pg = g.gate2[r] + cch;
+    const float* py = g.out2[r] + cch;
+#pragma unroll
+    for (int reg = 0; reg < 4; ++reg)
+#pragma unroll
+      for (int h = 0; h < 2; ++h) {
+        const int mm = m0 + h * 16 + kq * 4 + reg;
+        const size_t o = (size_t)(mm < M ? mm : M - 1) * cp;
+        S.gt[t][h][reg] = pg[o];
+        if constexpr (YV) S.yv[t][h][reg] = py[o];
+      }
+  }
+}
+template <int TJ>
+__device__ __forceinline__ void hd_bwd_yv_lds(const float* __restrict__ As, int lda, int KF, int ct0, int j, int kq,
+                                              HdSaved<TJ>& S) {
+#pragma unroll
+  for (int t = 0; t < TJ; ++t) {
+    const int kk = (ct0 + t) * 16 + j;
+    const int kc = kk < KF ? kk : KF - 1;
+#pragma unroll
+    for (int reg = 0; reg < 4; ++reg)
+#pragma unroll
+      for (int h = 0; h < 2; ++h) S.yv[t][h][reg] = As[(h * 16 + kq * 4 + reg) * lda + kc];
+  }
+}
+__device__ __forceinline__ void hd_bwd_load_fs(const HeadsBwdArgs& g, int ct, int m0, int j, int kq, float (&sv)[2][4]) {
+  const int M = g.M, Wm = g.Wm;
+  const int col = ct * 16 + j, cc = col < Wm ? col : Wm - 1;
+#pragma unroll
+  for (int reg = 0; reg < 4; ++reg)
+#pragma unroll
+    for (int h = 0; h < 2; ++h) {
+      const int r = h * 16 + kq * 4 + reg;
+      const int m = m0 + r < M ? m0 + r : M - 1;
+      sv[h][reg] = g.fs[(size_t)m * Wm + cc];
+    }
+}
+
+template <int NW, bool FUSED>
+__device__ __forceinline__ void hd_bwd_phases(const HeadsBwdArgs& g, float* dpFs, float* digs, const float* dfos,
+                                              const float* dpBs, const float* fss, const float* As, int lda,
+                                              HdSaved<16 / NW>& S, float (&sv)[2][4], bool hoist, bool hoist_fs, int tid, int m0) {
+  constexpr int TJ = 16 / NW;
+  const int lane = tid & 63, wave = tid >> 6;
+  const int M = g.M, W = g.W, Wm = g.Wm, KF = g.KF, ldi = g.ldi, ldw = g.ldw, WmP = g.WmP;
+  const int Wmp4 = (Wm + 3) & ~3, W4 = (W + 3) & ~3;
+  const int j = lane & 15, kq = lane >> 4;
+  const int nkt = (KF + 15) >> 4, nct = (Wm + 15) >> 4;
+  for (int ct = wave; ct < nct; ct += NW) {
+    hd_f4 c[1][2] = {{{0.f, 0.f, 0.f, 0.f}, {0.f, 0.f, 0.f, 0.f}}};
+    const int col = ct * 16 + j, cc = col < Wm ? col : Wm - 1;
+    const float* fr = g.FRw + cc;
+    hd_gemm_tiles<1>(dfos, ldw, W4, [&](int k, int) { return fr[(size_t)(k < W ? k : W - 1) * Wm]; }, kq, j, c);
+    if constexpr (FUSED) {
+#pragma unroll
+      for (int reg = 0; reg < 4; ++reg)
+#pragma unroll
+        for (int h = 0; h < 2; ++h) sv[h][reg] = fss[(h * 16 + kq * 4 + reg) * ldi + cc];
+    } else if (!hoist_fs) hd_bwd_load_fs(g, ct, m0, j, kq, sv);
+#pragma unroll
+    for (int reg = 0; reg < 4; ++reg)
+#pragma unroll
+      for (int h = 0; h < 2; ++h) {
+        const int r = h * 16 + kq * 4 + reg;
+        const float s = sv[h][reg];
+        const float v = c[0][h][reg] * s * (1.f - s);
+        if (col < Wm) {
+          dpFs[r * ldi + col] = v;
+          if (m0 + r < M) g.dpF[(size_t)(m0 + r) * Wm + col] = v;
+        }
+      }
+  }
+  __syncthreads();
+  for (int ct = wave; ct < nct; ct += NW) {
+    hd_f4 c[1][2] = {{{0.f, 0.f, 0.f, 0.f}, {0.f, 0.f, 0.f, 0.f}}};
+    const int col = ct * 16 + j, cc = col < Wm ? col : Wm - 1;
+    const float* fw = g.Fw + cc;
+    hd_gemm_tiles<1>(dpFs, ldi, Wmp4, [&](int k, int) { return fw[(size_t)(k < Wm ? k : Wm - 1) * Wm]; }, kq, j, c);
+    if (!FUSED && g.has_bc) {
+      const float* bw = g.BCw + cc;
+      hd_gemm_tiles<1>(dpBs, ldw, W4, [&](int k, int) { return bw[(size_t)(k < W ? k : W - 1) * Wm]; }, kq, j, c);
+    }
+#pragma unroll
+    for (int reg = 0; reg < 4; ++reg)
+#pragma unroll
+      for (int h = 0; h < 2; ++h) {
+        const int r = h * 16 + kq * 4 + reg;
+        if (col < Wm) {
+          digs[r * ldi + col] = c[0][h][reg];
+          if (m0 + r < M) g.dig[(size_t)(m0 + r) * Wm + col] = c[0][h][reg];
+        }
+      }
+  }
+  __syncthreads();
+  for (int ct0 = wave * TJ; ct0 < nkt; ct0 += TJ * NW) {
+    hd_f4 c[TJ][2];
+#pragma unroll
+    for (int t = 0; t < TJ; ++t) { c[t][0] = (hd_f4){0.f, 0.f, 0.f, 0.f}; c[t][1] = c[t][0]; }
+    const float* wr[TJ];
+#pragma unroll
+    for (int t = 0; t < TJ; ++t) {
+      const int kk = (ct0 + t) * 16 + j;
+      wr[t] = g.wfold + (size_t)(kk < KF ? kk : KF - 1) * WmP;
+    }
+    hd_gemm_tiles<TJ>(digs, ldi, Wmp4, [&](int k, int t) { return wr[t][k < Wm ? k : Wm - 1]; }, kq, j, c);
+    if (!hoist) hd_bwd_load_saved<TJ, !FUSED>(g, ct0, m0, j, kq, S);
+    if constexpr (FUSED) hd_bwd_yv_lds<TJ>(As, lda, KF, ct0, j, kq, S);
+#pragma unroll
+    for (int t = 0; t < TJ; ++t) {
+      const int kk = (ct0 + t) * 16 + j;
+      const int kc = kk < KF ? kk : KF - 1;
+      const int r = kc >= g.cp2[0];
+      const int cch = kc - (r ? g.cp2[0] : 0), cp = g.cp2[r];
+      const int q = ((cch >> 4) << 5) + (cch & 15);
+#pragma unroll
+      for (int reg = 0; reg < 4; ++reg)
+#pragma unroll
+        for (int h = 0; h < 2; ++h) {
+          const int m = m0 + h * 16 + kq * 4 + reg;
+          const float v = c[t][h][reg];
+          if (m < M && kk < KF) {
+            float* dp = g.dpre2[r] + (size_t)m * 2 * cp + q;
+            dp[0] = v * S.gt[t][h][reg];
+            dp[16] = v * S.yv[t][h][reg] * (1.f - S.gt[t][h][reg]);
+          }
+        }
+    }
+  }
+}
+
 template <int NW>
 __global__ __launch_bounds__(NW * 64) void sg_heads_bwd_kernel(const HeadsBwdArgs g) {
   constexpr int NT = NW * 64;
@@ -314,50 +466,19 @@
   float* dpBs = dfos + HD_RB * g.ldw;
   const int tid = threadIdx.x, lane = tid & 63, wave = tid >> 6;
   const int m0 = blockIdx.x * HD_RB;
-  const int M = g.M, W = g.W, Wm = g.Wm, KF = g.KF, ldi = g.ldi, ldw = g.ldw, WmP = g.WmP;
-  const int Wmp4 = (Wm + 3) & ~3, W4 = (W + 3) & ~3;
+  const int M = g.M, W = g.W, Wm = g.Wm, KF = g.KF, ldi = g.ldi, ldw = g.ldw;
+  const int W4 = (W + 3) & ~3;
 
   const int j = lane & 15, kq = lane >> 4;
   const int nkt = (KF + 15) >> 4;
   constexpr int TJ = 16 / NW;
   const bool hoist = nkt <= 16;
-  float gt[TJ][2][4], yv[TJ][2][4];
-  auto load_saved = [&](int ct0) {
-#pragma unroll
-    for (int t = 0; t < TJ; ++t) {
-      const int kk = (ct0 + t) * 16 + j;
-      const int kc = kk < KF ? kk : KF - 1;
-      const int r = kc >= g.cp2[0];
-      const int cch = kc - (r ? g.cp2[0] : 0), cp = g.cp2[r];
-      const float* pg = g.gate2[r] + cch;
-      const float* py = g.out2[r] + cch;
-#pragma unroll
-      for (int reg = 0; reg < 4; ++reg)
-#pragma unroll
-        for (int h = 0; h < 2; ++h) {
-          const int mm = m0 + h * 16 + kq * 4 + reg;
-          const size_t o = (size_t)(mm < M ? mm : M - 1) * cp;
-          gt[t][h][reg] = pg[o];
-          yv[t][h][reg] = py[o];
-        }
-    }
-  };
-  if (hoist) load_saved(wave * TJ);
+  HdSaved<TJ> S;
+  if (hoist) hd_bwd_load_saved<TJ, true>(g, wave * TJ, m0, j, kq, S);
   const int nct = (Wm + 15) >> 4;
   const bool hoist_fs = nct <= NW;
   float sv[2][4];
-  auto load_fs = [&](int ct) {
-    const int col = ct * 16 + j, cc = col < Wm ? col : Wm - 1;
-#pragma unroll
-    for (int reg = 0; reg < 4; ++reg)
-#pragma unroll
-      for (int h = 0; h < 2; ++h) {
-        const int r = h * 16 + kq * 4 + reg;
-        const int m = m0 + r < M ? m0 + r : M - 1;
-        sv[h][reg] = g.fs[(size_t)m * Wm + cc];
-      }
-  };
-  if (hoist_fs) load_fs(wave < nct ? wave : nct - 1);
+  if (hoist_fs) hd_bwd_load_fs(g, wave < nct ? wave : nct - 1, m0, j, kq, sv);
 
   for (int e = tid; e < HD_RB * W4; e += NT) {
     const int row = e / W4, t = e - row * W4;
@@ -378,79 +499,5 @@
     if (k < ldi) { dpFs[row * ldi + k] = 0.f; digs[row * ldi + k] = 0.f; }
   }
   __syncthreads();
-
-  for (int ct = wave; ct < nct; ct += NW) {
-    hd_f4 c[1][2] = {{{0.f, 0.f, 0.f, 0.f}, {0.f, 0.f, 0.f, 0.f}}};
-    const int col = ct * 16 + j, cc = col < Wm ? col : Wm - 1;
-    const float* fr = g.FRw + cc;
-    hd_gemm_tiles<1>(dfos, ldw, W4, [&](int k, int) { return fr[(size_t)(k < W ? k : W - 1) * Wm]; }, kq, j, c);
-    if (!hoist_fs) load_fs(ct);
-#pragma unroll
-    for (int reg = 0; reg < 4; ++reg)
-#pragma unroll
-      for (int h = 0; h < 2; ++h) {
-        const int r = h * 16 + kq * 4 + reg;
-        const float s = sv[h][reg];
-        const float v = c[0][h][reg] * s * (1.f - s);
-        if (col < Wm) {
-          dpFs[r * ldi + col] = v;
-          if (m0 + r < M) g.dpF[(size_t)(m0 + r) * Wm + col] = v;
-        }
-      }
-  }
-  __syncthreads();
-  for (int ct = wave; ct < nct; ct += NW) {
-    hd_f4 c[1][2] = {{{0.f, 0.f, 0.f, 0.f}, {0.f, 0.f, 0.f, 0.f}}};
-    const int col = ct * 16 + j, cc = col < Wm ? col : Wm - 1;
-    const float* fw = g.Fw + cc;
-    hd_gemm_tiles<1>(dpFs, ldi, Wmp4, [&](int k, int) { return fw[(size_t)(k < Wm ? k : Wm - 1) * Wm]; }, kq, j, c);
-    if (g.has_bc) {
-      const float* bw = g.BCw + cc;
-      hd_gemm_tiles<1>(dpBs, ldw, W4, [&](int k, int) { return bw[(size_t)(k < W ? k : W - 1) * Wm]; }, kq, j, c);
-    }
-#pragma unroll
-    for (int reg = 0; reg < 4; ++reg)
-#pragma unroll
-      for (int h = 0; h < 2; ++h) {
-        const int r = h * 16 + kq * 4 + reg;
-        if (col < Wm) {
-          digs[r * ldi + col] = c[0][h][reg];
-          if (m0 + r < M) g.dig[(size_t)(m0 + r) * Wm + col] = c[0][h][reg];
-        }
-      }
-  }
-  __syncthreads();
-  for (int ct0 = wave * TJ; ct0 < nkt; ct0 += TJ * NW) {
-    hd_f4 c[TJ][2];
-#pragma unroll
-    for (int t = 0; t < TJ; ++t) { c[t][0] = (hd_f4){0.f, 0.f, 0.f, 0.f}; c[t][1] = c[t][0]; }
-    const float* wr[TJ];
-#pragma unroll
-    for (int t = 0; t < TJ; ++t) {
-      const int kk = (ct0 + t) * 16 + j;
-      wr[t] = g.wfold + (size_t)(kk < KF ? kk : KF - 1) * WmP;
-    }
-    hd_gemm_tiles<TJ>(digs, ldi, Wmp4, [&](int k, int t) { return wr[t][k < Wm ? k : Wm - 1]; }, kq, j, c);
-    if (!hoist) load_saved(ct0);
-#pragma unroll
-    for (int t = 0; t < TJ; ++t) {
-      const int kk = (ct0 + t) * 16 + j;
-      const int kc = kk < KF ? kk : KF - 1;
-      const int r = kc >= g.cp2[0];
-      const int cch = kc - (r ? g.cp2[0] : 0), cp = g.cp2[r];
-      const int q = ((cch >> 4) << 5) + (cch & 15);
-#pragma unroll
-      for (int reg = 0; reg < 4; ++reg)
-#pragma unroll
-        for (int h = 0; h < 2; ++h) {
-          const int m = m0 + h * 16 + kq * 4 + reg;
-          const float v = c[t][h][reg];
-          if (m < M && kk < KF) {
-            float* dp = g.dpre2[r] + (size_t)m * 2 * cp + q;
-            dp[0] = v * gt[t][h][reg];
-            dp[16] = v * yv[t][h][reg] * (1.f - gt[t][h][reg]);
-          }
-        }
-    }
-  }
-}
+  hd_bwd_phases<NW, false>(g, dpFs, digs, dfos, dpBs, nullptr, nullptr, 0, S, sv, hoist, hoist_fs, tid, m0);
+}
diff --git a/stemgnn_amd/csrc/heads_turnaround.h b/stemgnn_amd/csrc/heads_turnaround.h
--- /dev/null
+++ b/stemgnn_amd/csrc/heads_turnaround.h
@@ -0,0 +1,60 @@
+#pragma once
+#include "heads.h"
+#include "tail_rows.h"
+
+static_assert(HD_RB == TRAIN_RB, "the turnaround kernel runs the heads and the tail on the same row blocks");
+
+#ifndef HD_TURN_WAVES
+#define HD_TURN_WAVES 16
+#endif
+
+struct HeadsTurnArgs {
+  HeadsFwdArgs f;
+  TailTrainArgs t;
+  HeadsBwdArgs b;
+};
+static inline size_t hd_turn_lds_floats(int KF, int WmP, int W, int H) {
+  return hd_fwd_lds_floats(KF, WmP, W) + tail_train_lds_floats(W, H) + hd_bwd_lds_floats(WmP, W);
+}
+
+template <int NW>
+__global__ __launch_bounds__(NW * 64) void sg_heads_turnaround_kernel(const HeadsTurnArgs g) {
+  static_assert(NW == 8 || NW == 16, "the forward's eight-wave form needs eight waves");
+  constexpr int NT = NW * 64, TJ = 16 / NW;
+  extern __shared__ __attribute__((aligned(16))) float hd_lds[];
+  const HeadsFwdArgs& f = g.f;
+  const HeadsBwdArgs& b = g.b;
+  const int W = f.W, H = g.t.H, Wm = f.Wm, ldi = f.ldi, ldw = b.ldw;
+  const int W4 = (W + 3) & ~3;
+  float* As = hd_lds;
+  float* igs = As + HD_RB * f.lda;
+  float* fss = igs + HD_RB * ldi;
+  float* Xs = fss + HD_RB * ldi;
+  float* tl = Xs + HD_RB * (W4 + 1);
+  const TailTrainLds L = tail_train_carve(tl, W, H);
+  float* dpFs = tl + tail_train_lds_floats(W, H);
+  float* digs = dpFs + HD_RB * ldi;
+  float* dfos = digs + HD_RB * ldi;
+  const int tid = threadIdx.x, lane = tid & 63, wave = tid >> 6;
+  const int m0 = blockIdx.x * HD_RB;
+  const int j = lane & 15, kq = lane >> 4;
+
+  const int nkt = (f.KF + 15) >> 4;
+  const bool hoist = nkt <= 16;
+  HdSaved<TJ> S;
+  if (hoist) hd_bwd_load_saved<TJ, false>(b, wave * TJ, m0, j, kq, S);
+  float sv[2][4];
+  for (int e = tid; e < HD_RB * 4; e += NT) {
+    const int row = e >> 2, k = Wm + (e & 3), t = W + (e & 3);
+    if (k < ldi) { dpFs[row * ldi + k] = 0.f; digs[row * ldi + k] = 0.f; }
+    if (t < W4) dfos[row * ldw + t] = 0.f;
+  }
+  if (tid < TRAIN_NT) tail_train_stage_weights(g.t, L, tid);
+
+  hd_fwd_body<8, true, true>(f, As, igs, fss, Xs, L.sx, W + 1, tid, m0, tid < 8 * 64);
+  __syncthreads();
+  tail_train_rows_body<true>(g.t, L, tid, m0, tid < TRAIN_NT, dfos, ldw);
+  __syncthreads();
+  if (wave >= NW - 4) tail_train_partials(g.t, L, tid - (NW - 4) * 64, blockIdx.x);
+  hd_bwd_phases<NW, true>(b, dpFs, digs, dfos, nullptr, fss, As, f.lda, S, sv, hoist, false, tid, m0);
+}
diff --git a/stemgnn_amd/csrc/tail.hip b/stemgnn_amd/csrc/tail.hip
--- a/stemgnn_amd/csrc/tail.hip
+++ b/stemgnn_amd/csrc/tail.hip
@@ -3,6 +3,7 @@
 
 #include "../../include/stemgnn_hip.h"
 #include "devattr.h"
+#include "tail_rows.h"
 
 #define SG_TRY(e)                                \
   do {                                           \
@@ -10,8 +11,6 @@
     if (_e != hipSuccess) return -(int)_e;       \
   } while (0)
 
-constexpr int TAIL_MAXW = 64;
-constexpr int TAIL_MAXH = 32;
 constexpr int TAIL_RB = 64;
 
 
@@ -179,90 +178,20 @@
   return 0;
 }
 
-constexpr int TRAIN_RB = 32;
-constexpr int TRAIN_RQ = 256 / TRAIN_RB;
 __global__ __launch_bounds__(256) void sg_fc_tail_train_kernel(const float* __restrict__ fsum, const float* __restrict__ target,
                                                                const float* __restrict__ w0, const float* __restrict__ b0,
                                                                const float* __restrict__ w2, const float* __restrict__ b2,
                                                                int B, int N, int W, int H, float* __restrict__ forecast,
                                                                float* __restrict__ dfsum, float* __restrict__ partial) {
   extern __shared__ __attribute__((aligned(16))) float sm[];
-  const int nacc = W * W + W + H * W + H;
-  float* sw0 = sm;
-  float* sb0 = sw0 + W * W;
-  float* sw2 = sb0 + W;
-  float* sb2 = sw2 + H * W;
-  float* sx = sb2 + H;
-  float* sdz = sx + TRAIN_RB * (W + 1);
-  float* sa = sdz + TRAIN_RB * (W + 1);
-  float* sdy = sa + TRAIN_RB * (W + 1);
-  float* sred = sdy + TRAIN_RB * (H + 1);
-  const int tid = threadIdx.x, r = tid % TRAIN_RB, q = tid / TRAIN_RB;
-  const int M = B * N, m0 = blockIdx.x * TRAIN_RB, m = m0 + r;
-  for (int i = tid; i < W * W; i += 256) sw0[i] = w0[i];
-  for (int i = tid; i < W; i += 256) sb0[i] = b0[i];
-  for (int i = tid; i < H * W; i += 256) sw2[i] = w2[i];
-  for (int i = tid; i < H; i += 256) sb2[i] = b2[i];
-  for (int i = tid; i < TRAIN_RB * W; i += 256) {
-    const int rr = i / W, t = i - rr * W;
-    sx[rr * (W + 1) + t] = m0 + rr < M ? fsum[(size_t)m0 * W + i] : 0.f;
-  }
-  __syncthreads();
-  for (int t = q; t < W; t += TRAIN_RQ) {
-    float z = sb0[t];
-    for (int u = 0; u < W; ++u) z = fmaf(sx[r * (W + 1) + u], sw0[t * W + u], z);
-    sdz[r * (W + 1) + t] = z;
-    sa[r * (W + 1) + t] = m < M ? (z > 0.f ? z : 0.01f * z) : 0.f;
-  }
-  __syncthreads();
-  float sq = 0.f;
-  {
-    const int mc = m < M ? m : 0, b = mc / N, n = mc - b * N;
-    const float scale = 2.f / ((float)B * (float)H * (float)N);
-    for (int h = q; h < H; h += TRAIN_RQ) {
-      float y = sb2[h];
-      for (int t = 0; t < W; ++t) y = fmaf(sa[r * (W + 1) + t], sw2[h * W + t], y);
-      const size_t o = ((size_t)b * H + h) * N + n;
-      const float d = m < M ? y - target[o] : 0.f;
-      if (m < M && forecast) forecast[o] = y;
-      sq = fmaf(d, d, sq);
-      sdy[r * (H + 1) + h] = d * scale;
-    }
-  }
-  sred[tid] = sq;
-  __syncthreads();
-  for (int t = q; t < W; t += TRAIN_RQ) {
-    const float z = sdz[r * (W + 1) + t];
-    float da = 0.f;
-    for (int h = 0; h < H; ++h) da = fmaf(sdy[r * (H + 1) + h], sw2[h * W + t], da);
-    sdz[r * (W + 1) + t] = m < M ? (z > 0.f ? da : 0.01f * da) : 0.f;
-  }
-  __syncthreads();
-  if (m < M)
-    for (int u = q; u < W; u += TRAIN_RQ) {
-      float d = 0.f;
-      for (int t = 0; t < W; ++t) d = fmaf(sdz[r * (W + 1) + t], sw0[t * W + u], d);
-      dfsum[(size_t)m * W + u] = d;
-    }
-  for (int e = tid; e < nacc + 1; e += 256) {
-    float sum = 0.f;
-    if (e < W * W) {
-      const int t = e / W, u = e - t * W;
-      for (int rr = 0; rr < TRAIN_RB; ++rr) sum = fmaf(sdz[rr * (W + 1) + t], sx[rr * (W + 1) + u], sum);
-    } else if (e < W * W + W) {
-      const int t = e - W * W;
-      for (int rr = 0; rr < TRAIN_RB; ++rr) sum += sdz[rr * (W + 1) + t];
-    } else if (e < W * W + W + H * W) {
-      const int qq = e - W * W - W, h = qq / W, t = qq - h * W;
-      for (int rr = 0; rr < TRAIN_RB; ++rr) sum = fmaf(sdy[rr * (H + 1) + h], sa[rr * (W + 1) + t], sum);
-    } else if (e < nacc) {
-      const int h = e - W * W - W - H * W;
-      for (int rr = 0; rr < TRAIN_RB; ++rr) sum += sdy[rr * (H + 1) + h];
-    } else {
-      for (int i = 0; i < 256; ++i) sum += sred[i];
-    }
-    partial[(size_t)blockIdx.x * (nacc + 1) + e] = sum;
-  }
+  const TailTrainArgs a{fsum, target, w0, b0, w2, b2, B, N, W, H, forecast, dfsum, partial};
+  const TailTrainLds L = tail_train_carve(sm, W, H);
+  const int tid = threadIdx.x, m0 = blockIdx.x * TRAIN_RB;
+  tail_train_stage_weights(a, L, tid);
+  tail_train_stage_rows(a, L, tid, m0);
+  __syncthreads();
+  tail_train_rows_body<false>(a, L, tid, m0, true, nullptr, 0);
+  tail_train_partials(a, L, tid, blockIdx.x);
 }
 
 __global__ __launch_bounds__(256) void sg_fc_tail_train_reduce_kernel(const float* __restrict__ partial, int nblocks, int W,
@@ -302,7 +231,7 @@
 }
 
 static size_t fc_tail_train_lds(int W, int H) {
-  return (size_t)(W * W + W + H * W + H + TRAIN_RB * (3 * (W + 1) + H + 1) + 256) * sizeof(float);
+  return tail_train_lds_floats(W, H) * sizeof(float);
 }
 extern "C" size_t stemgnn_fc_tail_train_scratch_floats(int B, int N, int W, int H) {
   return (size_t)((B * N + TRAIN_RB - 1) / TRAIN_RB) * (W * W + W + H * W + H + 1);
diff --git a/stemgnn_amd/csrc/tail_rows.h b/stemgnn_amd/csrc/tail_rows.h
--- /dev/null
+++ b/stemgnn_amd/csrc/tail_rows.h
@@ -0,0 +1,131 @@
+#pragma once
+#include <hip/hip_runtime.h>
+
+constexpr int TAIL_MAXW = 64;
+constexpr int TAIL_MAXH = 32;
+constexpr int TRAIN_RB = 32;
+constexpr int TRAIN_NT = 256;
+constexpr int TRAIN_RQ = TRAIN_NT / TRAIN_RB;
+
+struct TailTrainArgs {
+  const float *fsum, *target, *w0, *b0, *w2, *b2;
+  int B, N, W, H;
+  float *forecast, *dfsum, *partial;
+};
+
+struct TailTrainLds {
+  float *sw0, *sb0, *sw2, *sb2;
+  float *sx, *sdz, *sa;
+  float *sdy;
+  float *sred;
+};
+__host__ __device__ static inline size_t tail_train_lds_floats(int W, int H) {
+  return (size_t)(W * W + W + H * W + H + TRAIN_RB * (3 * (W + 1) + H + 1) + TRAIN_NT);
+}
+__device__ __forceinline__ TailTrainLds tail_train_carve(float* sm, int W, int H) {
+  TailTrainLds L;
+  L.sw0 = sm;
+  L.sb0 = L.sw0 + W * W;
+  L.sw2 = L.sb0 + W;
+  L.sb2 = L.sw2 + H * W;
+  L.sx = L.sb2 + H;
+  L.sdz = L.sx + TRAIN_RB * (W + 1);
+  L.sa = L.sdz + TRAIN_RB * (W + 1);
+  L.sdy = L.sa + TRAIN_RB * (W + 1);
+  L.sred = L.sdy + TRAIN_RB * (H + 1);
+  return L;
+}
+
+__device__ __forceinline__ void tail_train_stage_weights(const TailTrainArgs& a, const TailTrainLds& L, int tid) {
+  const int W = a.W, H = a.H;
+  for (int i = tid; i < W * W; i += TRAIN_NT) L.sw0[i] = a.w0[i];
+  for (int i = tid; i < W; i += TRAIN_NT) L.sb0[i] = a.b0[i];
+  for (int i = tid; i < H * W; i += TRAIN_NT) L.sw2[i] = a.w2[i];
+  for (int i = tid; i < H; i += TRAIN_NT) L.sb2[i] = a.b2[i];
+}
+__device__ __forceinline__ void tail_train_stage_rows(const TailTrainArgs& a, const TailTrainLds& L, int tid, int m0) {
+  const int W = a.W, M = a.B * a.N;
+  for (int i = tid; i < TRAIN_RB * W; i += TRAIN_NT) {
+    const int rr = i / W, t = i - rr * W;
+    L.sx[rr * (W + 1) + t] = m0 + rr < M ? a.fsum[(size_t)m0 * W + i] : 0.f;
+  }
+}
+
+template <bool KEEP>
+__device__ __forceinline__ void tail_train_rows_body(const TailTrainArgs& a, const TailTrainLds& L, int tid, int m0, bool active,
+                                                     float* dfs_lds, int ldw) {
+  const int B = a.B, N = a.N, W = a.W, H = a.H;
+  const int r = tid % TRAIN_RB, q = tid / TRAIN_RB;
+  const int M = B * N, m = m0 + r;
+  float* sx = L.sx; float* sdz = L.sdz; float* sa = L.sa; float* sdy = L.sdy;
+  const float *sw0 = L.sw0, *sb0 = L.sb0, *sw2 = L.sw2, *sb2 = L.sb2;
+  if (active)
+    for (int t = q; t < W; t += TRAIN_RQ) {
+      float z = sb0[t];
+      for (int u = 0; u < W; ++u) z = fmaf(sx[r * (W + 1) + u], sw0[t * W + u], z);
+      sdz[r * (W + 1) + t] = z;
+      sa[r * (W + 1) + t] = m < M ? (z > 0.f ? z : 0.01f * z) : 0.f;
+    }
+  __syncthreads();
+  if (active) {
+    float sq = 0.f;
+    const int mc = m < M ? m : 0, b = mc / N, n = mc - b * N;
+    const float scale = 2.f / ((float)B * (float)H * (float)N);
+    for (int h = q; h < H; h += TRAIN_RQ) {
+      float y = sb2[h];
+      for (int t = 0; t < W; ++t) y = fmaf(sa[r * (W + 1) + t], sw2[h * W + t], y);
+      const size_t o = ((size_t)b * H + h) * N + n;
+      const float d = m < M ? y - a.target[o] : 0.f;
+      if (m < M && a.forecast) a.forecast[o] = y;
+      sq = fmaf(d, d, sq);
+      sdy[r * (H + 1) + h] = d * scale;
+    }
+    L.sred[tid] = sq;
+  }
+  __syncthreads();
+  if (active)
+    for (int t = q; t < W; t += TRAIN_RQ) {
+      const float z = sdz[r * (W + 1) + t];
+      float da = 0.f;
+      for (int h = 0; h < H; ++h) da = fmaf(sdy[r * (H + 1) + h], sw2[h * W + t], da);
+      sdz[r * (W + 1) + t] = m < M ? (z > 0.f ? da : 0.01f * da) : 0.f;
+    }
+  __syncthreads();
+  if (active) {
+    if (m < M) {
+      for (int u = q; u < W; u += TRAIN_RQ) {
+        float d = 0.f;
+        for (int t = 0; t < W; ++t) d = fmaf(sdz[r * (W + 1) + t], sw0[t * W + u], d);
+        a.dfsum[(size_t)m * W + u] = d;
+        if constexpr (KEEP) dfs_lds[r * ldw + u] = d;
+      }
+    } else if constexpr (KEEP) {
+      for (int u = q; u < W; u += TRAIN_RQ) dfs_lds[r * ldw + u] = 0.f;
+    }
+  }
+}
+
+__device__ __forceinline__ void tail_train_partials(const TailTrainArgs& a, const TailTrainLds& L, int tid, int block) {
+  const int W = a.W, H = a.H;
+  const int nacc = W * W + W + H * W + H;
+  const float *sx = L.sx, *sdz = L.sdz, *sa = L.sa, *sdy = L.sdy, *sred = L.sred;
+  for (int e = tid; e < nacc + 1; e += TRAIN_NT) {
+    float sum = 0.f;
+    if (e < W * W) {
+      const int t = e / W, u = e - t * W;
+      for (int rr = 0; rr < TRAIN_RB; ++rr) sum = fmaf(sdz[rr * (W + 1) + t], sx[rr * (W + 1) + u], sum);
+    } else if (e < W * W + W) {
+      const int t = e - W * W;
+      for (int rr = 0; rr < TRAIN_RB; ++rr) sum += sdz[rr * (W + 1) + t];
+    } else if (e < W * W + W + H * W) {
+      const int qq = e - W * W - W, h = qq / W, t = qq - h * W;
+      for (int rr = 0; rr < TRAIN_RB; ++rr) sum = fmaf(sdy[rr * (H + 1) + h], sa[rr * (W + 1) + t], sum);
+    } else if (e < nacc) {
+      const int h = e - W * W - W - H * W;
+      for (int rr = 0; rr < TRAIN_RB; ++rr) sum += sdy[rr * (H + 1) + h];
+    } else {
+      for (int i = 0; i < TRAIN_NT; ++i) sum += sred[i];
+    }
+    a.partial[(size_t)block * (nacc + 1) + e] = sum;
+  }
+}
diff --git a/stemgnn_amd/ops.py b/stemgnn_amd/ops.py
--- a/stemgnn_amd/ops.py
+++ b/stemgnn_amd/ops.py
@@ -1,3 +1,4 @@
+import ctypes
 import os
 import weakref
 
@@ -359,10 +360,23 @@
         return dfsum, dw0, db0, dw2, db2, None
 
 
+class Turnaround:
+
+    def __init__(self):
+        self.fwd = None
+        self.done = False
+        self.fused = None
+        self.scratch = self.gradpart = self.dfsum = None
+
+    @staticmethod
+    def switch_on():
+        return os.environ.get("STEMGNN_HEADS_TURNAROUND", "1") != "0"
+
+
 class FcTailMse(torch.autograd.Function):
 
     @staticmethod
-    def forward(ctx, fsum, target, w0, b0, w2, b2, state=None, loss_out=None, accum=None, unit_grad=False):
+    def forward(ctx, fsum, target, w0, b0, w2, b2, state=None, loss_out=None, accum=None, unit_grad=False, turn=None):
         lib = _lib.load()
         ctx.state = _state(state)
         _require_gpu(fsum, "fsum")
@@ -387,17 +401,34 @@
 
         acc_ptr = accum.data_ptr() if accum is not None else None
         defer = direct and ctx.state.overlap and ctx.state.tail_finish is None
-        if defer:
+        if turn is not None:
+            if not direct or turn.fwd is None or turn.fwd[8].data_ptr() != fsum.data_ptr():
+                raise _lib.StemGNNHipError("FcTailMse: a Turnaround token needs direct fc gradients and its own hot-path forward")
+            parr, _blk, pk, sv, X, sb, sn, stt, _f, (tB, tN, tW, multi) = turn.fwd
+            turn.scratch = torch.empty(lib.stemgnn_scratch_floats(B, N, W, multi), device=dev, dtype=f32)
+            turn.gradpart = torch.empty(lib.stemgnn_gradpart_floats(W, multi, _NSPLIT), device=dev, dtype=f32)
+            path = ctypes.c_int(-1)
+            _lib.check(lib.stemgnn_block_turnaround(
+                parr, pk.data_ptr(), sv.data_ptr(), X.data_ptr(), sb, sn, stt, fsum.data_ptr(), target.data_ptr(),
+                w0c.data_ptr(), b0c.data_ptr(), w2c.data_ptr(), b2c.data_ptr(), scratch.data_ptr(), None, dfsum.data_ptr(),
+                turn.scratch.data_ptr(), turn.gradpart.data_ptr(), _NSPLIT, B, N, W, multi, H, ctypes.byref(path),
+                _stream()), "block_turnaround")
+            turn.fused, turn.dfsum, turn.done = int(path.value), dfsum, True
+        elif defer:
             _lib.check(lib.stemgnn_fc_tail_train_rows(
                 fsum.data_ptr(), target.data_ptr(), w0c.data_ptr(), b0c.data_ptr(), w2c.data_ptr(), b2c.data_ptr(), B, N, W, H,
                 scratch.data_ptr(), None, dfsum.data_ptr(), _stream()), "fc_tail_train_rows")
+        if turn is not None or defer:
             g0, g1, g2, g3 = grads
 
             def finish(stream, scratch=scratch, loss=loss, g0=g0, g1=g1, g2=g2, g3=g3):
                 _lib.check(lib.stemgnn_fc_tail_train_finish(scratch.data_ptr(), B, N, W, H, loss.data_ptr(), acc_ptr, g0.data_ptr(),
                                                             g1.data_ptr(), g2.data_ptr(), g3.data_ptr(), stream),
                            "fc_tail_train_finish")
-            ctx.state.tail_finish = finish
+            if defer:
+                ctx.state.tail_finish = finish
+            else:
+                finish(_stream())
         else:
             _lib.check(lib.stemgnn_fc_tail_train(
                 fsum.data_ptr(), target.data_ptr(), w0c.data_ptr(), b0c.data_ptr(), w2c.data_ptr(), b2c.data_ptr(), B, N, W, H,
@@ -422,8 +453,8 @@
             if grads is not None:
                 grads = [g * grad_loss for g in grads]
         if grads is None:
-            return dfsum, None, None, None, None, None, None, None, None, None
-        return dfsum, None, grads[0], grads[1], grads[2], grads[3], None, None, None, None
+            return dfsum, None, None, None, None, None, None, None, None, None, None
+        return dfsum, None, grads[0], grads[1], grads[2], grads[3], None, None, None, None, None
 
 
 class GluFn(torch.autograd.Function):
@@ -606,9 +637,11 @@
 class SpectralHotPath(torch.autograd.Function):
 
     @staticmethod
-    def forward(ctx, h, x, wk, wq, multi, alpha, drop_p, training, seed, state, *block_params):
+    def forward(ctx, h, x, wk, wq, multi, alpha, drop_p, training, seed, state, turn, *block_params):
         lib = _lib.load()
         state = ctx.state = _state(state)
+        state.tail_finish = None
+        ctx.turn = turn
         ctx.factored, state.gru_front_live = bool(getattr(state, "gru_front_live", False)), False
         for name, t in (("gru output", h), ("x", x), ("weight_key", wk), ("weight_query", wq)):
             _require_gpu(t, name)
@@ -681,9 +714,12 @@
                 _lib.check(lib.stemgnn_spectral_glu_fwd(pk.data_ptr(), sv.data_ptr(), B, N, W, multi, st),
                            "spectral_glu_fwd")
             split.append(sp)
-            _lib.check(lib.stemgnn_igft_heads_fwd(
-                parr, pk.data_ptr(), sv.data_ptr(), X.data_ptr(), sb, sn, stt, fsum.data_ptr(), int(s == 1),
-                backcast.data_ptr() if s == 0 else None, B, N, W, multi, st), "igft_heads_fwd")
+            if s == 1 and turn is not None:
+                turn.fwd = (parr, blocks[s], pk, sv, X, sb, sn, stt, fsum, (B, N, W, multi))
+            else:
+                _lib.check(lib.stemgnn_igft_heads_fwd(
+                    parr, pk.data_ptr(), sv.data_ptr(), X.data_ptr(), sb, sn, stt, fsum.data_ptr(), int(s == 1),
+                    backcast.data_ptr() if s == 0 else None, B, N, W, multi, st), "igft_heads_fwd")
             packed.append(pk)
             saved.append(sv)
 
@@ -698,7 +734,7 @@
     @staticmethod
     def backward(ctx, dfsum, datt, _dmulL):
         if dfsum is None and datt is None:
-            return (None,) * (10 + 2 * _lib.SG_BLOCK_NPARAMS)
+            return (None,) * (11 + 2 * _lib.SG_BLOCK_NPARAMS)
         lib = _lib.load()
         B, N, W, multi, alpha, drop_p, training = ctx.dims
         h, x, wk, wq, seed, tables, mul_L, attn_saved, backcast, packed, saved = ctx.aux
@@ -708,6 +744,10 @@
         dev, f32 = x.device, torch.float32
         st = _stream()
         tail_finish, state.tail_finish = state.tail_finish, None
+        turn = ctx.turn
+        if turn is not None and not turn.done:
+            raise _lib.StemGNNHipError("SpectralHotPath.backward: the Turnaround token's launch (FcTailMse.forward) never ran")
+        turned = turn is not None and dfsum is not None and dfsum.data_ptr() == turn.dfsum.data_ptr()
         if dfsum is None and tail_finish is not None:
             dfsum = torch.zeros(B, N, W, device=dev, dtype=f32)
         attn_only = dfsum is None
@@ -725,7 +765,7 @@
         grads = [[None] * 33, [None] * 33]
         direct_idx = set()
         nig = ctx.needs_input_grad
-        live = [not attn_only and any(nig[10 + 33 * s + i] for i, p in enumerate(blocks[s]) if p is not None) for s in (0, 1)]
+        live = [not attn_only and any(nig[11 + 33 * s + i] for i, p in enumerate(blocks[s]) if p is not None) for s in (0, 1)]
         kq_live = nig[2] or nig[3]
         for s in (1, 0):
             for i, p in enumerate(blocks[s]):
@@ -748,7 +788,9 @@
         scratch0 = None if attn_only else torch.empty(n_scratch, device=dev, dtype=f32)
         gradpart0 = None if attn_only else torch.empty(n_gradpart, device=dev, dtype=f32)
         bufs = {0: (scratch0, gradpart0), 1: (scratch0, gradpart0)}
-        if defer_b1:
+        if turn is not None:
+            bufs[1] = (turn.scratch, turn.gradpart)
+        elif defer_b1:
             bufs[1] = (torch.empty(n_scratch, device=dev, dtype=f32), torch.empty(n_gradpart, device=dev, dtype=f32))
 
         def stage_fns(s):
@@ -794,7 +836,8 @@
             dG = scratch[off_dG:]
             X, sb, sn, stt = xviews[s]
             heads, glu, wgrad, unpack = stage_fns(s)
-            heads(st)
+            if not (s == 1 and turned):
+                heads(st)
             glu(st)
             if not overlap:
                 if live[s]:
@@ -913,7 +956,7 @@
         if kq_direct or not kq_live:
             dwk = dwq = None
         dx = dX0.permute(0, 2, 1) if dX0 is not None else None
-        return (dh, dx, dwk, dwq, None, None, None, None, None, None, *grads[0], *grads[1])
+        return (dh, dx, dwk, dwq, None, None, None, None, None, None, None, *grads[0], *grads[1])
 
 
 
```
